# asbschmidt/CUDASW4

Hardware: AMD Instinct MI355X
Metric: GCUPS (higher is better)
Workload: dtype f16x2; 1 GPU; peak: allqueries.fasta (20 queries, 41752 residues) vs pseudo DB 1000000 x 512, half2 kernel configuration, blosum62, gop -11 gex -1, top 10, C++ host driver; db_subjects=1000000, db_residues=512000000, queries=20, kernel=half2, queries_in_flight=1, tail_overlaps=10, numa_node_rank0=0, numa_bound=True, resident=True, residency=resident, cached_chars=512000000, parallelism=db-shard x1 (one DB sharded), one top-K gather per step + host merge

## Files before the change

### cudasw4_amd/capi.py

```python
import ctypes
import os

_HERE = os.path.dirname(os.path.abspath(__file__))
LIB_PATH = os.environ.get("CUDASW4_AMD_LIB", os.path.join(_HERE, "lib", "libcudasw4_amd.so"))

KIND_F16X2, KIND_I16X2, KIND_I32, KIND_F32 = 0, 1, 2, 3
KIND_NAMES = {"half2": KIND_F16X2, "f16x2": KIND_F16X2, "dpxs16": KIND_I16X2, "i16x2": KIND_I16X2,
              "dpxs32": KIND_I32, "i32": KIND_I32, "float": KIND_F32, "f32": KIND_F32}
MAX_ACC = {KIND_F16X2: 2048, KIND_I16X2: 25000}

SW_OK = 0
ERR_NAMES = {-1: "SW_ERR_INVALID", -2: "SW_ERR_HIP", -3: "SW_ERR_NO_QUERY", -4: "SW_ERR_NO_MATRIX",
             -5: "SW_ERR_TEMP", -6: "SW_ERR_NO_DEVICE"}

EXPORTS = ["sw_batch_create", "sw_batch_destroy", "sw_scan_batch", "sw_batch_join", "sw_batch_side_events", "sw_batch_feedback",
           "sw_batch_handshake_active", "sw_batch_stats", "sw_batch_signal_state", "sw_batch_open_gates", "sw_batch_reset",
           "sw_batch_test_lose_side_launch", "sw_query_length", "sw_batch_describe_plan",
           "sw_version", "sw_last_error", "sw_device_count", "sw_ctx_create", "sw_ctx_destroy", "sw_set_matrix",
           "sw_set_query", "sw_scan_temp_bytes", "sw_scan_partition", "sw_rescore_overflow", "sw_rescore_overflow_stat",
           "sw_topk_temp_bytes",
           "sw_topk", "sw_plan_query", "sw_check_letter_codes", "sw_plan_launch", "sw_set_start_signal",
           "sw_window_overlap", "sw_reduce_windows", "sw_rescore_service", "sw_rescore_overflow_claim",
           "sw_rescore_service_temp_bytes", "sw_streams_run_concurrently", "sw_set_dry_signal", "sw_set_dirty_counter", "sw_set_grid_reserve",
           "sw_set_long16_min", "sw_scan_rows_pipelined",
           "sw_scan_rows_pipelined_temp_bytes", "sw_probe_handshake", "sw_launch_vgpr_slot",
           "sw_set_rows_pipeline_slot", "sw_packed_launch_falls_back", "sw_scan_partition_counted", "sw_rescore_overflow_pipelined", "sw_rescore_overflow_pipelined_temp_bytes", "sw_measure_valu_rate",
           "sw_align_hits"]
PSSM_EXPORTS = ["sw_set_query_pssm", "sw_query_is_pssm", "sw_align_hits_pssm", "sw_pssm_accumulate"]
STATS_EXPORTS = ["sw_score_histogram"]
STATS_LBINS, STATS_SBINS = 64, 256
RANK_EXPORTS = ["sw_zscore_keys", "sw_gather_hits"]
RANK_KEY_NONE = -3.0e38
HSPS_EXPORTS = ["sw_align_hsps", "sw_align_hsps_pssm"]
MAX_HSPS = 16
SHUFFLE_EXPORTS = ["sw_shuffle_subjects"]
MASK_EXPORTS = ["sw_mask_subjects", "sw_mask_subjects_phases"]


ALIGN_OK, ALIGN_EMPTY, ALIGN_NO_TRACE, ALIGN_SCORE_MISMATCH, ALIGN_BAD_LENGTH = 0, 1, 2, 3, 4
ALIGN_NOT_COMPUTED = 5
ALIGN_COORDS_ONLY = 1
CIGAR_OPS = {1: "I", 2: "D", 7: "=", 8: "X"}
ALIGN_RESULT_FIELDS = ["score", "status", "q_begin", "q_end", "s_begin", "s_end", "columns", "identities", "mismatches",
                       "gap_opens", "gap_columns", "cigar_len"]


def align_result_dtype():
    import numpy as np
    return np.dtype([(f, np.int32) for f in ALIGN_RESULT_FIELDS] + [("cigar_offset", np.int64)])


def align_trace_bytes(rows, cols):
    return (rows + 511) // 512 * (cols + 63) * 256


def cigar_string(words):
    return "".join("%d%s" % (int(w) >> 4, CIGAR_OPS[int(w) & 15]) for w in words) or "*"


class _AlignArgs(ctypes.Structure):
    _fields_ = [("query", ctypes.c_void_p), ("qlen", ctypes.c_int32), ("n", ctypes.c_int32),
                ("chars", ctypes.c_void_p), ("offsets", ctypes.c_void_p), ("lengths", ctypes.c_void_p),
                ("max_subject_len", ctypes.c_int32), ("gop", ctypes.c_int), ("gex", ctypes.c_int),
                ("expected_scores", ctypes.c_void_p), ("results", ctypes.c_void_p), ("cigar", ctypes.c_void_p),
                ("cigar_offsets", ctypes.c_void_p), ("flags", ctypes.c_int), ("trace_bytes", ctypes.c_size_t),
                ("temp", ctypes.c_void_p), ("temp_bytes", ctypes.c_size_t),
                ("temp_bytes_needed", ctypes.POINTER(ctypes.c_size_t)), ("phase_events", ctypes.c_void_p),
                ("stream", ctypes.c_void_p)]


class _HspArgs(ctypes.Structure):
    _fields_ = [("max_hsps", ctypes.c_int32), ("min_score", ctypes.c_int32)]


class _MaskParams(ctypes.Structure):
    _fields_ = [("window", ctypes.c_int32), ("trigger_sum", ctypes.c_int32), ("extend_sum", ctypes.c_int32)]


class SwError(RuntimeError):
    def __init__(self, code, msg):
        super().__init__("%s (%d): %s" % (ERR_NAMES.get(code, "SW_ERR"), code, msg))
        self.code = code


def _load():
    if not os.path.exists(LIB_PATH):
        raise ImportError("libcudasw4_amd.so is not built (run `python -c 'import __graft_entry__ as g; g.build()'` "
                          "or `make -C cudasw4_amd/csrc`): %s" % LIB_PATH)
    try:
        import torch
    except ImportError:
        pass
    L = ctypes.CDLL(LIB_PATH)
    vp, i32, i64, sz = ctypes.c_void_p, ctypes.c_int32, ctypes.c_int64, ctypes.c_size_t
    L.sw_version.restype = ctypes.c_char_p
    L.sw_last_error.restype = ctypes.c_char_p
    L.sw_device_count.restype = ctypes.c_int
    L.sw_ctx_create.argtypes = [ctypes.c_int, ctypes.POINTER(vp)]
    L.sw_ctx_destroy.argtypes = [vp]
    L.sw_set_matrix.argtypes = [vp, vp, ctypes.c_int]
    L.sw_set_query.argtypes = [vp, vp, i32, vp]
    L.sw_scan_temp_bytes.restype = sz
    L.sw_scan_temp_bytes.argtypes = [vp, ctypes.c_int, ctypes.c_int, i32, i32]
    L.sw_scan_partition.argtypes = [vp, ctypes.c_int, ctypes.c_int, vp, vp, vp, i32, i32, i32, ctypes.c_int,
                                    ctypes.c_int, vp, vp, i64, vp, vp, ctypes.c_int, vp, sz, vp]
    L.sw_rescore_overflow.argtypes = [vp, ctypes.c_int, vp, vp, i32, vp, vp, vp, i32, ctypes.c_int, ctypes.c_int,
                                      vp, vp, i64, vp, sz, vp]
    L.sw_rescore_overflow_stat.argtypes = [vp, ctypes.c_int, vp, vp, i32, vp, vp, vp, i32, ctypes.c_int, ctypes.c_int,
                                           vp, vp, i64, vp, sz, i32, vp, vp]
    L.sw_topk_temp_bytes.restype = sz
    L.sw_topk_temp_bytes.argtypes = [i64, ctypes.c_int]
    L.sw_topk.argtypes = [vp, vp, vp, i64, ctypes.c_int, vp, vp, vp, sz, vp]
    L.sw_plan_query.argtypes = [ctypes.c_int, i32, ctypes.POINTER(i32), ctypes.POINTER(i32)]
    L.sw_check_letter_codes.argtypes = [ctypes.c_void_p, ctypes.c_void_p, ctypes.c_size_t, ctypes.c_void_p, ctypes.c_void_p]
    L.sw_set_start_signal.argtypes = [vp, vp]
    L.sw_probe_handshake.argtypes = [vp, vp, vp, vp]
    L.sw_rescore_overflow_claim.argtypes = [vp, ctypes.c_int, vp, vp, i32, vp, vp, vp, i32, ctypes.c_int, ctypes.c_int, vp, vp, i64, vp, sz, i32, vp, vp]
    L.sw_rescore_overflow_pipelined_temp_bytes.restype = sz
    L.sw_rescore_overflow_pipelined_temp_bytes.argtypes = [vp, i32]
    L.sw_rescore_overflow_pipelined.argtypes = [vp, vp, vp, i32, vp, vp, vp, i32, i32, ctypes.c_int, ctypes.c_int, vp, vp, i64, vp, i32, vp, vp, sz, vp]
    L.sw_measure_valu_rate.argtypes = [vp, ctypes.c_int, ctypes.c_int, ctypes.POINTER(ctypes.c_double), ctypes.POINTER(ctypes.c_double)]
    L.sw_launch_vgpr_slot.argtypes = [vp, ctypes.c_int, ctypes.c_int, i32, i32]
    L.sw_set_rows_pipeline_slot.argtypes = [vp, ctypes.c_int]
    L.sw_set_dry_signal.argtypes = [vp, vp, ctypes.c_uint32]
    L.sw_set_grid_reserve.argtypes = [vp, i32]
    L.sw_set_long16_min.argtypes = [vp, i32]
    L.sw_scan_rows_pipelined_temp_bytes.restype = sz
    L.sw_scan_rows_pipelined_temp_bytes.argtypes = [vp, i32, i32]
    L.sw_scan_rows_pipelined.argtypes = [vp, vp, vp, vp, i32, i32, i32, ctypes.c_int, ctypes.c_int, vp, vp, i64, vp, vp, vp, i32, vp, sz, vp]
    L.sw_window_overlap.argtypes = [vp, ctypes.c_int, ctypes.c_int]
    L.sw_window_overlap.restype = i32
    L.sw_reduce_windows.argtypes = [vp, vp, vp, vp, i32, vp, vp, ctypes.c_int64, vp]
    L.sw_plan_launch.argtypes = [vp, ctypes.c_int, ctypes.c_int, i32, i32, ctypes.POINTER(i32), ctypes.POINTER(i32),
                                 ctypes.POINTER(i32), ctypes.POINTER(i32)]
    if hasattr(L, "sw_align_hits"):
        L.sw_align_hits.argtypes = [vp, ctypes.POINTER(_AlignArgs)]
    if hasattr(L, "sw_set_query_pssm"):
        L.sw_set_query_pssm.argtypes = [vp, vp, i32, vp]
        L.sw_query_is_pssm.argtypes = [vp]
    if hasattr(L, "sw_score_histogram"):
        L.sw_score_histogram.argtypes = [vp, vp, vp, i64, vp, vp, vp, vp]
    if hasattr(L, "sw_zscore_keys"):
        dbl = ctypes.c_double
        L.sw_zscore_keys.argtypes = [vp, vp, vp, i64, dbl, dbl, dbl, dbl, vp, vp, vp, vp]
        L.sw_gather_hits.argtypes = [vp, vp, ctypes.c_int, vp, vp, vp, vp, vp]
    if hasattr(L, "sw_shuffle_subjects"):
        L.sw_shuffle_subjects.argtypes = [vp, vp, vp, vp, vp, i32, ctypes.c_uint32, i32, i32, vp, sz, vp]
    if hasattr(L, "sw_mask_subjects"):
        L.sw_mask_subjects.argtypes = [vp, vp, vp, vp, i32, ctypes.POINTER(_MaskParams), vp, vp, sz, ctypes.POINTER(sz), vp, vp]
        L.sw_mask_subjects_phases.argtypes = [vp, vp, vp, vp, i32, ctypes.POINTER(_MaskParams), vp, vp, sz, vp, vp, ctypes.POINTER(vp)]
    return L


lib = _load()


def check(rc):
    if rc != SW_OK:
        raise SwError(rc, lib.sw_last_error().decode())


def version():
    return lib.sw_version().decode()


def device_count():
    return int(lib.sw_device_count())


def plan_query(kind, qlen):
    r, s = ctypes.c_int32(), ctypes.c_int32()
    check(lib.sw_plan_query(kind, qlen, ctypes.byref(r), ctypes.byref(s)))
    return r.value, s.value


class Context:

    def __init__(self, device=0):
        h = ctypes.c_void_p()
        check(lib.sw_ctx_create(device, ctypes.byref(h)))
        self.handle = h
        self.device = device

    def close(self):
        if self.handle:
            lib.sw_ctx_destroy(self.handle)
            self.handle = None

    def __del__(self):
        try:
            self.close()
        except Exception:
            pass

    def set_matrix(self, m21):
        import numpy as np
        m = np.ascontiguousarray(m21, dtype=np.int8).reshape(-1)
        dim = int(round(len(m) ** 0.5))
        check(lib.sw_set_matrix(self.handle, m.ctypes.data, dim))

    def set_query(self, codes, stream=0):
        import numpy as np
        q = np.ascontiguousarray(codes, dtype=np.int8)
        check(lib.sw_set_query(self.handle, q.ctypes.data, len(q), stream))

    def set_query_pssm(self, pssm, stream=0):
        from . import pssm as _pssm
        if not hasattr(lib, "sw_set_query_pssm"):
            raise SwError(-1, "this build of libcudasw4_amd.so has no sw_set_query_pssm")
        m = _pssm.as_pssm(pssm)
        check(lib.sw_set_query_pssm(self.handle, m.ctypes.data, m.shape[0], stream))

    def query_is_pssm(self):
        return bool(lib.sw_query_is_pssm(self.handle))

    def scan_temp_bytes(self, kind, part_id, n, max_subject_len):
        return int(lib.sw_scan_temp_bytes(self.handle, kind, part_id, n, max_subject_len))

    def scan_partition(self, kind, part_id, chars, offsets, lengths, first_pos, n, max_subject_len, gop, gex,
                       scores, ids, id_offset=0, ovf_pos=0, ovf_count=0, ovf_check=0, temp=0, temp_bytes=0, stream=0):
        check(lib.sw_scan_partition(self.handle, kind, part_id, chars, offsets, lengths, first_pos, n, max_subject_len,
                                    gop, gex, scores, ids, id_offset, ovf_pos, ovf_count, ovf_check, temp, temp_bytes,
                                    stream))

    def measure_valu_rate(self, mix, millis=50):
        r, hz = ctypes.c_double(), ctypes.c_double()
        check(lib.sw_measure_valu_rate(self.handle, mix, millis, ctypes.byref(r), ctypes.byref(hz)))
        return r.value, hz.value

    def launch_vgpr_slot(self, kind, part_id, n, max_subject_len):
        return int(lib.sw_launch_vgpr_slot(self.handle, kind, part_id, n, max_subject_len))

    def set_rows_pipeline_slot(self, vgprs):
        check(lib.sw_set_rows_pipeline_slot(self.handle, vgprs))

    def scan_rows_pipelined_temp_bytes(self, n, max_subject_len):
        return int(lib.sw_scan_rows_pipelined_temp_bytes(self.handle, n, max_subject_len))

    def scan_rows_pipelined(self, chars, offsets, lengths, first_pos, n, max_subject_len, gop, gex, scores, ids, id_offset=0,
                            fail_count=0, temp=0, temp_bytes=0, stream=0, over_limit_count=0, over_limit_count2=0, packed_limit=0):
        check(lib.sw_scan_rows_pipelined(self.handle, chars, offsets, lengths, first_pos, n, max_subject_len, gop, gex, scores,
                                         ids, id_offset, fail_count, over_limit_count, over_limit_count2, packed_limit, temp,
                                         temp_bytes, stream))

    def rescore_overflow_pipelined_temp_bytes(self, max_subject_len):
        return int(lib.sw_rescore_overflow_pipelined_temp_bytes(self.handle, max_subject_len))

    def rescore_overflow_pipelined(self, ovf_pos, ovf_count, max_count, chars, offsets, lengths, max_subject_len, min_subject_len,
                                   gop, gex, scores, ids, id_offset, fail_count, packed_limit, true_count, temp, temp_bytes, stream=0):
        check(lib.sw_rescore_overflow_pipelined(self.handle, ovf_pos, ovf_count, max_count, chars, offsets, lengths, max_subject_len,
                                                min_subject_len, gop, gex, scores, ids, id_offset, fail_count, packed_limit,
                                                true_count, temp, temp_bytes, stream))

    def rescore_overflow_claim(self, kind, ovf_pos, ovf_count, max_count, chars, offsets, lengths, max_subject_len, gop, gex,
                               scores, ids, id_offset, temp, temp_bytes, packed_limit, true_count, stream=0):
        check(lib.sw_rescore_overflow_claim(self.handle, kind, ovf_pos, ovf_count, max_count, chars, offsets, lengths,
                                            max_subject_len, gop, gex, scores, ids, id_offset, temp, temp_bytes, packed_limit,
                                            true_count, stream))

    def rescore_overflow(self, kind, ovf_pos, ovf_count, max_count, chars, offsets, lengths, max_subject_len, gop, gex,
                         scores, ids, id_offset=0, temp=0, temp_bytes=0, stream=0):
        check(lib.sw_rescore_overflow(self.handle, kind, ovf_pos, ovf_count, max_count, chars, offsets, lengths,
                                      max_subject_len, gop, gex, scores, ids, id_offset, temp, temp_bytes, stream))

    def rescore_overflow_stat(self, kind, ovf_pos, ovf_count, max_count, chars, offsets, lengths, max_subject_len, gop, gex,
                              scores, ids, id_offset, temp, temp_bytes, packed_limit, true_count, stream=0):
        check(lib.sw_rescore_overflow_stat(self.handle, kind, ovf_pos, ovf_count, max_count, chars, offsets, lengths,
                                           max_subject_len, gop, gex, scores, ids, id_offset, temp, temp_bytes,
                                           packed_limit, true_count, stream))

    def plan_launch(self, kind, part_id, n, max_subject_len):
        k, r, s, l = ctypes.c_int32(), ctypes.c_int32(), ctypes.c_int32(), ctypes.c_int32()
        check(lib.sw_plan_launch(self.handle, kind, part_id, n, max_subject_len, ctypes.byref(k), ctypes.byref(r),
                                 ctypes.byref(s), ctypes.byref(l)))
        return k.value, r.value, s.value, l.value

    def check_letter_codes(self, chars, n, bad_flag, stream=0):
        check(lib.sw_check_letter_codes(self.handle, chars, n, bad_flag, stream))

    def topk(self, scores, ids, n, k, out_scores, out_ids, temp, temp_bytes, stream=0):
        check(lib.sw_topk(self.handle, scores, ids, n, k, out_scores, out_ids, temp, temp_bytes, stream))


def align_hits(ctx, query, qlen, n, chars, offsets, lengths, max_subject_len, gop, gex, results, cigar=0, cigar_offsets=0,
               expected_scores=0, flags=0, trace_bytes=0, temp=0, temp_bytes=0, stream=0, phase_events=None):
    need = ctypes.c_size_t(0)
    ev = (ctypes.c_void_p * 4)(*phase_events) if phase_events is not None else None
    a = _AlignArgs(query, qlen, n, chars, offsets, lengths, max_subject_len, gop, gex, expected_scores, results, cigar,
                   cigar_offsets, flags, trace_bytes, temp, temp_bytes, ctypes.pointer(need),
                   ctypes.cast(ev, ctypes.c_void_p) if ev is not None else None, stream)
    check(lib.sw_align_hits(ctx.handle if ctx is not None else None, ctypes.byref(a)))
    return int(need.value)


def align_hits_pssm(ctx, pssm, consensus, qlen, n, chars, offsets, lengths, max_subject_len, gop, gex, results, cigar=0,
                    cigar_offsets=0, expected_scores=0, flags=0, trace_bytes=0, temp=0, temp_bytes=0, stream=0, phase_events=None):
    if not hasattr(lib, "sw_align_hits_pssm"):
        raise SwError(-1, "this build of libcudasw4_amd.so has no sw_align_hits_pssm")
    f = lib.sw_align_hits_pssm
    if f.argtypes is None:
        f.argtypes = [ctypes.c_void_p, ctypes.POINTER(_AlignArgs), ctypes.c_void_p]
    need = ctypes.c_size_t(0)
    ev = (ctypes.c_void_p * 4)(*phase_events) if phase_events is not None else None
    a = _AlignArgs(consensus or None, qlen, n, chars, offsets, lengths, max_subject_len, gop, gex, expected_scores, results, cigar,
                   cigar_offsets, flags, trace_bytes, temp, temp_bytes, ctypes.pointer(need),
                   ctypes.cast(ev, ctypes.c_void_p) if ev is not None else None, stream)
    check(f(ctx.handle if ctx is not None else None, ctypes.byref(a), pssm or None))
    return int(need.value)


def _align_args(query, qlen, n, chars, offsets, lengths, max_subject_len, gop, gex, results, cigar, cigar_offsets, expected_scores,
                flags, trace_bytes, temp, temp_bytes, stream, phase_events):
    need = ctypes.c_size_t(0)
    ev = (ctypes.c_void_p * 4)(*phase_events) if phase_events is not None else None
    a = _AlignArgs(query or None, qlen, n, chars, offsets, lengths, max_subject_len, gop, gex, expected_scores, results, cigar,
                   cigar_offsets, flags, trace_bytes, temp, temp_bytes, ctypes.pointer(need),
                   ctypes.cast(ev, ctypes.c_void_p) if ev is not None else None, stream)
    return a, need, ev


def align_hsps(ctx, query, qlen, n, chars, offsets, lengths, max_subject_len, gop, gex, results, cigar=0, cigar_offsets=0,
               max_hsps=1, min_score=1, expected_scores=0, flags=0, trace_bytes=0, temp=0, temp_bytes=0, stream=0,
               phase_events=None):
    if not hasattr(lib, "sw_align_hsps"):
        raise SwError(-1, "this build of libcudasw4_amd.so has no sw_align_hsps")
    f = lib.sw_align_hsps
    if f.argtypes is None:
        f.argtypes = [ctypes.c_void_p, ctypes.POINTER(_AlignArgs), ctypes.POINTER(_HspArgs)]
    a, need, _keep = _align_args(query, qlen, n, chars, offsets, lengths, max_subject_len, gop, gex, results, cigar, cigar_offsets,
                                 expected_scores, flags, trace_bytes, temp, temp_bytes, stream, phase_events)
    h = _HspArgs(max_hsps, min_score)
    check(f(ctx.handle if ctx is not None else None, ctypes.byref(a), ctypes.byref(h)))
    return int(need.value)


def align_hsps_pssm(ctx, pssm, consensus, qlen, n, chars, offsets, lengths, max_subject_len, gop, gex, results, cigar=0,
                    cigar_offsets=0, max_hsps=1, min_score=1, expected_scores=0, flags=0, trace_bytes=0, temp=0, temp_bytes=0,
                    stream=0, phase_events=None):
    if not hasattr(lib, "sw_align_hsps_pssm"):
        raise SwError(-1, "this build of libcudasw4_amd.so has no sw_align_hsps_pssm")
    f = lib.sw_align_hsps_pssm
    if f.argtypes is None:
        f.argtypes = [ctypes.c_void_p, ctypes.POINTER(_AlignArgs), ctypes.POINTER(_HspArgs), ctypes.c_void_p]
    a, need, _keep = _align_args(consensus, qlen, n, chars, offsets, lengths, max_subject_len, gop, gex, results, cigar,
                                 cigar_offsets, expected_scores, flags, trace_bytes, temp, temp_bytes, stream, phase_events)
    h = _HspArgs(max_hsps, min_score)
    check(f(ctx.handle if ctx is not None else None, ctypes.byref(a), ctypes.byref(h), pssm or None))
    return int(need.value)


class _PssmAccumulateArgs(ctypes.Structure):
    _fields_ = [("query", ctypes.c_void_p), ("qlen", ctypes.c_int32), ("n", ctypes.c_int32), ("chars", ctypes.c_void_p),
                ("offsets", ctypes.c_void_p), ("lengths", ctypes.c_void_p), ("results", ctypes.c_void_p),
                ("cigar", ctypes.c_void_p), ("include", ctypes.c_void_p), ("counts", ctypes.c_void_p),
                ("weights", ctypes.c_void_p), ("wcounts", ctypes.c_void_p), ("used", ctypes.c_void_p),
                ("phase_events", ctypes.c_void_p), ("stream", ctypes.c_void_p)]


def pssm_accumulate(ctx, query, qlen, n, chars, offsets, lengths, results, cigar, include, counts, weights, wcounts, used,
                    stream=0, phase_events=None):
    if not hasattr(lib, "sw_pssm_accumulate"):
        raise SwError(-1, "this build of libcudasw4_amd.so has no sw_pssm_accumulate")
    f = lib.sw_pssm_accumulate
    if f.argtypes is None:
        f.argtypes = [ctypes.c_void_p, ctypes.POINTER(_PssmAccumulateArgs)]
    ev = (ctypes.c_void_p * 3)(*phase_events) if phase_events is not None else None
    a = _PssmAccumulateArgs(query or None, qlen, n, chars or None, offsets or None, lengths or None, results or None,
                            cigar or None, include or None, counts or None, weights or None, wcounts or None, used or None,
                            ctypes.cast(ev, ctypes.c_void_p) if ev is not None else None, stream or None)
    check(f(ctx.handle if ctx is not None else None, ctypes.byref(a)))


def score_histogram(ctx, scores, lengths, n, hist, sumlen, skipped, stream=0):
    if not hasattr(lib, "sw_score_histogram"):
        raise SwError(-1, "this build of libcudasw4_amd.so has no sw_score_histogram")
    check(lib.sw_score_histogram(ctx.handle if ctx is not None else None, scores or None, lengths or None, n, hist or None,
                                 sumlen or None, skipped or None, stream or None))


def zscore_keys(ctx, scores, lengths, n, a, b1, sd, z_min, keys, positions=0, count=0, stream=0):
    if not hasattr(lib, "sw_zscore_keys"):
        raise SwError(-1, "this build of libcudasw4_amd.so has no sw_zscore_keys")
    check(lib.sw_zscore_keys(ctx.handle if ctx is not None else None, scores or None, lengths or None, n, a, b1, sd, z_min,
                             keys or None, positions or None, count or None, stream or None))

# ... 45 lines not shown
```

### cudasw4_amd/csrc/sw_api.hip

```cpp
#include <hip/hip_runtime.h>

#include <algorithm>
#include <cstdio>
#include <cmath>
#include <cstdlib>
#include <cstring>
#include <string>

#include "../../include/cudasw4_amd.h"
#include "../../include/cudasw4_amd_engine.h"
#include "../../include/cudasw4_amd_pssm.h"
#include "sw_ctx.hpp"
#include "sw_launch.hpp"
#include "sw_pssm.hpp"
#include "sw_rows_pipeline.hpp"

using swi::fail;
using swi::kWorkSlots;
using swi::Profile;
using swp::LaunchPlan;
using swp::LaunchRequest;
using swp::PlanSettings;

namespace {

thread_local std::string g_last_error = "";

const swk::KindLaunch* kind_launch(int kind) {
    switch (kind) {
        case SW_KIND_F16X2: return &swk::launch_f16x2();
        case SW_KIND_I16X2: return &swk::launch_i16x2();
        case SW_KIND_I32: return &swk::launch_i32();
        case SW_KIND_F32: return &swk::launch_f32();
    }
    return nullptr;
}

bool kind_packed(int kind) { return kind == SW_KIND_F16X2 || kind == SW_KIND_I16X2; }

struct QueryPlan {
    int rows = 0;
    int nstripes = 0;
    int lanes = 16;
};

QueryPlan plan_query(int kind, int32_t qlen, int lanes) {
    const swk::KindLaunch* kl = kind_launch(kind);
    QueryPlan pl;
    pl.lanes = lanes;
    if (!kl || qlen <= 0) return pl;
    const int maxrows = swk::max_rows(kind, lanes);
    const int maxrows_multi = (kind == SW_KIND_F32 && lanes <= 16) ? std::min(maxrows, swk::kMaxRowsScalarMulti) : maxrows;
    double two_wave_penalty = 1.05;
    if (const char* e = getenv("CUDASW4_AMD_TWO_WAVE_PENALTY")) two_wave_penalty = std::max(1.0, atof(e));
    const bool has_three_wave_multi = kl->packed && lanes <= 16 && swk::kWaves3MaxRowsPackedMulti > maxrows / 2;
    double best = 1e300;
    auto consider = [&](int ns) {
        const int64_t per_lane = (qlen + (int64_t)lanes * ns - 1) / ((int64_t)lanes * ns);
        int r = (int)((per_lane + swk::kRowsGranule - 1) / swk::kRowsGranule * swk::kRowsGranule);
        r = std::max(r, swk::kRowsGranule);
        if (r > (ns > 1 ? maxrows_multi : maxrows)) return;
        if (ns > 1 && 2 * r <= maxrows) return;
        double cost = ns * (r + (ns > 1 ? 3.0 : 1.2));
        if (has_three_wave_multi && ns > 1 && r > swk::kWaves3MaxRowsPackedMulti) cost *= two_wave_penalty;
        if (cost < best - 1e-9) { best = cost; pl.rows = r; pl.nstripes = ns; }
    };
    if (qlen <= (int64_t)lanes * maxrows) consider(1);
    const int64_t stripe_multi = (int64_t)lanes * maxrows_multi;
    const int ns_m = std::max<int>(2, (int)((qlen + stripe_multi - 1) / stripe_multi));
    int ns_hi = ns_m + 2;
    if (has_three_wave_multi) {
        const int64_t stripe3 = (int64_t)lanes * swk::kWaves3MaxRowsPackedMulti;
        ns_hi = std::max<int>(ns_hi, (int)((qlen + stripe3 - 1) / stripe3) + 1);
    }
    for (int ns = ns_m; ns <= ns_hi; ns++) consider(ns);
    return pl;
}

}

#ifndef SW_LANES8_MAX_QUERY_PACKED
#define SW_LANES8_MAX_QUERY_PACKED 256
#endif
#ifndef SW_LANES4_MAX_QUERY_PACKED
#define SW_LANES4_MAX_QUERY_PACKED 96
#endif
#ifndef SW_LANES4_MAX_QUERY_SCALAR
#define SW_LANES4_MAX_QUERY_SCALAR 128
#endif
#ifndef SW_LANES4_MAX_SUBJECT
#define SW_LANES4_MAX_SUBJECT 1280
#endif
#ifndef SW_LANES4_MIN_BATCHES_PER_CU
#define SW_LANES4_MIN_BATCHES_PER_CU 12
#endif
#ifndef SW_LANES8_MAX_SUBJECT
#define SW_LANES8_MAX_SUBJECT 192
#endif
#ifndef SW_LANES8_MAX_QUERY_SCALAR
#define SW_LANES8_MAX_QUERY_SCALAR 256
#endif

namespace {

void refresh_score_max(sw_ctx* ctx) { ctx->plan.score_max = std::max(1, ctx->pssm_mode ? ctx->pssm_max : ctx->matrix_max); }
bool have_scores(const sw_ctx* ctx) { return ctx->have_matrix || ctx->pssm_mode; }

int max_grid(const PlanSettings& s) {
    const int g = std::max(1, s.num_cus) * s.grid_mult;
    return s.grid_cap > 0 ? std::min(g, s.grid_cap) : g;
}

int rescore_lanes(int32_t max_subject_len) { return max_subject_len > 1280 ? 64 : 16; }

int shape_index(int lanes) { return lanes == 64 ? 1 : lanes == 8 ? 2 : lanes == 4 ? 3 : 0; }

int effective_kind_of(const PlanSettings& s, int kind, int32_t max_subject_len) {
    if (kind != SW_KIND_I32 || s.i32_native || !s.have_query) return kind;
    const int64_t bound = (int64_t)std::min(s.qlen, max_subject_len) * s.score_max + ((int64_t)1 << 22) + 4096;
    return bound < ((int64_t)1 << 24) ? SW_KIND_F32 : SW_KIND_I32;
}

int lanes_for_partition_any(const PlanSettings& s, int kind, int part_id, int32_t n, int32_t max_subject_len);
int lanes_for_partition(const PlanSettings& s, int kind, int part_id, int32_t n, int32_t max_subject_len) {
    const int lanes = lanes_for_partition_any(s, kind, part_id, n, max_subject_len);
    return (lanes == 16 && kind_packed(kind) && max_subject_len >= 0xffff) ? 64 : lanes;
}
int lanes_for_partition_any(const PlanSettings& s, int kind, int part_id, int32_t n, int32_t max_subject_len) {
    if (part_id < SW_NUM_LENGTH_PARTITIONS - 2) {
        if (!s.have_query) return 16;
        const int32_t limit4 = s.lanes4_max_q >= 0 ? s.lanes4_max_q : kind_packed(kind) ? SW_LANES4_MAX_QUERY_PACKED : SW_LANES4_MAX_QUERY_SCALAR;
        const int64_t batches4 = (int64_t)n / (64 * (kind_packed(kind) ? 2 : 1));
        const bool enough4 = s.lanes4_max_q >= 0 || batches4 >= (int64_t)SW_LANES4_MIN_BATCHES_PER_CU * std::max(1, s.num_cus);
        const int32_t lmax4 = s.lanes4_max_subject >= 0 ? s.lanes4_max_subject : SW_LANES4_MAX_SUBJECT;
        if (s.qlen <= 4 * swk::max_rows(kind, 4) && s.qlen <= limit4 && enough4 && max_subject_len <= lmax4) return 4;
        const bool fits8 = s.qlen <= 8 * swk::max_rows(kind, 8);
        const int32_t limit = s.lanes8_max_q >= 0 ? s.lanes8_max_q : kind_packed(kind) ? SW_LANES8_MAX_QUERY_PACKED : SW_LANES8_MAX_QUERY_SCALAR;
        if (fits8 && s.qlen <= limit) return 8;
        return 16;
    }
    const int64_t fills_gpu_twice = (int64_t)2 * std::max(1, s.num_cus) * 4 * 32;
    if (part_id == SW_NUM_LENGTH_PARTITIONS - 2) return n >= (s.long16_min >= 0 ? s.long16_min : 512) ? 16 : 64;
    return n >= fills_gpu_twice ? 16 : 64;
}


int ensure_profile(sw_ctx* ctx, const LaunchPlan& lp, int shift, hipStream_t stream) {
    Profile& pr = ctx->profiles[lp.kind][shape_index(lp.lanes)][lp.frame];
    if (pr.valid && (pr.shift != shift || pr.rows != lp.rows || pr.nstripes != lp.nstripes)) pr.valid = false;
    if (pr.valid) {
        SW_HIP(hipStreamWaitEvent(stream, pr.ready, 0));
        return SW_OK;
    }
    const swk::KindLaunch* kl = kind_launch(lp.kind);
    const int32_t qlen = ctx->plan.qlen;
    const size_t bytes = kl->tile_bytes(lp.rows, lp.lanes) * (size_t)lp.nstripes;
    if (bytes == 0) return fail(SW_ERR_INVALID, "no kernel compiled for this query plan");
    if (bytes > pr.capacity) {
        const size_t cap = std::max<size_t>(std::max(bytes, 2 * pr.capacity), size_t(2) << 20);
        if (pr.dev) SW_HIP(hipFree(pr.dev));
        pr.dev = nullptr;
        pr.capacity = 0;
        SW_HIP(hipMalloc(&pr.dev, cap));
        pr.capacity = cap;
    }
    if (ctx->pssm_mode) SW_HIP(kl->profile(lp.rows, lp.lanes, nullptr, qlen, ctx->d_pssm, qlen, lp.nstripes, pr.dev, shift, lp.frame == 2 ? 1 : 0, stream));
    else SW_HIP(kl->profile(lp.rows, lp.lanes, ctx->d_query, qlen, ctx->d_matrix, ctx->dim, lp.nstripes, pr.dev, shift, lp.frame == 2 ? 1 : 0, stream));
    pr.shift = shift;
    if (!pr.ready) SW_HIP(hipEventCreateWithFlags(&pr.ready, hipEventDisableTiming));
    SW_HIP(hipEventRecord(pr.ready, stream));
    pr.rows = lp.rows;
    pr.nstripes = lp.nstripes;
    pr.valid = true;
    return SW_OK;
}

int32_t border_capacity(int32_t max_len, int lanes) {
    const int64_t steps = ((int64_t)max_len + lanes - 1 + 3) / 4 * 4;
    return (int32_t)((steps + 15) / 16 * 16 + 16);
}
size_t border_bytes_per_wg(int32_t lcap, int lanes) {
    if (lanes == 4) return 0;
    const size_t region = lanes == 16 ? swk::group_region_words<16>(lcap) : lanes == 8 ? swk::group_region_words<8>(lcap) : swk::group_region_words<64>(lcap);
    return (size_t)(swk::kThreads / lanes) * region * sizeof(uint32_t);
}

constexpr int kChainMinRounds = 16;
constexpr int32_t kChainMaxSubject = 1024;
int chain_wanted(const PlanSettings& s, int kind, int lanes, bool multi, int stream_slots, int64_t nbatches, int32_t max_subject_len) {
    if (!kind_packed(kind) || lanes != 16 || !multi || stream_slots != 1) return 1;
    if (s.chain <= 1 || max_subject_len > kChainMaxSubject) return 1;
    if (!s.chain_all && nbatches <= (int64_t)std::max(s.chain, kChainMinRounds) * max_grid(s)) return 1;
    return std::min<int>(s.chain, swk::kChainMax);
}
int32_t chain_capacity(int32_t max_len, int chain, int lanes) {
    return border_capacity((int32_t)std::min<int64_t>(swk::chain_columns(max_len, chain), SW_MAX_SUBJECT_LEN), lanes);
}
size_t chain_bytes_per_wg(int32_t max_len, int chain, int lanes) {
    if (chain <= 1) return border_bytes_per_wg(border_capacity(max_len, lanes), lanes);
    return border_bytes_per_wg(chain_capacity(max_len, chain, lanes), lanes) + (size_t)(swk::kThreads / lanes) * swk::kChainMaxWords * sizeof(uint32_t);
}

__global__ void max_length_kernel(const int32_t* lengths, const int32_t* positions, const int32_t* count_ptr, int32_t first_pos,
                                  int32_t n, int32_t* out) {
    const int32_t cnt = count_ptr ? min(*count_ptr, n) : n;
    int32_t m = 0;
    for (int32_t i = blockIdx.x * blockDim.x + threadIdx.x; i < cnt; i += gridDim.x * blockDim.x)
        m = max(m, lengths[positions ? positions[i] : first_pos + i]);
    if (m > 0) atomicMax(out, m);
}

struct StreamPlan { int slots = 0, cols = 0, room = 0, base = 0, jump = 0; };
StreamPlan stream_plan(const PlanSettings& s, int kind, int lanes, int a, const QueryPlan& pl, int32_t max_subject_len) {
    StreamPlan sp;
    if (!kind_packed(kind) || lanes != 16 || a < 0) return sp;
    const bool multi = pl.nstripes > 1;
    const int P = swk::frame_classes(true, pl.rows, lanes, multi);
    sp.base = kind == SW_KIND_F16X2 ? -2016 : 0;
    const int top = kind == SW_KIND_F16X2 ? 1024 : 12400;
    sp.jump = s.stream_jump > 0 ? s.stream_jump : (kind == SW_KIND_F16X2 ? 512 : 2048);
    sp.room = top - sp.base - a * (2 * lanes + 4 + P);
    sp.cols = a > 0 ? std::min(sp.room / a, s.stream_cols_max) : s.stream_cols_max;
    sp.slots = std::max(1, std::min(s.stream_slots, swk::kStreamMaxSlots));
    if (sp.room < 4 * lanes * a || sp.cols < 4 * lanes) sp.slots = 1;
    if (multi) {
        const int32_t limit = s.stream_multi_max_subject >= 0 ? s.stream_multi_max_subject : (kind == SW_KIND_F16X2 ? 320 : 192);
        if (max_subject_len > limit) sp.slots = 1;
        sp.cols = std::min(sp.cols, s.stream_multi_cols_max);
    }
    return sp;
}

bool offs_possible(const PlanSettings& s, int kind, int lanes, int32_t max_subject_len, int gop, int gex, int ovf_check, int64_t* K_out) {
    const int a = -gex;
    const int64_t room = kind == SW_KIND_F16X2 ? 1536 : kind == SW_KIND_I16X2 ? 12500 : (int64_t)1 << 22;
    int64_t K = 1 << 21;
    while (K >= 4 * lanes && (int64_t)a * (K + 3 * lanes + 16) > room) K >>= 1;
    if (kind == SW_KIND_I16X2) K = std::min<int64_t>(K, std::max<int64_t>(2048, 4 * lanes));
    if (!kind_packed(kind) && max_subject_len + 3 * lanes + 16 > K) K = 0;
    if (K_out) *K_out = K;
    return s.use_offs && K >= 4 * lanes && (!kind_packed(kind) || (ovf_check && a >= 0)) && gop - gex >= -1000;
}
int packed_fallback_kind(int kind) { return kind == SW_KIND_F16X2 ? SW_KIND_F32 : SW_KIND_I32; }

}

namespace swp {

void settings_from_env(PlanSettings& s) {
    if (const char* e = getenv("CUDASW4_AMD_GRID_CAP")) s.grid_cap = std::max(0, atoi(e));
    if (const char* e = getenv("CUDASW4_AMD_NO_OFFS")) s.use_offs = !(e[0] == '1');
    if (const char* e = getenv("CUDASW4_AMD_I32_NATIVE")) s.i32_native = e[0] == '1';
    if (const char* e = getenv("CUDASW4_AMD_LANES8_MAX_Q")) s.lanes8_max_q = atoi(e);
    if (const char* e = getenv("CUDASW4_AMD_LANES4_MAX_Q")) s.lanes4_max_q = atoi(e);
    if (const char* e = getenv("CUDASW4_AMD_LANES4_MAX_SUBJECT")) s.lanes4_max_subject = atoi(e);
    if (const char* e = getenv("CUDASW4_AMD_STREAM")) s.stream_slots = std::max(0, std::min(swk::kStreamMaxSlots, atoi(e)));
    if (const char* e = getenv("CUDASW4_AMD_CHAIN")) s.chain = std::max(1, std::min(swk::kChainMax, atoi(e)));
    if (const char* e = getenv("CUDASW4_AMD_CHAIN_ALL")) s.chain_all = e[0] == '1';
}

LaunchPlan plan_launch(const PlanSettings& s, const LaunchRequest& req) {
    LaunchPlan lp;
    const int32_t max_len = req.max_subject_len;
    lp.kind = req.kind;
    if (!kind_launch(req.kind)) return lp;
    const bool list = req.part_id < 0;
    auto lanes_of = [&](int kind) { return list ? rescore_lanes(max_len) : lanes_for_partition(s, kind, req.part_id, req.n, max_len); };
    lp.kind = effective_kind_of(s, req.kind, max_len);
    lp.lanes = lanes_of(lp.kind);
    int64_t K = 0;
    if (req.gaps_known) {
        lp.offs = offs_possible(s, lp.kind, lp.lanes, max_len, req.gop, req.gex, req.ovf_list, &K);
        if (kind_packed(lp.kind) && !lp.offs) {
            lp.fell_back = true;
            lp.kind = effective_kind_of(s, packed_fallback_kind(lp.kind), max_len);
            lp.lanes = lanes_of(lp.kind);
            lp.offs = offs_possible(s, lp.kind, lp.lanes, max_len, req.gop, req.gex, false, &K);
        }
    }
    const int kind = lp.kind, lanes = lp.lanes;
    if (!s.have_query || max_len < 0) return lp;
    lp.valid = true;
    const QueryPlan pl = plan_query(kind, s.qlen, lanes);
    lp.rows = pl.rows;
    lp.nstripes = pl.nstripes;
    lp.multi = pl.nstripes > 1;
    lp.vgpr_slot = pl.rows > 0 ? swk::vgpr_slot_of(kind, pl.rows, lanes, lp.multi) : 0;
    const StreamPlan sp = req.service_workgroups > 0 ? StreamPlan() : stream_plan(s, kind, lanes, req.gaps_known ? -req.gex : 1, pl, max_len);
    lp.stream_slots = sp.slots; lp.stream_cols = sp.cols; lp.stream_room = sp.room; lp.stream_base = sp.base; lp.stream_jump = sp.jump;
    const bool uniform = swk::uniform_frame_launch(kind_packed(kind), lp.offs, lanes, lp.multi, sp.slots);
    lp.frame = lp.offs ? (uniform ? 2 : 1) : 0;
    if (lp.offs) {
        lp.flag_period = K;
        lp.period = uniform ? std::min<int64_t>(K, swk::kUniformMaxPeriod) : K;
    }
    const int subj_per_batch = (swk::kThreads / lanes) * (kind_packed(kind) ? 2 : 1);
    lp.nbatches = std::max<int64_t>(0, ((int64_t)req.n + subj_per_batch - 1) / subj_per_batch);
    int64_t grid = std::min<int64_t>(lp.nbatches, max_grid(s));
    if (req.service_workgroups > 0) grid = std::min<int64_t>(grid, req.service_workgroups);
    if (lp.multi) {
        auto round_capacity = [&](int cols) { return border_capacity(sp.slots > 1 ? std::max(max_len, cols) : max_len, lanes); };
        int cols = sp.cols;
        int chain = (list || req.claim || req.service_workgroups > 0) ? 1 : chain_wanted(s, kind, lanes, true, sp.slots, lp.nbatches, max_len);
        auto per_wg = [&]() { return chain > 1 ? chain_bytes_per_wg(max_len, chain, lanes) : border_bytes_per_wg(round_capacity(cols), lanes); };
        lp.scratch_needed = (size_t)grid * per_wg();
        if (sp.slots > 1) {
            while (cols > max_len && (size_t)grid * per_wg() > req.scratch) cols = cols * 3 / 4;
            lp.stream_cols = cols;
        }
        while (chain > 1 && (size_t)grid * per_wg() > req.scratch) chain--;
        lp.chain = chain;
        lp.lcap = chain > 1 ? chain_capacity(max_len, chain, lanes) : round_capacity(cols);
        lp.bytes_per_wg = per_wg();
        lp.scratch_too_small = req.scratch < lp.bytes_per_wg;
        if (lp.bytes_per_wg > 0) grid = (int64_t)std::min<size_t>((size_t)grid, req.scratch / lp.bytes_per_wg);
    }
    lp.grid = (int)grid;
    if (!req.gaps_known && kind_packed(req.kind) && !list) {
        LaunchRequest fb = req;
        fb.kind = packed_fallback_kind(req.kind);
        lp.scratch_needed = std::max(lp.scratch_needed, plan_launch(s, fb).scratch_needed);
    }
    return lp;
}

}

namespace {

constexpr uint32_t kWorkZeroBlock = 64;
hipError_t take_work_slot(sw_ctx* ctx, hipStream_t stream, uint32_t** out) {
    uint32_t* w = ctx->d_work + 2 * (ctx->work_next++ % kWorkSlots);
    *out = w;
    if (ctx->work_zeroed > 0) { ctx->work_zeroed--; return hipSuccess; }
    return hipMemsetAsync(w, 0, 2 * sizeof(uint32_t), stream);
}

struct Signals {
    uint32_t* start = nullptr;
    uint32_t* dry = nullptr;
};
Signals take_signals(sw_ctx* ctx) {
    const Signals sg{ctx->start_signal, ctx->dry_signal};
    ctx->start_signal = nullptr;
    ctx->dry_signal = nullptr;
    return sg;
}

int check_max_subject_len(sw_ctx* ctx, const int32_t* lengths, const int32_t* positions, const int32_t* count_ptr, int32_t first_pos,
                          int32_t n, int32_t max_subject_len, hipStream_t stream) {
    if (!ctx->check_bounds) return SW_OK;
    int32_t* slot = reinterpret_cast<int32_t*>(ctx->d_zeros + 64);
    int32_t longest = 0;
    SW_HIP(hipMemsetAsync(slot, 0, sizeof(int32_t), stream));
    hipLaunchKernelGGL(max_length_kernel, dim3(std::min(1024, (n + 255) / 256)), dim3(256), 0, stream, lengths, positions, count_ptr, first_pos, n, slot);
    SW_HIP(hipGetLastError());
    SW_HIP(hipMemcpyAsync(&longest, slot, sizeof(int32_t), hipMemcpyDeviceToHost, stream));
    SW_HIP(hipStreamSynchronize(stream));
    if (longest > max_subject_len)
        return fail(SW_ERR_INVALID, "max_subject_len " + std::to_string(max_subject_len) + " under-reports: a subject of the range has " +
                                        std::to_string(longest) + " residues");
    return SW_OK;
}

struct KindCode {
    swk::u32 (*encode_gap)(int);
    swk::u32 (*zero_at)(int, int);
    swk::u32 (*pos_word)(int);
};
template <int KIND>
constexpr KindCode kind_code() { return {swk::Arith<KIND>::encode_gap, swk::Arith<KIND>::zero_at, swk::Arith<KIND>::pos_word}; }
const KindCode kKindCode[4] = {kind_code<swk::F16X2>(), kind_code<swk::I16X2>(), kind_code<swk::I32>(), kind_code<swk::F32>()};

swk::ScanParams fill_scan_params(const LaunchPlan& lp, int gop, int gex) {
    const KindCode& code = kKindCode[lp.kind];
    const int a = -gex;
    swk::ScanParams p{};
    p.nstripes = lp.nstripes;
    p.gop = code.encode_gap(gop); p.gex = code.encode_gap(gex);
    if (lp.offs) {
        p.gop = code.encode_gap(gop - gex);
        p.gex_mag = a;
        const bool uniform = lp.frame == 2;
        const int P = swk::frame_classes(kind_packed(lp.kind), lp.rows, lp.lanes, lp.multi, uniform);
        p.wrap_class = code.encode_gap(-a * P);
        p.wrap_last = code.encode_gap(-a * ((lp.rows - 1) % P + (uniform ? 0 : 1)));
        p.flag_period = (int32_t)lp.flag_period;
        p.renorm_quads = (int32_t)(lp.period / 4);
        p.renorm_word = code.encode_gap(-(int)((int64_t)a * lp.period));
        if (uniform) {
            p.uniform_frame = 1;
            for (int u = 0; u < swk::kLevelWords; u++) p.levels[u] = code.zero_at(a, std::min<int>(u, (int)lp.period + 16));
        }
    }
    if (lp.stream_slots >= 1) {
        p.stream_slots = lp.stream_slots; p.stream_cols = lp.stream_cols; p.stream_room = lp.stream_room; p.level_base = lp.stream_base;
        p.jump = lp.stream_jump; p.jump_limit = lp.stream_jump - 4;
        p.jump_word = code.pos_word(lp.stream_jump);
    }
    if (lp.multi) p.lcap = lp.lcap;
    if (lp.chain > 1) p.chain = lp.chain;
    p.start_quorum = (uint32_t)std::min(lp.grid, 64);
    return p;
}

struct ListMode {
    int32_t* claim = nullptr;
    int service_workgroups = 0;
    const uint32_t* done_flag = nullptr;
    uint32_t done_value = 0;
};

LaunchRequest launch_request(int kind, int part_id, int32_t n, int32_t max_subject_len, int gop, int gex, bool ovf_list, size_t scratch,
                             const ListMode& list = ListMode()) {
    LaunchRequest req;
    req.kind = kind; req.part_id = part_id; req.n = n; req.max_subject_len = max_subject_len;
    req.gaps_known = true; req.gop = gop; req.gex = gex; req.ovf_list = ovf_list;
    req.claim = list.claim != nullptr; req.service_workgroups = list.service_workgroups;
    req.scratch = scratch;
    return req;
}
LaunchRequest sizing_request(int kind, int part_id, int32_t n, int32_t max_subject_len) {
    LaunchRequest req;
    req.kind = kind; req.part_id = part_id; req.n = n; req.max_subject_len = max_subject_len;
    return req;
}

int scan_common(sw_ctx* ctx, const LaunchPlan& lp, const Signals& sg, const int8_t* chars, const uint64_t* offsets, const int32_t* lengths,
                const int32_t* positions, const int32_t* count_ptr, int32_t first_pos, int32_t n,
                int32_t max_subject_len, int gop, int gex, float* scores, int32_t* ids, int64_t id_offset,
                int32_t* ovf_pos, int32_t* ovf_count, int ovf_check, void* temp,
                hipStream_t stream, int32_t* stat_count = nullptr, int32_t stat_limit = 0, const ListMode& list = ListMode()) {
    const int kind = lp.kind, lanes = lp.lanes;
    const swk::KindLaunch* kl = kind_launch(kind);
    if (n < 0 || max_subject_len < 0) return fail(SW_ERR_INVALID, "negative count or length");
    if (max_subject_len > SW_MAX_SUBJECT_LEN)
        return fail(SW_ERR_INVALID, "max_subject_len " + std::to_string(max_subject_len) + ": pass the longest subject of the range (lengths[last]), not the partition's nominal boundary");
    if (gop > 0 || gex > 0) return fail(SW_ERR_INVALID, "gap scores must be <= 0");
    if (kind_packed(kind) && (gop < -1000 || gex < -1000)) return fail(SW_ERR_INVALID, "gap score out of range for a 16-bit kind");
    if (!have_scores(ctx)) return fail(SW_ERR_NO_MATRIX, "sw_set_matrix has not been called");
    if (!ctx->plan.have_query) return fail(SW_ERR_NO_QUERY, "sw_set_query has not been called");
    if (n == 0) return SW_OK;
    if (lp.fell_back) { ovf_pos = nullptr; ovf_count = nullptr; ovf_check = 0; }
    if (!chars || !offsets || !lengths || !scores || !ids) return fail(SW_ERR_INVALID, "null buffer");
    if (ovf_check && kind_packed(kind) && (!ovf_pos || !ovf_count)) return fail(SW_ERR_INVALID, "overflow check without overflow buffers");
    SW_HIP(hipSetDevice(ctx->device));
    int rc = check_max_subject_len(ctx, lengths, positions, count_ptr, first_pos, n, max_subject_len, stream);
    if (rc != SW_OK) return rc;
    if (kind_packed(kind) && !lp.offs) return fail(SW_ERR_INVALID, "internal: a packed launch without the column-offset recurrence (packed_fallback_kind)");
    rc = ensure_profile(ctx, lp, lp.offs ? -gex : 0, stream);
    if (rc != SW_OK) return rc;

    swk::ScanParams p = fill_scan_params(lp, gop, gex);
    p.claim = list.claim;
    p.service = list.service_workgroups > 0 ? 1 : 0;
    p.done_flag = list.done_flag;
    p.done_value = list.done_value;
    p.chars = chars; p.offsets = offsets; p.lengths = lengths;
    p.positions = positions; p.count_ptr = count_ptr;
    p.first_pos = first_pos; p.n = n;
    p.profile = ctx->profiles[kind][shape_index(lanes)][lp.frame].dev;
    p.scores = scores; p.ids = ids; p.id_offset = id_offset;
    p.ovf_pos = ovf_pos; p.ovf_count = ovf_count; p.ovf_check = (ovf_check && kind_packed(kind)) ? 1 : 0;
    p.zeros = ctx->d_zeros + kind * 16;
    p.stat_count = stat_count; p.stat_limit = stat_limit;
    if (lp.chain > 1) p.chain_all = ctx->plan.chain_all ? 1 : 0;
    if (lp.multi) {
        if (lp.scratch_too_small) return fail(SW_ERR_TEMP, "temp buffer too small for a multi-stripe query");
        p.scratch = static_cast<uint32_t*>(temp);
    }
    SW_HIP(take_work_slot(ctx, stream, &p.work_counter));
    p.start_signal = sg.start;
    p.dry_signal = sg.dry;
    if (!stat_count && !positions && p.stream_slots > 1 && lanes == 16 && kind_packed(kind)) { p.stat_count = ctx->dirty_counter; p.stat_limit = INT32_MAX; }
    p.dry_value = ctx->dry_value;
    const int reserve = (list.service_workgroups > 0 || list.claim) ? 0 : ctx->grid_reserve;
    SW_HIP(kl->scan(lp.rows, lanes, lp.multi, lp.offs, lp.grid, reserve, stream, p));
    return SW_OK;
}

}


namespace swi {
int fail(int code, const std::string& msg) {
    g_last_error = msg;
    return code;
}
int32_t query_length(const sw_ctx* ctx) { return ctx && ctx->plan.have_query ? ctx->plan.qlen : 0; }
int device_of(const sw_ctx* ctx) { return ctx ? ctx->device : -1; }
int num_cus(const sw_ctx* ctx) { return ctx ? ctx->plan.num_cus : 0; }
const int8_t* matrix(const sw_ctx* ctx, int* dim) {
    if (!ctx || !ctx->have_matrix) return nullptr;
    *dim = ctx->dim;
    return ctx->d_matrix;
}
}

namespace {
template <class Fill>
int install_query(sw_ctx* ctx, int8_t** dev, size_t* dev_capacity, size_t bytes, int32_t qlen, bool pssm, void* stream, Fill fill) {
    SW_HIP(hipSetDevice(ctx->device));
    if (bytes > *dev_capacity) {
        if (*dev) SW_HIP(hipFree(*dev));
        *dev = nullptr;
        *dev_capacity = 0;
        const size_t cap = std::max<size_t>((bytes + 4095) / 4096 * 4096 * 2, size_t(1) << 16);
        SW_HIP(hipMalloc(dev, cap));
        *dev_capacity = cap;
    }
    hipStream_t s = static_cast<hipStream_t>(stream);
    const int slot = ctx->query_next;
    ctx->query_next = (ctx->query_next + 1) % sw_ctx::kQuerySlots;
    if (ctx->query_slot_used[slot]) SW_HIP(hipEventSynchronize(ctx->query_copied[slot]));
    if (bytes > ctx->h_query_capacity[slot]) {
        if (ctx->h_query[slot]) SW_HIP(hipHostFree(ctx->h_query[slot]));
        ctx->h_query[slot] = nullptr;
        ctx->h_query_capacity[slot] = 0;
        const size_t cap = std::max<size_t>((bytes + 4095) / 4096 * 4096 * 2, size_t(1) << 16);
        SW_HIP(hipHostMalloc(&ctx->h_query[slot], cap));
        ctx->h_query_capacity[slot] = cap;
    }
    if (!ctx->query_copied[slot]) SW_HIP(hipEventCreateWithFlags(&ctx->query_copied[slot], hipEventDisableTiming));
    fill(ctx->h_query[slot]);
    SW_HIP(hipMemcpyAsync(*dev, ctx->h_query[slot], bytes, hipMemcpyHostToDevice, s));
    ctx->work_next = (ctx->work_next + kWorkZeroBlock - 1) / kWorkZeroBlock * kWorkZeroBlock;
    SW_HIP(hipMemsetAsync(ctx->d_work + 2 * (ctx->work_next % kWorkSlots), 0, 2 * kWorkZeroBlock * sizeof(uint32_t), s));
    ctx->work_zeroed = kWorkZeroBlock;
    SW_HIP(hipEventRecord(ctx->query_copied[slot], s));
    ctx->query_slot_used[slot] = true;
    ctx->plan.qlen = qlen;
    ctx->plan.have_query = true;
    ctx->pssm_mode = pssm;
    refresh_score_max(ctx);
    for (auto& row : ctx->profiles)
        for (auto& shape : row)
            for (auto& pr : shape) pr.valid = false;
    return SW_OK;
}
// ... 267 lines not shown
        else out_pos[slot] = -1;
    }
    __syncthreads();
    if (threadIdx.x == 0) *out_count = min(k, cap);
}
constexpr int32_t kPipeRescoreCap = 64;
size_t pipe_rescore_header_bytes() { return 256 + (size_t)kPipeRescoreCap * sizeof(int32_t); }
}

int sw_scan_rows_pipelined(sw_ctx* ctx, const int8_t* chars, const uint64_t* offsets, const int32_t* lengths, int32_t first_pos,
                           int32_t n, int32_t max_subject_len, int gop, int gex, float* scores, int32_t* ids, int64_t id_offset,
                           int32_t* fail_count, int32_t* over_limit_count, int32_t* over_limit_count2, int32_t packed_limit,
                           void* temp, size_t temp_bytes, void* stream_) {
    if (!ctx) return fail(SW_ERR_INVALID, "null context");
    const Signals sg = take_signals(ctx);
    uint32_t* const start_signal = sg.start;
    const bool dry_armed = sg.dry != nullptr;
    hipStream_t stream = static_cast<hipStream_t>(stream_);
    if ((int64_t)max_subject_len * (int64_t)(-gex) >= ((int64_t)1 << 28)) return fail(SW_ERR_INVALID, "subject length x gap extension out of range for sw_scan_rows_pipelined");
    const int rc = rows_common_checks(ctx, chars, offsets, lengths, first_pos, n, max_subject_len, gop, gex, scores, ids, dry_armed, stream, "sw_scan_rows_pipelined");
    if (rc != SW_OK || n == 0) return rc;
    const int cpl = pipeline_cpl(ctx, n, max_subject_len);
    const int64_t stages = pipeline_stages(cpl, max_subject_len);
    const int64_t tickets = (int64_t)n * stages;
    if (tickets > (int64_t)1 << 24) return fail(SW_ERR_INVALID, "too many pipeline stages for one sw_scan_rows_pipelined launch");
    const size_t need = kPipeCtrlBytes + (size_t)tickets * ((size_t)ctx->plan.qlen + 1) * sizeof(unsigned long long);
    if (!temp || temp_bytes < need) return fail(SW_ERR_TEMP, "temp buffer too small for sw_scan_rows_pipelined (sw_scan_rows_pipelined_temp_bytes)");
    swk::PipelineParams p{};
    p.chars = chars; p.offsets = offsets; p.lengths = lengths; p.first_pos = first_pos; p.n = n;
    p.gop = gop; p.gex = gex; p.scores = scores; p.ids = ids; p.id_offset = id_offset;
    p.fail_count = fail_count;
    p.stat_count = over_limit_count; p.stat_count2 = over_limit_count2; p.stat_limit = packed_limit;
    return launch_pipeline(ctx, p, cpl, stages, tickets, start_signal, temp, stream);
}

size_t sw_rescore_overflow_pipelined_temp_bytes(sw_ctx* ctx, int32_t max_subject_len) {
    if (!ctx || !ctx->plan.have_query || max_subject_len < 0) return 0;
    const int64_t tickets = (int64_t)kPipeRescoreCap * pipeline_stages(pipeline_cpl(ctx, kPipeRescoreCap, max_subject_len), max_subject_len);
    return pipe_rescore_header_bytes() + kPipeCtrlBytes + (size_t)tickets * ((size_t)ctx->plan.qlen + 1) * sizeof(unsigned long long);
}

int sw_rescore_overflow_pipelined(sw_ctx* ctx, int32_t* ovf_pos, const int32_t* ovf_count, int32_t max_count, const int8_t* chars,
                                  const uint64_t* offsets, const int32_t* lengths, int32_t max_subject_len, int32_t min_subject_len,
                                  int gop, int gex, float* scores, int32_t* ids, int64_t id_offset, int32_t* fail_count,
                                  int32_t packed_limit, int32_t* true_overflow_count, void* temp, size_t temp_bytes, void* stream_) {
    if (!ctx) return fail(SW_ERR_INVALID, "null context");
    const bool dry_armed = take_signals(ctx).dry != nullptr;
    hipStream_t stream = static_cast<hipStream_t>(stream_);
    if (!ovf_pos || !ovf_count) return fail(SW_ERR_INVALID, "null overflow buffers");
    if (max_count <= 0) return SW_OK;
    if ((int64_t)max_subject_len * (int64_t)(-gex) >= ((int64_t)1 << 28)) return fail(SW_ERR_INVALID, "subject length x gap extension out of range for sw_rescore_overflow_pipelined");
    const int rc = rows_common_checks(ctx, chars, offsets, lengths, 0, 1, max_subject_len, gop, gex, scores, ids, dry_armed, stream, "sw_rescore_overflow_pipelined");
    if (rc != SW_OK) return rc;
    const int cpl = pipeline_cpl(ctx, kPipeRescoreCap, max_subject_len);
    const int64_t stages = pipeline_stages(cpl, max_subject_len);
    const int64_t tickets = (int64_t)kPipeRescoreCap * stages;
    const size_t need = sw_rescore_overflow_pipelined_temp_bytes(ctx, max_subject_len);
    if (!temp || temp_bytes < need) return fail(SW_ERR_TEMP, "temp buffer too small for sw_rescore_overflow_pipelined");
    int32_t* out_count = static_cast<int32_t*>(temp);
    int32_t* out_pos = reinterpret_cast<int32_t*>(static_cast<char*>(temp) + 256);
    hipLaunchKernelGGL(pipeline_pick_kernel, dim3(1), dim3(256), 0, stream, ovf_pos, ovf_count, max_count, lengths, std::max(min_subject_len, 1),
                       kPipeRescoreCap, out_pos, out_count);
    SW_HIP(hipGetLastError());
    swk::PipelineParams p{};
    p.chars = chars; p.offsets = offsets; p.lengths = lengths; p.first_pos = 0; p.n = kPipeRescoreCap;
    p.positions = out_pos; p.count_ptr = out_count;
    p.gop = gop; p.gex = gex; p.scores = scores; p.ids = ids; p.id_offset = id_offset;
    p.fail_count = fail_count;
    p.stat_count = true_overflow_count; p.stat_count2 = nullptr; p.stat_limit = packed_limit;
    return launch_pipeline(ctx, p, cpl, stages, tickets, nullptr, static_cast<char*>(temp) + pipe_rescore_header_bytes(), stream);
}

int sw_set_dirty_counter(sw_ctx* ctx, int32_t* counter) {
    if (!ctx) return fail(SW_ERR_INVALID, "null context");
    ctx->dirty_counter = counter;
    return SW_OK;
}

int sw_set_dry_signal(sw_ctx* ctx, uint32_t* signal, uint32_t value) {
    if (!ctx) return fail(SW_ERR_INVALID, "null context");
    ctx->dry_signal = signal;
    ctx->dry_value = value;
    return SW_OK;
}

int sw_set_long16_min(sw_ctx* ctx, int32_t subjects) {
    if (!ctx) return fail(SW_ERR_INVALID, "null context");
    ctx->plan.long16_min = subjects < 0 ? ctx->long16_min_default : subjects;
    return SW_OK;
}

int sw_set_grid_reserve(sw_ctx* ctx, int32_t workgroups) {
    if (!ctx) return fail(SW_ERR_INVALID, "null context");
    if (workgroups < 0) return fail(SW_ERR_INVALID, "negative reserve");
    ctx->grid_reserve = workgroups;
    return SW_OK;
}

namespace {
__global__ void reduce_windows_kernel(const float* __restrict__ win_scores, const int32_t* __restrict__ win_first,
                                      const int32_t* __restrict__ real_pos, int32_t n_real, float* __restrict__ scores,
                                      int32_t* __restrict__ ids, int64_t id_offset) {
    const int32_t i = blockIdx.x * blockDim.x + threadIdx.x;
    if (i >= n_real) return;
    float m = -1.0f;
    for (int32_t w = win_first[i]; w < win_first[i + 1]; w++) m = fmaxf(m, win_scores[w]);
    const int32_t pos = real_pos[i];
    scores[pos] = m;
    ids[pos] = (int32_t)(id_offset + pos);
}
}

int32_t sw_window_overlap(sw_ctx* ctx, int gop, int gex) {
    if (!ctx || !ctx->plan.have_query || !have_scores(ctx)) return -1;
    const int cost = std::min(-gop, -gex);
    if (cost <= 0) return -1;
    const int64_t span = (int64_t)ctx->plan.qlen + (int64_t)ctx->plan.qlen * ctx->plan.score_max / cost + 1;
    return span > 0x3fffffff ? -1 : (int32_t)span;
}

int sw_reduce_windows(sw_ctx* ctx, const float* win_scores, const int32_t* win_first, const int32_t* real_pos, int32_t n_real,
                      float* scores, int32_t* ids, int64_t id_offset, void* stream) {
    if (!ctx) return fail(SW_ERR_INVALID, "null context");
    if (n_real <= 0) return SW_OK;
    if (!win_scores || !win_first || !real_pos || !scores || !ids) return fail(SW_ERR_INVALID, "null buffer");
    SW_HIP(hipSetDevice(ctx->device));
    hipLaunchKernelGGL(reduce_windows_kernel, dim3((n_real + 255) / 256), dim3(256), 0, static_cast<hipStream_t>(stream), win_scores,
                       win_first, real_pos, n_real, scores, ids, id_offset);
    SW_HIP(hipGetLastError());
    return SW_OK;
}

int sw_plan_query(int kind, int32_t qlen, int32_t* rows_per_lane, int32_t* nstripes) {
    if (!kind_launch(kind) || qlen <= 0) return fail(SW_ERR_INVALID, "bad kind or query length");
    const QueryPlan pl = plan_query(kind, qlen, 16);
    if (rows_per_lane) *rows_per_lane = pl.rows;
    if (nstripes) *nstripes = pl.nstripes;
    return SW_OK;
}

int sw_plan_launch(sw_ctx* ctx, int kind, int part_id, int32_t n, int32_t max_subject_len, int32_t* effective_kind,
                   int32_t* rows_per_lane, int32_t* nstripes, int32_t* lanes) {
    if (!ctx || !kind_launch(kind)) return fail(SW_ERR_INVALID, "null context or unknown kind");
    if (!ctx->plan.have_query) return fail(SW_ERR_NO_QUERY, "sw_set_query has not been called");
    if (part_id >= SW_NUM_LENGTH_PARTITIONS || max_subject_len < 0) return fail(SW_ERR_INVALID, "bad partition id or length");
    const LaunchPlan lp = swp::plan_launch(ctx->plan, sizing_request(kind, part_id, n, max_subject_len));
    if (effective_kind) *effective_kind = lp.kind;
    if (rows_per_lane) *rows_per_lane = lp.rows;
    if (nstripes) *nstripes = lp.nstripes;
    if (lanes) *lanes = lp.lanes;
    return SW_OK;
}

int sw_launch_vgpr_slot(sw_ctx* ctx, int kind, int part_id, int32_t n, int32_t max_subject_len) {
    if (!ctx || !kind_launch(kind) || !ctx->plan.have_query || part_id >= SW_NUM_LENGTH_PARTITIONS || max_subject_len < 0) return 0;
    return swp::plan_launch(ctx->plan, sizing_request(kind, part_id, n, max_subject_len)).vgpr_slot;
}

int sw_set_rows_pipeline_slot(sw_ctx* ctx, int vgprs) {
    if (!ctx) return fail(SW_ERR_INVALID, "null context");
    if (vgprs != 0 && vgprs != 128 && vgprs != 168 && vgprs != 256) return fail(SW_ERR_INVALID, "a register-file slot is 128, 168 or 256 VGPRs (0: as few as the stage needs)");
    ctx->pipe_slot = vgprs;
    return SW_OK;
}

size_t sw_scan_temp_bytes(sw_ctx* ctx, int kind, int part_id, int32_t n, int32_t max_subject_len) {
    if (!ctx || !ctx->plan.have_query || !kind_launch(kind) || max_subject_len < 0 || n <= 0) return 0;
    return swp::plan_launch(ctx->plan, sizing_request(kind, part_id, n, max_subject_len)).scratch_needed;
}

int sw_scan_partition(sw_ctx* ctx, int kind, int part_id, const int8_t* chars, const uint64_t* offsets,
                      const int32_t* lengths, int32_t first_pos, int32_t n, int32_t max_subject_len, int gop, int gex,
                      float* scores, int32_t* ids, int64_t id_offset, int32_t* ovf_pos, int32_t* ovf_count,
                      int ovf_check, void* temp, size_t temp_bytes, void* stream) {
    if (!ctx) return fail(SW_ERR_INVALID, "null context");
    const Signals sg = take_signals(ctx);
    if (part_id < 0 || part_id >= SW_NUM_LENGTH_PARTITIONS || !kind_launch(kind))
        return fail(SW_ERR_INVALID, part_id < 0 || part_id >= SW_NUM_LENGTH_PARTITIONS ? "partition id out of range" : "unknown kind");
    const LaunchPlan lp = swp::plan_launch(ctx->plan, launch_request(kind, part_id, n, max_subject_len, gop, gex, ovf_check != 0, temp ? temp_bytes : 0));
    return scan_common(ctx, lp, sg, chars, offsets, lengths, nullptr, nullptr, first_pos, n, max_subject_len, gop, gex,
                       scores, ids, id_offset, ovf_pos, ovf_count, ovf_check, temp, static_cast<hipStream_t>(stream));
}

namespace {
bool packed_range(const sw_ctx* ctx, int kind, int part_id) {
    return ctx && kind_launch(kind) && kind_packed(kind) && ctx->plan.have_query && part_id >= 0 && part_id < SW_NUM_LENGTH_PARTITIONS;
}
__global__ void add_counter_kernel(const int32_t* src, int32_t* dst) {
    if (*src) atomicAdd(dst, *src);
}
}

int sw_packed_launch_falls_back(sw_ctx* ctx, int kind, int part_id, int32_t n, int32_t max_subject_len, int gop, int gex) {
    if (!packed_range(ctx, kind, part_id)) return 0;
    return swp::plan_launch(ctx->plan, launch_request(kind, part_id, n, max_subject_len, gop, gex, true, swp::kUnlimitedScratch)).fell_back ? 1 : 0;
}

int sw_scan_partition_counted(sw_ctx* ctx, int kind, int part_id, const int8_t* chars, const uint64_t* offsets,
                              const int32_t* lengths, int32_t first_pos, int32_t n, int32_t max_subject_len, int gop, int gex,
                              float* scores, int32_t* ids, int64_t id_offset, int32_t packed_limit, int32_t* over_limit_count,
                              int32_t* over_limit_total, void* temp, size_t temp_bytes, void* stream) {
    if (!ctx) return fail(SW_ERR_INVALID, "null context");
    const Signals sg = take_signals(ctx);
    LaunchPlan lp;
    if (over_limit_count && packed_range(ctx, kind, part_id))
        lp = swp::plan_launch(ctx->plan, launch_request(kind, part_id, n, max_subject_len, gop, gex, true, temp ? temp_bytes : 0));
    if (!lp.fell_back)
        return fail(SW_ERR_INVALID, "sw_scan_partition_counted: not a packed launch that falls back to its 32-bit kind, or no counter");
    const int rc = scan_common(ctx, lp, sg, chars, offsets, lengths, nullptr, nullptr, first_pos, n, max_subject_len, gop, gex,
                               scores, ids, id_offset, nullptr, nullptr, 0, temp, static_cast<hipStream_t>(stream),
                               over_limit_count, packed_limit);
    if (rc != SW_OK || n == 0 || !over_limit_total) return rc;
    hipLaunchKernelGGL(add_counter_kernel, dim3(1), dim3(1), 0, static_cast<hipStream_t>(stream), over_limit_count, over_limit_total);
    SW_HIP(hipGetLastError());
    return SW_OK;
}

namespace {
int rescore_list(sw_ctx* ctx, int kind, const int32_t* ovf_pos, const int32_t* ovf_count, int32_t max_count, const int8_t* chars,
                 const uint64_t* offsets, const int32_t* lengths, int32_t max_subject_len, int gop, int gex, float* scores, int32_t* ids,
                 int64_t id_offset, void* temp, size_t temp_bytes, int32_t packed_limit, int32_t* true_overflow_count, const ListMode& list,
                 bool service, void* stream) {
    if (!ctx) return fail(SW_ERR_INVALID, "null context");
    const Signals sg = take_signals(ctx);
    if (kind != SW_KIND_I32 && kind != SW_KIND_F32) return fail(SW_ERR_INVALID, "overflow re-score needs a 32-bit kind");
    if (service && (!ovf_pos || !ovf_count || !list.done_flag)) return fail(SW_ERR_INVALID, "null overflow buffers or flag");
    if (!ovf_pos || !ovf_count) return fail(SW_ERR_INVALID, "null overflow buffers");
    if (max_count <= 0 || (service && list.service_workgroups <= 0)) return SW_OK;
    const LaunchPlan lp = swp::plan_launch(ctx->plan, launch_request(kind, -1, max_count, max_subject_len, gop, gex, false, temp ? temp_bytes : 0, list));
    return scan_common(ctx, lp, sg, chars, offsets, lengths, ovf_pos, ovf_count, 0, max_count, max_subject_len, gop, gex,
                       scores, ids, id_offset, nullptr, nullptr, 0, temp, static_cast<hipStream_t>(stream),
                       true_overflow_count, packed_limit, list);
}
}

int sw_rescore_overflow(sw_ctx* ctx, int kind, const int32_t* ovf_pos, const int32_t* ovf_count, int32_t max_count,
                        const int8_t* chars, const uint64_t* offsets, const int32_t* lengths, int32_t max_subject_len,
                        int gop, int gex, float* scores, int32_t* ids, int64_t id_offset, void* temp,
                        size_t temp_bytes, void* stream) {
    return sw_rescore_overflow_stat(ctx, kind, ovf_pos, ovf_count, max_count, chars, offsets, lengths, max_subject_len, gop, gex,
                                    scores, ids, id_offset, temp, temp_bytes, 0, nullptr, stream);
}

int sw_rescore_overflow_stat(sw_ctx* ctx, int kind, const int32_t* ovf_pos, const int32_t* ovf_count, int32_t max_count,
                             const int8_t* chars, const uint64_t* offsets, const int32_t* lengths, int32_t max_subject_len,
                             int gop, int gex, float* scores, int32_t* ids, int64_t id_offset, void* temp,
                             size_t temp_bytes, int32_t packed_limit, int32_t* true_overflow_count, void* stream) {
    return rescore_list(ctx, kind, ovf_pos, ovf_count, max_count, chars, offsets, lengths, max_subject_len, gop, gex, scores, ids, id_offset,
                        temp, temp_bytes, packed_limit, true_overflow_count, ListMode(), false, stream);
}

size_t sw_rescore_service_temp_bytes(sw_ctx* ctx, int kind, int32_t max_subject_len, int workgroups) {
    if (!ctx || !ctx->plan.have_query || !kind_launch(kind) || max_subject_len < 0 || workgroups <= 0) return 0;
    LaunchRequest req = sizing_request(kind, -1, 0, max_subject_len);
    req.service_workgroups = workgroups;
    return (size_t)workgroups * swp::plan_launch(ctx->plan, req).bytes_per_wg;
}

int sw_rescore_service(sw_ctx* ctx, int kind, int32_t* ovf_pos, const int32_t* ovf_count, int32_t max_count,
                       const int8_t* chars, const uint64_t* offsets, const int32_t* lengths, int32_t max_subject_len,
                       int gop, int gex, float* scores, int32_t* ids, int64_t id_offset, void* temp, size_t temp_bytes,
                       int32_t packed_limit, int32_t* true_overflow_count, const uint32_t* done_flag, uint32_t done_value,
                       int workgroups, void* stream) {
    ListMode lm;
    lm.claim = ovf_pos;
    lm.service_workgroups = workgroups;
    lm.done_flag = done_flag;
    lm.done_value = done_value;
    return rescore_list(ctx, kind, ovf_pos, ovf_count, max_count, chars, offsets, lengths, max_subject_len, gop, gex, scores, ids, id_offset,
                        temp, temp_bytes, packed_limit, true_overflow_count, lm, true, stream);
}

int sw_rescore_overflow_claim(sw_ctx* ctx, int kind, int32_t* ovf_pos, const int32_t* ovf_count, int32_t max_count,
                              const int8_t* chars, const uint64_t* offsets, const int32_t* lengths, int32_t max_subject_len,
                              int gop, int gex, float* scores, int32_t* ids, int64_t id_offset, void* temp, size_t temp_bytes,
                              int32_t packed_limit, int32_t* true_overflow_count, void* stream) {
    ListMode lm;
    lm.claim = ovf_pos;
    return rescore_list(ctx, kind, ovf_pos, ovf_count, max_count, chars, offsets, lengths, max_subject_len, gop, gex, scores, ids, id_offset,
                        temp, temp_bytes, packed_limit, true_overflow_count, lm, false, stream);
}

}
```

### cudasw4_amd/csrc/sw_ctx.hpp

```cpp
#pragma once
#include <hip/hip_runtime.h>

#include <cstddef>
#include <cstdint>
#include <string>

#include "../../include/cudasw4_amd.h"
#include "sw_internal.hpp"
#include "sw_plan.hpp"

#define SW_HIP(expr)                                                                              \
    do {                                                                                          \
        hipError_t e__ = (expr);                                                                  \
        if (e__ != hipSuccess)                                                                    \
            return swi::fail(SW_ERR_HIP, std::string(#expr) + ": " + hipGetErrorString(e__));     \
    } while (0)

namespace swi {
struct Profile {
    unsigned char* dev = nullptr;
    size_t capacity = 0;
    bool valid = false;
    int rows = 0, nstripes = 0;
    int shift = 0;
    hipEvent_t ready = nullptr;
};
constexpr uint32_t kWorkSlots = 4096;
}

struct sw_ctx {
    int device = 0;
    swp::PlanSettings plan;
    int8_t* d_matrix = nullptr;
    int dim = 21;
    uint32_t* d_zeros = nullptr;
    uint32_t* d_work = nullptr;
    uint32_t work_next = 0;
    uint32_t work_zeroed = 0;
    uint32_t* start_signal = nullptr;
    uint32_t* dry_signal = nullptr;
    int32_t* dirty_counter = nullptr;
    uint32_t dry_value = 0;
    int grid_reserve = 0;
    bool have_matrix = false;
    int8_t* d_query = nullptr;
    size_t query_capacity = 0;
    static constexpr int kQuerySlots = 4;
    int8_t* h_query[kQuerySlots] = {};
    size_t h_query_capacity[kQuerySlots] = {};
    hipEvent_t query_copied[kQuerySlots] = {};
    bool query_slot_used[kQuerySlots] = {};
    int query_next = 0;
    bool pssm_mode = false;
    int8_t* d_pssm = nullptr;
    size_t pssm_capacity = 0;
    int pssm_max = 1;
    swi::Profile profiles[4][4][3];
    int64_t long16_min_default = -1;
    int matrix_max = 1;
    bool check_bounds = false;
    uint32_t pipe_spin_limit = 1u << 20;
    int32_t pipe_drop_stage = -1;
    int32_t pipe_cpl = 0;
    int32_t pipe_quorum = 0;
    int32_t pipe_slot = 0;
};
```

### cudasw4_amd/csrc/sw_dp_kernel.hpp

```cpp
#pragma once

#include <hip/hip_runtime.h>
#include <stdint.h>

#include <type_traits>

#include "sw_pssm.hpp"

namespace swk {

typedef uint32_t u32;
typedef short s16x2 __attribute__((ext_vector_type(2)));
typedef unsigned short u16x2 __attribute__((ext_vector_type(2)));
typedef _Float16 f16x2 __attribute__((ext_vector_type(2)));

constexpr int kGroup = 16;
constexpr int kThreads = 256;
constexpr int kPadLetter = 20;
constexpr int kLetters = 21;

enum { F16X2 = 0, I16X2 = 1, I32 = 2, F32 = 3 };

constexpr int DPP_ROW_SHL1 = 0x101;
constexpr int DPP_ROW_SHR1 = 0x111;
constexpr int DPP_ROW_ROR1 = 0x121;
constexpr int DPP_QUAD_SHR1 = 0x90;
constexpr int DPP_WAVE_SHL1 = 0x130;
constexpr int DPP_WAVE_SHR1 = 0x138;

template <int LANES>
struct Shift {
    static_assert(LANES == 4 || LANES == 8 || LANES == 16 || LANES == 64, "group = a DPP quad, half a DPP row, a DPP row or the whole wave");
    static constexpr int kShr1 = LANES <= 16 ? DPP_ROW_SHR1 : DPP_WAVE_SHR1;
    static constexpr int kShl1 = LANES <= 16 ? DPP_ROW_SHL1 : DPP_WAVE_SHL1;
};

template <int CTRL, bool ZERO_FILL>
__device__ __forceinline__ u32 dpp(u32 old, u32 src) {
    return (u32)__builtin_amdgcn_update_dpp((int)old, (int)src, CTRL, 0xf, 0xf, ZERO_FILL);
}

template <int LANES, bool ZERO_FILL>
__device__ __forceinline__ u32 prev_lane(u32 headval, u32 src, bool head) {
    if constexpr (LANES == 8) {
        const u32 v = dpp<DPP_ROW_SHR1, false>(headval, src);
        return head ? headval : v;
    } else if constexpr (LANES == 4) {
        const u32 v = dpp<DPP_QUAD_SHR1, false>(headval, src);
        return head ? headval : v;
    } else {
        (void)head;
        return dpp<Shift<LANES>::kShr1, ZERO_FILL>(headval, src);
    }
}

template <int KIND>
struct Arith;

template <>
struct Arith<I16X2> {
    static constexpr bool kPacked = true;
    static constexpr int kSubjects = 2;
    static constexpr int kLimit = 25000;
    static constexpr bool kWindow = true;
    static constexpr int kBias = 1024;
    static constexpr u32 kZero = (u32)kBias | ((u32)kBias << 16);
    static __host__ __device__ u32 encode_gap(int g) { u32 m = (u32)(-g) & 0xffffu; return m | (m << 16); }
    static __host__ __device__ u32 encode_score(int s) { return (u32)(uint16_t)(int16_t)s; }
    static __device__ __forceinline__ u32 add(u32 a, u32 b) {
        return __builtin_bit_cast(u32, (u16x2)(__builtin_bit_cast(u16x2, a) + __builtin_bit_cast(u16x2, b)));
    }
    static __device__ __forceinline__ u32 max3(u32 a, u32 b, u32 c) {
        return __builtin_bit_cast(u32, __builtin_elementwise_maximum(
            __builtin_elementwise_maximum(__builtin_bit_cast(f16x2, a), __builtin_bit_cast(f16x2, b)),
            __builtin_bit_cast(f16x2, c)));
    }
    static __device__ __forceinline__ u32 max2(u32 a, u32 b) {
        return __builtin_bit_cast(u32, __builtin_elementwise_maximum(__builtin_bit_cast(f16x2, a), __builtin_bit_cast(f16x2, b)));
    }
    static __device__ __forceinline__ u32 cell_h(u32 t, u32 e, u32 f) { return max3(t, e, f); }
    static __device__ __forceinline__ u32 gap(u32 a, u32 g) {
        return __builtin_bit_cast(u32, (u16x2)(__builtin_bit_cast(u16x2, a) - __builtin_bit_cast(u16x2, g)));
    }
    static __device__ __forceinline__ u32 fold2(u32 m, u32 a, u32 b) { return max3(m, a, b); }
    static __host__ __device__ u32 zero_at(int a, int k) { u32 z = (u32)(kBias + a * k) & 0xffffu; return z | (z << 16); }
    static __host__ __device__ u32 pos_word(int a) { u32 m = (u32)a & 0xffffu; return m | (m << 16); }
    static __device__ __forceinline__ u32 level_word(int v) { const u32 z = (u32)(kBias + v) & 0xffffu; return z | (z << 16); }
    static __device__ __forceinline__ u32 true_of(u32 m, u32 z) { return gap(m, z); }
    static __device__ __forceinline__ u32 lower(u32 a, u32 w) {
        return __builtin_bit_cast(u32, __builtin_elementwise_sub_sat(__builtin_bit_cast(u16x2, a), __builtin_bit_cast(u16x2, w)));
    }
    static __device__ __forceinline__ u32 true_max(u32 a, u32 b) {
        return __builtin_bit_cast(u32, __builtin_elementwise_max(__builtin_bit_cast(u16x2, a), __builtin_bit_cast(u16x2, b)));
    }
    static __device__ __forceinline__ int true_lo(u32 v) { return (int)(v & 0xffffu); }
    static __device__ __forceinline__ int true_hi(u32 v) { return (int)(v >> 16); }
    static constexpr u32 kOne = 1u;
    static __device__ __forceinline__ u32 add_pair(u32 wa, u32 wb, u32 c) {
        u32 d;
        asm("v_pk_mad_u16 %0, %1, %2, %3 op_sel:[0,1,0] op_sel_hi:[1,0,1]" : "=v"(d) : "v"(wa), "v"(wb), "v"(c));
        return d;
    }
};

template <>
struct Arith<F16X2> {
    static constexpr bool kPacked = true;
    static constexpr int kSubjects = 2;
    static constexpr int kLimit = 2048;
    static constexpr bool kWindow = true;
    static constexpr u32 kZero = 0u;
    static __host__ __device__ u32 half_bits(int v) {
        if (v == 0) return 0;
        u32 sign = v < 0 ? 0x8000u : 0u;
        u32 a = (u32)(v < 0 ? -v : v);
        int e = 0;
        while ((a >> (e + 1)) != 0) e++;
        u32 mant = (a << (10 - e)) & 0x3ffu;
        return sign | ((u32)(e + 15) << 10) | mant;
    }
    static __host__ __device__ u32 encode_gap(int g) { u32 h = half_bits(g); return h | (h << 16); }
    static __host__ __device__ u32 encode_score(int s) { return half_bits(s); }
    static __device__ __forceinline__ u32 add(u32 a, u32 b) {
        return __builtin_bit_cast(u32, (f16x2)(__builtin_bit_cast(f16x2, a) + __builtin_bit_cast(f16x2, b)));
    }
    static __device__ __forceinline__ u32 max3(u32 a, u32 b, u32 c) {
        return __builtin_bit_cast(u32, __builtin_elementwise_maximum(
            __builtin_elementwise_maximum(__builtin_bit_cast(f16x2, a), __builtin_bit_cast(f16x2, b)),
            __builtin_bit_cast(f16x2, c)));
    }
    static __device__ __forceinline__ u32 max2(u32 a, u32 b) {
        return __builtin_bit_cast(u32, __builtin_elementwise_maximum(__builtin_bit_cast(f16x2, a), __builtin_bit_cast(f16x2, b)));
    }
    static __device__ __forceinline__ u32 cell_h(u32 t, u32 e, u32 f) { return max3(t, e, f); }
    static __device__ __forceinline__ u32 gap(u32 a, u32 g) { return add(a, g); }
    static __device__ __forceinline__ u32 fold2(u32 m, u32 a, u32 b) { return max3(m, a, b); }
    static __host__ __device__ u32 zero_at(int a, int k) { u32 h = half_bits(a * k); return h | (h << 16); }
    static __host__ __device__ u32 pos_word(int a) { u32 h = half_bits(a); return h | (h << 16); }
    static __device__ __forceinline__ u32 level_word(int v) {
        const u32 h = (u32)__builtin_bit_cast(unsigned short, (_Float16)(float)v);
        return h | (h << 16);
    }
    static __device__ __forceinline__ u32 true_of(u32 m, u32 z) {
        return __builtin_bit_cast(u32, (f16x2)(__builtin_bit_cast(f16x2, m) - __builtin_bit_cast(f16x2, z)));
    }
    static __device__ __forceinline__ u32 lower(u32 a, u32 w) { return add(a, w); }
    static __device__ __forceinline__ u32 true_max(u32 a, u32 b) { return max2(a, b); }
    static __device__ __forceinline__ int true_lo(u32 v) { return (int)(float)__builtin_bit_cast(f16x2, v).x; }
    static __device__ __forceinline__ int true_hi(u32 v) { return (int)(float)__builtin_bit_cast(f16x2, v).y; }
    static constexpr u32 kOne = 0x3c00u;
    static __device__ __forceinline__ u32 add_pair(u32 wa, u32 wb, u32 c) {
        u32 d;
        asm("v_pk_fma_f16 %0, %1, %2, %3 op_sel:[0,1,0] op_sel_hi:[1,0,1]" : "=v"(d) : "v"(wa), "v"(wb), "v"(c));
        return d;
    }
};

template <>
struct Arith<I32> {
    static constexpr bool kPacked = false;
    static constexpr int kSubjects = 1;
    static constexpr int kLimit = 0x7fffffff;
    static constexpr bool kWindow = true;
    static constexpr u32 kZero = 0u;
    static __host__ __device__ u32 encode_gap(int g) { return (u32)g; }
    static __host__ __device__ u32 encode_score(int s) { return (u32)s; }
    static __device__ __forceinline__ u32 max3(u32 a, u32 b, u32 c) {
        u32 d;
        asm("v_max3_i32 %0, %1, %2, %3" : "=v"(d) : "v"(a), "v"(b), "v"(c));
        return d;
    }
    static __device__ __forceinline__ u32 max3_zero(u32 a, u32 b) {
        u32 d;
        asm("v_max3_i32 %0, %1, %2, 0" : "=v"(d) : "v"(a), "v"(b));
        return d;
    }
    static __device__ __forceinline__ u32 add(u32 a, u32 b) { return a + b; }
    static __device__ __forceinline__ u32 max2(u32 a, u32 b) { return (u32)((int)a > (int)b ? (int)a : (int)b); }
    static __device__ __forceinline__ u32 cell_h(u32 t, u32 e, u32 f) { return max3(t, e, f); }
    static __device__ __forceinline__ u32 gap(u32 a, u32 g) { return a + g; }
    static __device__ __forceinline__ u32 gap_state(u32 ext, u32 open) { return max3_zero(ext, open); }
    static __device__ __forceinline__ u32 fold2(u32 m, u32 a, u32 b) { return max3(m, a, b); }
    static __device__ __forceinline__ int score_lo(u32 v) { return (int)v; }
    static __host__ __device__ u32 zero_at(int a, int k) { return (u32)(a * k); }
    static __host__ __device__ u32 pos_word(int a) { return (u32)a; }
    static __device__ __forceinline__ u32 true_of(u32 m, u32 z) { return m - z; }
    static __device__ __forceinline__ u32 true_max(u32 a, u32 b) { return max2(a, b); }
    static __device__ __forceinline__ int true_lo(u32 v) { return (int)v; }
    static __device__ __forceinline__ int true_hi(u32) { return 0; }
};

template <>
struct Arith<F32> {
    static constexpr bool kPacked = false;
    static constexpr int kSubjects = 1;
    static constexpr int kLimit = 0x7fffffff;
    static constexpr bool kWindow = false;
    static constexpr u32 kZero = 0u;
    static __host__ __device__ u32 encode_gap(int g) { return __builtin_bit_cast(u32, (float)g); }
    static __host__ __device__ u32 encode_score(int s) { return __builtin_bit_cast(u32, (float)s); }
    static __device__ __forceinline__ float f(u32 v) { return __builtin_bit_cast(float, v); }
    static __device__ __forceinline__ u32 u(float v) { return __builtin_bit_cast(u32, v); }
    static __device__ __forceinline__ u32 add(u32 a, u32 b) { return u(f(a) + f(b)); }
    static __device__ __forceinline__ u32 max2(u32 a, u32 b) { return u(__builtin_fmaxf(f(a), f(b))); }
    static __device__ __forceinline__ u32 max3(u32 a, u32 b, u32 c) { return u(__builtin_fmaxf(__builtin_fmaxf(f(a), f(b)), f(c))); }
    static __device__ __forceinline__ u32 cell_h(u32 t, u32 e, u32 ff) { return u(__builtin_fmaxf(__builtin_fmaxf(f(t), f(e)), f(ff))); }
    static __device__ __forceinline__ u32 gap(u32 a, u32 g) { return u(f(a) + f(g)); }
    static __device__ __forceinline__ u32 gap_state(u32 ext, u32 open) { return u(__builtin_fmaxf(__builtin_fmaxf(f(ext), f(open)), 0.0f)); }
    static __device__ __forceinline__ u32 fold2(u32 m, u32 a, u32 b) { return u(__builtin_fmaxf(__builtin_fmaxf(f(m), f(a)), f(b))); }
    static __device__ __forceinline__ int score_lo(u32 v) { return (int)f(v); }
    static __host__ __device__ u32 zero_at(int a, int k) { return __builtin_bit_cast(u32, (float)(a * k)); }
    static __host__ __device__ u32 pos_word(int a) { return __builtin_bit_cast(u32, (float)a); }
    static __device__ __forceinline__ u32 true_of(u32 m, u32 z) { return u(f(m) - f(z)); }
    static __device__ __forceinline__ u32 true_max(u32 a, u32 b) { return max2(a, b); }
    static __device__ __forceinline__ int true_lo(u32 v) { return (int)f(v); }
    static __device__ __forceinline__ int true_hi(u32) { return 0; }
};

template <int NW>
struct Chunks {
    static constexpr int kRem = NW % 4;
    static constexpr int kWant3 = (4 - kRem) % 4;
    static constexpr bool kSplit = NW >= 3 * kWant3;
    static constexpr int kN3 = kSplit ? kWant3 : 1;
    static constexpr int kN4 = kSplit ? (NW - 3 * kWant3) / 4 : NW / 4;
    static constexpr int kCount = kN4 + kN3;
    static constexpr int first(int c) { return c < kN4 ? 4 * c : 4 * kN4 + 3 * (c - kN4); }
    static constexpr int words(int c) { return c < kN4 ? 4 : (kSplit ? 3 : kRem); }
    static constexpr int chunk_of(int w) { return w < 4 * kN4 ? w / 4 : kN4 + (w - 4 * kN4) / 3; }
    static constexpr bool starts_chunk(int w) { return first(chunk_of(w)) == w; }
    static constexpr bool lead_ok(int lead, int ahead, int slack) {
        for (int r = 0; r < NW; r++) {
            const int need = chunk_of(r + ahead < NW ? r + ahead : NW - 1);
            if (need >= lead && first(need - lead) + slack > r) return false;
        }
        return true;
    }
    static constexpr int lead_for(int ahead, int slack) {
        int lead = 1;
        while (lead < kCount && !lead_ok(lead, ahead, slack)) lead++;
        return lead;
    }
};

template <int KIND, int R, int LANES = kGroup>
struct Geometry {
    static constexpr bool kPacked = Arith<KIND>::kPacked;
    static constexpr bool kWide = kPacked && LANES <= 16;
    static constexpr int NW = (kPacked && !kWide) ? (R + 1) / 2 : R;
    using C = Chunks<NW>;
    static constexpr int NCH = C::kCount;
    static constexpr int kChunkRowBytes = (LANES <= 16 ? 16 : LANES) * 16;
    static constexpr int kRowBytes = NCH * kChunkRowBytes;
    static constexpr int kTileBytes = kLetters * kRowBytes;
    static constexpr int kStripeRows = LANES * R;
    static constexpr int kLetterShift = LANES <= 16 ? 8 : 10;
    static constexpr int kLetterUnits = kRowBytes >> kLetterShift;
    static_assert(kPadLetter * kLetterUnits < 256, "letter offset must fit a byte");
};

constexpr int kUniformMaxPeriod = 256;
constexpr int kLevelWords = kUniformMaxPeriod + 16;

struct ScanParams {
    const int8_t* chars;
    const uint64_t* offsets;
    const int32_t* lengths;
    const int32_t* positions;
    const int32_t* count_ptr;
    int32_t first_pos;
    int32_t n;
    const unsigned char* profile;
    int32_t nstripes;
    u32 gop, gex;
    float* scores;
    int32_t* ids;
    int64_t id_offset;
    int32_t* ovf_pos;
    int32_t* ovf_count;
    int32_t ovf_check;
    u32* scratch;
    int32_t lcap;
    const u32* zeros;
    u32* work_counter;
    int32_t gex_mag;
    int32_t renorm_quads;
    u32 renorm_word;
    u32 wrap_class;
    u32 wrap_last;
    int32_t* stat_count;
    int32_t stat_limit;
    u32* start_signal;
    u32 start_quorum;
    int32_t* claim;
    int32_t service;
    const u32* done_flag;
    u32 done_value;
    u32* dry_signal;
    u32 dry_value;
    int32_t stream_slots;
    int32_t stream_cols;
    int32_t stream_room;
    int32_t level_base;
    int32_t jump;
    u32 jump_word;
    int32_t jump_limit;
    int32_t uniform_frame;
    int32_t flag_period;
    int32_t chain;
    int32_t chain_all;
    u32 levels[kLevelWords];
};

constexpr int32_t kListEmpty = -1, kListTaken = -2;

typedef u32 u32x3 __attribute__((ext_vector_type(3)));

template <int NW, int CHUNK_ROW_BYTES>
__device__ __forceinline__ void lds_read_chunk(u32 (&dst)[NW], const unsigned char* p, int c) {
    using C = Chunks<NW>;
    const int w = C::first(c);
    if (c < C::kN4) {
        const uint4 v = *reinterpret_cast<const uint4*>(p + c * CHUNK_ROW_BYTES);
        dst[w + 0] = v.x; dst[w + 1] = v.y; dst[w + 2] = v.z; dst[w + 3] = v.w;
    } else if (c < C::kCount) {
        const u32x3 v = *reinterpret_cast<const u32x3*>(p + c * CHUNK_ROW_BYTES);
        if constexpr (C::kSplit) {
            dst[w + 0] = v.x; dst[w + 1] = v.y; dst[w + 2] = v.z;
        } else {
            u32 x = v.x;
            if constexpr (C::kRem == 1) asm("" : "+v"(x) : "v"(v.y), "v"(v.z));
            if constexpr (C::kRem == 2) asm("" : "+v"(x) : "v"(v.z));
            dst[w] = x;
            if constexpr (C::kRem == 2) dst[w + 1] = v.y;
        }
    }
}

template <int NW, int CHUNK_ROW_BYTES>
__device__ __forceinline__ void lds_read_words(u32 (&dst)[NW], const unsigned char* p) {
#pragma unroll
    for (int c = 0; c < Chunks<NW>::kCount; c++) lds_read_chunk<NW, CHUNK_ROW_BYTES>(dst, p, c);
}

#ifndef SWK_WAVES3_MAX_R
#define SWK_WAVES3_MAX_R 36
#endif
#ifndef SWK_WAVES3_MAX_R_MULTI
#define SWK_WAVES3_MAX_R_MULTI 32
#endif
#ifndef SWK_WAVES4_MAX_R
#define SWK_WAVES4_MAX_R 22
#endif
#ifndef SWK_CLASSES_PACKED
#define SWK_CLASSES_PACKED 8
#endif
#ifndef SWK_CLASSES_PACKED_SMALL
#define SWK_CLASSES_PACKED_SMALL 4
#endif
#ifndef SWK_CLASSES_SCALAR
#define SWK_CLASSES_SCALAR 4
#endif
constexpr int frame_classes(bool packed, int R, int lanes, bool multi, bool uniform = false) {
    (void)lanes;
    const int want = packed ? ((R > SWK_WAVES3_MAX_R || (multi && R >= 25 && (uniform || R > SWK_WAVES3_MAX_R_MULTI))) ? SWK_CLASSES_PACKED : SWK_CLASSES_PACKED_SMALL)
                            : SWK_CLASSES_SCALAR;
    int P = want;
    while (P > 1 && 2 * P > R) P--;
    return P;
}

constexpr int kLookahead = 12;

template <int NW, int CHUNK_ROW_BYTES>
__device__ __forceinline__ void lds_read_chunk2(u32 (&da)[NW], u32 (&db)[NW], const unsigned char* pa, const unsigned char* pb, int c) {
    lds_read_chunk<NW, CHUNK_ROW_BYTES>(da, pa, c);
    lds_read_chunk<NW, CHUNK_ROW_BYTES>(db, pb, c);
    __builtin_amdgcn_sched_barrier(0);
}

template <int NW, int CHUNK_ROW_BYTES>
__device__ __forceinline__ void lds_read_words2(u32 (&da)[NW], u32 (&db)[NW], const unsigned char* pa, const unsigned char* pb) {
#pragma unroll
    for (int c = 0; c < Chunks<NW>::kCount; c++) lds_read_chunk2<NW, CHUNK_ROW_BYTES>(da, db, pa, pb, c);
}

template <int NW, int CHUNK_ROW_BYTES>
__device__ __forceinline__ void lds_read_chunk1(u32 (&da)[NW], const unsigned char* pa, int c) {
    lds_read_chunk<NW, CHUNK_ROW_BYTES>(da, pa, c);
    __builtin_amdgcn_sched_barrier(0);
}

template <int KIND, int R, int P = 1>
struct StripeState {
    u32 H[R];
    u32 E[R];
    u32 upH_prev;
    u32 Hlast;
    u32 Fout;
    u32 yA, yB;
    u32 maxv[P + 3];
    u32 Zc[P + 4];
};

template <int KIND, int R, int LANES, int BYTE, bool MULTI, bool OFFS = false, int P = 1, bool ZFILL = true, bool UNI = false, bool ADDR = false>
__device__ __forceinline__ void dp_step(StripeState<KIND, R, P>& st, const unsigned char* tile,
                                        u32 lettersA, u32 lettersB, u32 gop, u32 gex, u32 inH, u32 inF,
                                        u32 apos = 0, bool first = false, u32 wrapP = 0, u32 wrapLast = 0, bool head = false,
                                        u32 laneStep = 0, const u32* zw = nullptr) {
    using A = Arith<KIND>;
    using G = Geometry<KIND, R, LANES>;
    const u32 step2 = LANES < 16 ? laneStep : 0x00100010u;
    const u32 step1 = LANES < 16 ? laneStep : 16u;
    constexpr u32 kSel = 0x0c0c000cu | ((u32)BYTE << 8);
    constexpr int kPostShift = G::kLetterShift - 8;

    static_assert(!A::kPacked || OFFS, "packed kinds run the column-offset recurrence only");
    u32 wa[G::NW];
    u32 wb[G::NW];
    static_assert(!ADDR || (A::kPacked && LANES == 16 && OFFS), "the address stream serves the packed kinds on 16-lane groups");
    if constexpr (ADDR) {
    } else if constexpr (A::kPacked && LANES <= 16) {
        constexpr u32 kSel2 = ((u32)(4 + BYTE) << 24) | 0x000c000cu | ((u32)BYTE << 8);
        const u32 inj = __builtin_amdgcn_perm(lettersB, lettersA, kSel2);
        st.yA = prev_lane<LANES, false>(inj, st.yA, head) + step2;
    } else {
        const u32 injA = __builtin_amdgcn_perm(0u, lettersA, kSel) << kPostShift;
        st.yA = prev_lane<LANES, false>(injA, st.yA, head) + step1;
        if constexpr (A::kPacked || !OFFS) lds_read_words<G::NW, G::kChunkRowBytes>(wa, tile + st.yA);
        if constexpr (A::kPacked) {
            const u32 injB = __builtin_amdgcn_perm(0u, lettersB, kSel) << kPostShift;
            st.yB = prev_lane<LANES, false>(injB, st.yB, head) + step1;
            lds_read_words<G::NW, G::kChunkRowBytes>(wb, tile + st.yB);
        }
    }

    if constexpr (OFFS) {
        constexpr int kLastClass = (R - 1) % P;
        constexpr int Q = A::kWindow ? BYTE : 0;
        u32 upH, F;
        if constexpr (MULTI) {
            (void)first;
            upH = prev_lane<LANES, false>(inH, st.Hlast, head);
            F = prev_lane<LANES, false>(inF, st.Fout, head);
        } else {
            const u32 bH = UNI ? zw[Q + kLastClass] : st.Zc[Q + kLastClass];
            upH = prev_lane<LANES, false>(bH, st.Hlast, head);
            if constexpr (ZFILL) F = prev_lane<LANES, true>(0u, st.Fout, head);
            else F = prev_lane<LANES, false>(st.Zc[Q], st.Fout, head);
        }
        u32 diag = st.upH_prev;
        st.upH_prev = upH;
        u32 m[P];
#pragma unroll
        for (int c = 0; c < P; c++) m[c] = A::kWindow ? st.maxv[Q + c] : A::add(st.maxv[c], apos);
        auto score = [&](int r) -> u32 {
            if constexpr (G::kWide) return 0u;
            else if constexpr (A::kPacked) return __builtin_amdgcn_perm(wb[r >> 1], wa[r >> 1], (r & 1) ? 0x07060302u : 0x05040100u);
            else return wa[r];
        };
        auto diag_term = [&](int, u32 d, u32 sc) -> u32 { return A::add(d, sc); };
        constexpr int kAhead = G::kWide ? (kLookahead < R ? kLookahead : R) : 1;
        using CH = Chunks<G::NW>;
        constexpr int kChunksAll = CH::kCount;
        constexpr int kChunks0 = G::kWide ? CH::lead_for(kAhead, 4) : 1;
        static_assert(!G::kWide || kChunks0 >= kChunksAll || CH::lead_ok(kChunks0, kAhead, 4), "a score word would be used before its read is issued");
        const unsigned char* const pa = ADDR ? tile + 16 + __builtin_amdgcn_perm(lettersA, laneStep, 0x0c0c0500u) : tile + (st.yA & 0xffffu);
        const unsigned char* const pb = ADDR ? tile + 16 + __builtin_amdgcn_perm(lettersA, laneStep, 0x0c0c0700u) : tile + (st.yA >> 16);
        u32 tq[G::kWide ? R : 1];
        if constexpr (G::kWide) {
#pragma unroll
            for (int k = 0; k < kChunks0 && k < kChunksAll; k++) lds_read_chunk2<G::NW, G::kChunkRowBytes>(wa, wb, pa, pb, k);
#pragma unroll
            for (int r = 0; r < kAhead; r++) tq[r] = A::add_pair(wa[r], wb[r], r == 0 ? diag : st.H[r - 1]);
        }
        constexpr bool kProg1 = !A::kPacked;
        constexpr int kChunks0S = kProg1 ? CH::lead_for(2, 6) : 1;
        if constexpr (kProg1) {
#pragma unroll
            for (int k = 0; k < kChunks0S && k < kChunksAll; k++) lds_read_chunk1<G::NW, G::kChunkRowBytes>(wa, tile + st.yA, k);
        }
        u32 s_next = score(0);
        u32 t_next = G::kWide ? 0u : diag_term(0, diag, s_next);
        s_next = R > 1 ? score(1) : 0u;
#pragma unroll
        for (int r = 0; r < R; r++) {
            const int c = r % P;
            const u32 zop = UNI ? zw[Q + c + 2] : st.Zc[Q + c + 1];
            if constexpr (G::kWide) {
                if (r % 4 == 0) __builtin_amdgcn_sched_barrier(0);
                if (CH::starts_chunk(r) && CH::chunk_of(r) + kChunks0 < kChunksAll)
                    lds_read_chunk2<G::NW, G::kChunkRowBytes>(wa, wb, pa, pb, CH::chunk_of(r) + kChunks0);
                t_next = tq[r];
            }
            if constexpr (kProg1) {
                if (r % 4 == 0) __builtin_amdgcn_sched_barrier(0);
                if (CH::starts_chunk(r) && CH::chunk_of(r) + kChunks0S < kChunksAll)
                    lds_read_chunk1<G::NW, G::kChunkRowBytes>(wa, tile + st.yA, CH::chunk_of(r) + kChunks0S);
            }
            const u32 t = t_next;
            const u32 h = A::cell_h(t, st.E[r], F);
            const u32 s1 = s_next;
            if (r + 2 < R) s_next = score(r + 2);
            const u32 hg = A::gap(h, gop);
            if constexpr (G::kWide) {
                if (r + kAhead < R) tq[r + kAhead] = A::add_pair(wa[r + kAhead], wb[r + kAhead], st.H[r + kAhead - 1]);
            } else {
                if (r + 1 < R) t_next = diag_term(r + 1, st.H[r], s1);
            }
            const u32 fm = A::max3(F, hg, zop);
            st.E[r] = A::max3(st.E[r], hg, zop);
            if (r == R - 1) F = (UNI && kLastClass == 0) ? fm : A::gap(fm, wrapLast);
            else if (c == P - 1) F = A::gap(fm, wrapP);
            else F = fm;
            if ((r / P) & 1) m[c] = A::fold2(m[c], st.H[r - P], h);
            else if (r + P >= R) m[c] = A::max2(m[c], h);
            st.H[r] = h;
        }
#pragma unroll
        for (int c = 0; c < P; c++) st.maxv[Q + c] = m[c];
        if constexpr (!A::kWindow) {
#pragma unroll
            for (int k = (kLastClass == 0 ? 0 : 1); k <= P; k++) st.Zc[k] = A::add(st.Zc[k], apos);
        }
        st.Hlast = st.H[R - 1];
        st.Fout = F;
    } else {
        u32 upH, F;
        if constexpr (MULTI) {
            upH = prev_lane<LANES, false>(inH, st.Hlast, head);
            F = prev_lane<LANES, false>(inF, st.Fout, head);
        } else {
            upH = prev_lane<LANES, true>(0u, st.Hlast, head);
            F = prev_lane<LANES, true>(0u, st.Fout, head);
        }
        u32 diag = st.upH_prev;
        st.upH_prev = upH;

        u32 maxv = st.maxv[0];
#pragma unroll
        for (int r = 0; r < R; r++) {
            const u32 t = A::add(diag, wa[r]);
            diag = st.H[r];
            const u32 h = A::cell_h(t, st.E[r], F);
            const u32 hg = A::gap(h, gop);
            st.E[r] = A::gap_state(A::gap(st.E[r], gex), hg);
            F = A::gap_state(A::gap(F, gex), hg);
            st.H[r] = h;
            if (r & 1) maxv = A::fold2(maxv, st.H[r - 1], h);
            else if (r == R - 1) maxv = A::max2(maxv, h);
        }
        st.maxv[0] = maxv;
        st.Hlast = st.H[R - 1];
        st.Fout = F;
    }
}

template <int TILE_BYTES>
__device__ __forceinline__ void load_tile(unsigned char* lds, const unsigned char* gsrc) {
    static_assert(TILE_BYTES % 16 == 0, "tile must be 16-byte granular");
    const uint4* src = reinterpret_cast<const uint4*>(gsrc);
    uint4* dst = reinterpret_cast<uint4*>(lds + 16);
    for (int i = threadIdx.x; i < TILE_BYTES / 16; i += kThreads) dst[i] = src[i];
}

template <class MAX>
__device__ __forceinline__ u32 half_row_max(u32 v, MAX&& mx) {
    v = mx(v, dpp<0x141, false>(v, v));
    v = mx(v, dpp<0xB1, false>(v, v));
    v = mx(v, dpp<0x4E, false>(v, v));
    return v;
}

template <class MAX>
__device__ __forceinline__ u32 quad_max(u32 v, MAX&& mx) {
    v = mx(v, dpp<0xB1, false>(v, v));
    v = mx(v, dpp<0x4E, false>(v, v));
    return v;
}

template <int KIND>
__device__ __forceinline__ u32 row_max_true(u32 v) {
    using A = Arith<KIND>;
    v = A::true_max(v, dpp<0x128, false>(v, v));
    v = A::true_max(v, dpp<0x124, false>(v, v));
    v = A::true_max(v, dpp<0x122, false>(v, v));
    v = A::true_max(v, dpp<0x121, false>(v, v));
    return v;
}

template <int KIND, int LANES>
__device__ __forceinline__ u32 group_max(u32 v) {
    using A = Arith<KIND>;
    if constexpr (LANES == 8) return half_row_max(v, [](u32 a, u32 b) { return A::max2(a, b); });
    if constexpr (LANES == 4) return quad_max(v, [](u32 a, u32 b) { return A::max2(a, b); });
    v = row_max_true<KIND>(v);
    if constexpr (LANES == 64) {
        v = A::max2(v, (u32)__shfl_xor((int)v, 16));
        v = A::max2(v, (u32)__shfl_xor((int)v, 32));
    }
    return v;
}

template <int LANES>
struct Border {
    static constexpr int kBlockCols = 2 * LANES;
    static constexpr int kQuadsPerBlock = LANES / 2;
    static constexpr int kBlockBytes = 8 * kBlockCols;
    static constexpr int kBlockWords = 2 * kBlockCols;
    static constexpr int kInBytes = kBlockBytes, kOutBytes = kBlockBytes, kDummyBytes = 8 * (kThreads / LANES) + 32;
    static constexpr int kGroupBytes = kInBytes + kOutBytes + 16;
    static constexpr int ring_bytes(int groups) { return groups * kGroupBytes + kDummyBytes; }
    static_assert(kGroupBytes % 16 == 0, "rings are read and written 16 bytes at a time");
    static constexpr int blocks(int steps) { return (steps + kBlockCols - 1) / kBlockCols + 3; }
};
template <int LANES>
constexpr int border_region_words(int lcap) { return Border<LANES>::blocks(lcap) * Border<LANES>::kBlockWords; }

template <int LANES>
constexpr int stream_region_words(int lcap) { return LANES == 16 ? Border<LANES>::blocks(lcap) * Border<LANES>::kBlockCols : 0; }
template <int LANES>
constexpr int group_region_words(int lcap) { return border_region_words<LANES>(lcap) + stream_region_words<LANES>(lcap); }

constexpr int kChainMax = 8;
constexpr int kChainMinCols = 12;
constexpr int kChainMaxWords = (kChainMax - 1) * kGroup;
constexpr int chain_pair_columns(int lmax) { return ((lmax + 3) & ~3) < kChainMinCols ? kChainMinCols : ((lmax + 3) & ~3); }
constexpr int64_t chain_columns(int max_len, int c) { return (int64_t)(c - 1) * (chain_pair_columns(max_len) + 4) + max_len; }

__device__ __forceinline__ void announce_start(const ScanParams& p) {
    if (p.start_signal && threadIdx.x == 0) {
        if (atomicAdd(p.work_counter + 1, 1u) + 1u == p.start_quorum)
            __hip_atomic_fetch_add(p.start_signal, 1u, __ATOMIC_RELEASE, __HIP_MEMORY_SCOPE_SYSTEM);
    }
}

#ifndef SWK_I32_WAVES3_MAX_R
#define SWK_I32_WAVES3_MAX_R 32
#endif
#ifndef SWK_I32_WAVES3_MAX_R_MULTI
#define SWK_I32_WAVES3_MAX_R_MULTI 32
#endif
#ifndef SWK_F32_WAVES3_MAX_R
#define SWK_F32_WAVES3_MAX_R 48
#endif
#ifndef SWK_F32_WAVES3_MAX_R_MULTI
#define SWK_F32_WAVES3_MAX_R_MULTI 48
#endif
constexpr int min_waves_of(int KIND, int R, int LANES, bool MULTI) {
    const bool packed = KIND == F16X2 || KIND == I16X2;
    if (packed && LANES <= 16 && MULTI && R <= SWK_WAVES3_MAX_R_MULTI) return 3;
    if (packed) return (LANES <= 16 && !MULTI && R <= SWK_WAVES4_MAX_R) ? 4 : (LANES <= 16 && !MULTI && R <= SWK_WAVES3_MAX_R) ? 3 : 2;
    if (KIND == I32 && LANES <= 16 && R > (MULTI ? SWK_I32_WAVES3_MAX_R_MULTI : SWK_I32_WAVES3_MAX_R)) return 2;
    if (KIND == F32 && LANES <= 16 && R > (MULTI ? SWK_F32_WAVES3_MAX_R_MULTI : SWK_F32_WAVES3_MAX_R)) return 2;
    return (R <= 16 && !MULTI && LANES <= 16) ? 4 : 3;
}
template <int KIND, int R, int LANES, bool MULTI>
constexpr int min_waves() { return min_waves_of(KIND, R, LANES, MULTI); }
constexpr int vgpr_slot_of(int KIND, int R, int LANES, bool MULTI) { return (512 / min_waves_of(KIND, R, LANES, MULTI)) & ~7; }

template <int KIND, int R, int LANES, bool MULTI, bool OFFS = false>
__global__ void __launch_bounds__(kThreads, (min_waves<KIND, R, LANES, MULTI>())) sw_scan_kernel(const ScanParams p) {
    using A = Arith<KIND>;
    using G = Geometry<KIND, R, LANES>;
    constexpr int kGroups = kThreads / LANES;
    using BD = Border<LANES>;
    constexpr int SHL1 = Shift<LANES>::kShl1;
    constexpr int kQuadsPerLetterBlock = LANES;
    static_assert(!A::kPacked || OFFS, "packed kinds run the column-offset recurrence only (sw_launch.hpp: launch_scan_ro)");
    constexpr bool kUni = A::kPacked;
    constexpr bool kAddr = A::kPacked && MULTI && LANES == 16;
    constexpr bool kChain = kAddr;
    constexpr int P = OFFS ? frame_classes(A::kPacked, R, LANES, MULTI, kUni) : 1;
    __shared__ __attribute__((aligned(16))) unsigned char lds[16 + G::kTileBytes];
    __shared__ int chainEnd[kChain ? (kThreads / 64) * kChainMax : 1];
    __shared__ __attribute__((aligned(16))) unsigned char rings[MULTI ? BD::ring_bytes(kGroups) : 16];

    const int tid = threadIdx.x;
    const int lane = tid & (LANES - 1);
    const int group = tid / LANES;
    const bool head = lane == 0;
    const int slot = LANES < 16 ? (tid & 15) : lane;
    const u32 laneStep = kAddr ? 16u * (u32)slot : (A::kPacked ? 0x00100010u : 16u) * ((LANES < 16 && head) ? u32(slot + 1) : 1u);
    announce_start(p);
    if (p.positions) __builtin_amdgcn_s_setprio(2);
    const bool service = p.service != 0;
    const int n = (p.count_ptr && !service) ? *p.count_ptr : p.n;
    constexpr int kSubjPerBatch = kGroups * A::kSubjects;
    const int nbatches = (n + kSubjPerBatch - 1) / kSubjPerBatch;
    if (!service && (int)blockIdx.x >= nbatches) return;
    const int kC = kChain ? min(max(p.chain, 1), kChainMax) : 1;
    const int nchain = (!kChain || kC == 1) ? 0 : p.chain_all ? (nbatches + kC - 1) / kC : max(0, (nbatches - kC * (int)gridDim.x + kC - 1) / kC);
    const int nclaims = kChain ? nchain + max(0, nbatches - nchain * kC) : nbatches;

    if constexpr (!MULTI) {
        load_tile<G::kTileBytes>(lds, p.profile);
        __syncthreads();
    }

    unsigned char* const ringIn = rings + (MULTI ? group * BD::kGroupBytes : 0);
    unsigned char* const ringOut = ringIn + BD::kInBytes;
    u32* const gBorder = MULTI ? p.scratch + ((size_t)blockIdx.x * kGroups + group) * (size_t)group_region_words<LANES>(p.lcap) : nullptr;
    typedef const __attribute__((address_space(1))) unsigned char* StreamPtr;
    StreamPtr streamBase = nullptr;
    u32 streamOff = 0;
    if constexpr (kAddr) {
        constexpr int kGroupsPerWave = 64 / LANES;
        const int g0 = group & ~(kGroupsPerWave - 1);
        const uintptr_t b = reinterpret_cast<uintptr_t>(p.scratch + ((size_t)blockIdx.x * kGroups + g0) * (size_t)group_region_words<LANES>(p.lcap) +
                                                        border_region_words<LANES>(p.lcap));
        streamBase = (StreamPtr)(((uintptr_t)(u32)__builtin_amdgcn_readfirstlane((int)(b >> 32)) << 32) |
                                 (uintptr_t)(u32)__builtin_amdgcn_readfirstlane((int)(u32)b));
        streamOff = 4u * (u32)((group - g0) * group_region_words<LANES>(p.lcap) + LANES - lane);
    }

    const u32 apos = OFFS ? A::pos_word(p.gex_mag) : 0u;
    const u32 apos4 = OFFS ? A::pos_word(4 * p.gex_mag) : 0u;
    const int rq = kUni ? p.renorm_quads : 0;
    const int kmask = 4 * rq - 1;
    const u32 zstart = (OFFS && !kUni) ? A::zero_at(p.gex_mag, LANES - lane) : A::kZero;
    const u32 zbefore = (OFFS && !kUni) ? A::zero_at(p.gex_mag, LANES - lane - 1) : A::kZero;

    __shared__ int next_batch, batch_avail;
    auto claim_entry = [&](int i) -> int {
        for (int spin = 0; spin < (1 << 20); spin++) {
            const int v = __hip_atomic_load(p.claim + i, __ATOMIC_RELAXED, __HIP_MEMORY_SCOPE_AGENT);
            if (v == kListTaken) return -1;
            if (v >= 0) return atomicCAS(p.claim + i, v, kListTaken) == v ? v : -1;
            __builtin_amdgcn_s_sleep(2);
        }
        return -1;
    };
    for (;;) {
        __syncthreads();
        if (tid == 0) {
            int b = (int)atomicAdd(p.work_counter, 1u), avail = n;
            if (service) {
                avail = 0;
                for (u32 spin = 0; b < nbatches; spin++) {
                    avail = __hip_atomic_load(p.count_ptr, __ATOMIC_RELAXED, __HIP_MEMORY_SCOPE_AGENT);
                    if (avail > b * kSubjPerBatch) break;
                    const u32 done = __hip_atomic_load(p.done_flag, __ATOMIC_RELAXED, __HIP_MEMORY_SCOPE_SYSTEM);
                    if ((int32_t)(done - p.done_value) >= 0 || spin > 600000u) { b = nbatches; break; }
                    __builtin_amdgcn_s_sleep(127);
                }
                avail = min(avail, n);
            }
            if (b == nclaims && p.dry_signal) __hip_atomic_store(p.dry_signal, p.dry_value, __ATOMIC_RELAXED, __HIP_MEMORY_SCOPE_SYSTEM);
            next_batch = b;
            batch_avail = avail;
        }
        __syncthreads();
        const int b = next_batch;
        if (b >= nclaims) break;
        const int navail = batch_avail;
        int hb = b, cnt = 1;
        if constexpr (kChain) {
            if (b < nchain) { hb = kC * b; cnt = min(kC, nbatches - hb); }
            else hb = nchain * kC + (b - nchain);
            hb = __builtin_amdgcn_readfirstlane(hb);
            cnt = __builtin_amdgcn_readfirstlane(cnt);
        }
        struct Pair {
            bool valid0 = false, valid1 = false;
            int pos0 = 0, pos1 = 0, len0 = 0, len1 = 0, lmax = 0;
            const int8_t* s0 = nullptr;
            const int8_t* s1 = nullptr;
        };
        auto load_pair = [&](int hbk) -> Pair {
            Pair r;
            const int batch = service ? hbk : nbatches - 1 - hbk;
            const int i0 = batch * kSubjPerBatch + group * A::kSubjects;
            const int i1 = i0 + 1;
            r.valid0 = i0 < navail;
            r.valid1 = A::kPacked && (i1 < navail);
            r.s0 = p.chars;
            r.s1 = p.chars;
            if (p.claim) {
                int v = -1;
                if (r.valid0 && lane == 0) v = claim_entry(i0);
                if constexpr (LANES == 64) v = __builtin_amdgcn_readfirstlane(v);
                else v = __shfl(v, (tid & 63) & ~(LANES - 1));
                r.valid0 = v >= 0;
                r.pos0 = r.valid0 ? v : 0;
                if (r.valid0) {
                    r.len0 = p.lengths[r.pos0];
                    r.s0 = p.chars + (p.offsets[r.pos0] - p.offsets[0]);
                }
                r.valid1 = false;
            } else {
                if (r.valid0) {
                    r.pos0 = p.positions ? p.positions[i0] : p.first_pos + i0;
                    r.len0 = p.lengths[r.pos0];
                    r.s0 = p.chars + (p.offsets[r.pos0] - p.offsets[0]);
                }
                if (r.valid1) {
                    r.pos1 = p.positions ? p.positions[i1] : p.first_pos + i1;
                    r.len1 = p.lengths[r.pos1];
                    r.s1 = p.chars + (p.offsets[r.pos1] - p.offsets[0]);
                }
            }
            int lmax = r.len0 > r.len1 ? r.len0 : r.len1;
            if constexpr (LANES <= 16) {
                if constexpr (LANES <= 4) lmax = max(lmax, __shfl_xor(lmax, 4));
                if constexpr (LANES <= 8) lmax = max(lmax, __shfl_xor(lmax, 8));
                lmax = max(lmax, __shfl_xor(lmax, 16));
                lmax = max(lmax, __shfl_xor(lmax, 32));
            }
            r.lmax = lmax;
            return r;
        };
        Pair pr;
        if constexpr (!kChain) pr = load_pair(hb);
        const bool valid0 = pr.valid0, valid1 = pr.valid1;
        const int pos0 = pr.pos0, pos1 = pr.pos1, len0 = pr.len0, len1 = pr.len1;
        const int8_t* const s0 = pr.s0;
        const int8_t* const s1 = pr.s1;
        int nquads = (pr.lmax + LANES - 1 + 3) >> 2;
        if constexpr (MULTI) nquads = min(nquads, (p.lcap - 4) >> 2);
        nquads = __builtin_amdgcn_readfirstlane(nquads);
        const int len0pad = (len0 + 3) & ~3, len1pad = (len1 + 3) & ~3;
        auto letters4 = [&](const int8_t* s, int lenpad, int j) -> u32 {
            u32 w = 0x14141414u;
            if (j < lenpad) w = *reinterpret_cast<const u32*>(s + j);
            return w * (u32)G::kLetterUnits;
        };
        if constexpr (kAddr) {
            u32* const sw = gBorder + border_region_words<LANES>(p.lcap) + LANES;
            const int wcap = 4 * ((p.lcap - 4) >> 2) + LANES;
            sw[lane - LANES] = (u32)(kPadLetter * G::kLetterUnits) * 0x01000100u;
            auto put4 = [&](const Pair& q, int col0, int c) {
                if (col0 + 4 * c + 4 > wcap) return;
                const u32 a = letters4(q.s0, (q.len0 + 3) & ~3, 4 * c), b = letters4(q.s1, (q.len1 + 3) & ~3, 4 * c);
                *reinterpret_cast<uint4*>(sw + col0 + 4 * c) = make_uint4(__builtin_amdgcn_perm(b, a, 0x040c000cu), __builtin_amdgcn_perm(b, a, 0x050c010cu),
                                                                          __builtin_amdgcn_perm(b, a, 0x060c020cu), __builtin_amdgcn_perm(b, a, 0x070c030cu));
            };
            int col0 = 0;
            for (int k = 0; k + 1 < cnt; k++) {
                const Pair q = load_pair(hb + k);
                const int T = chain_pair_columns(__builtin_amdgcn_readfirstlane(q.lmax));
                for (int c = lane; c < T / 4 + 1; c += LANES) put4(q, col0, c);
                if ((tid & 63) == 0) chainEnd[(tid >> 6) * kChainMax + k] = col0 + T;
                col0 += T + 4;
            }
            const Pair q = load_pair(hb + cnt - 1);
            nquads = (col0 + __builtin_amdgcn_readfirstlane(q.lmax) + LANES - 1 + 3) >> 2;
            nquads = __builtin_amdgcn_readfirstlane(min(nquads, (p.lcap - 4) >> 2));
            for (int c = lane; c < nquads - col0 / 4 + LANES / 4; c += LANES) put4(q, col0, c);
            __builtin_amdgcn_fence(__ATOMIC_RELEASE, "workgroup");
        }

        u32 maxv = 0u;
        for (int stripe = 0; stripe < p.nstripes; stripe++) {
            const bool first = stripe == 0;
            if constexpr (MULTI) {
                __syncthreads();
                load_tile<G::kTileBytes>(lds, p.profile + (size_t)stripe * G::kTileBytes);
                __syncthreads();
            }
            StripeState<KIND, R, P> st;
            u32 zw[P + 5];
            const int tg0 = kUni ? __builtin_amdgcn_readfirstlane(LANES * stripe) : 0;
            auto load_levels = [&](int q) {
                const int u0 = __builtin_amdgcn_readfirstlane((tg0 + 4 * q) & kmask);
#pragma unroll
                for (int k = 0; k < P + 5; k++) zw[k] = p.levels[u0 + k];
#pragma unroll
                for (int k = 0; k < P + 5; k++) asm volatile("" : "+s"(zw[k]));
            };
            if constexpr (kUni) {
                load_levels(0);
#pragma unroll
                for (int r = 0; r < R; r++) { st.H[r] = zw[r % P]; st.E[r] = zw[r % P + 1]; }
                st.upH_prev = A::gap(zw[(R - 1) % P], p.gex); st.Hlast = zw[(R - 1) % P]; st.Fout = zw[0];
                const u32 seed = (kChain && cnt > 1) ? 0u : maxv;
#pragma unroll
                for (int d = 0; d < P + 3; d++) st.maxv[d] = A::add(seed, zw[d + 1]);
            } else {
                u32 zc[P + 5];
                zc[0] = zbefore; zc[1] = zstart;
#pragma unroll
                for (int k = 2; k < P + 5; k++) zc[k] = A::add(zc[k - 1], apos);
#pragma unroll
                for (int r = 0; r < R; r++) { st.H[r] = zc[r % P]; st.E[r] = zc[r % P + 1]; }
                st.upH_prev = zc[(R - 1) % P]; st.Hlast = zc[(R - 1) % P]; st.Fout = zbefore;
#pragma unroll
                for (int k = 0; k < P + 4; k++) st.Zc[k] = zc[k + 1];
#pragma unroll
                for (int d = 0; d < P + 3; d++) st.maxv[d] = OFFS ? A::add(maxv, zc[A::kWindow ? d + 1 : d]) : maxv;
            }
            st.yA = ((u32)(kPadLetter * G::kLetterUnits) << G::kLetterShift) + 16u * (u32)(slot + 1);
            st.yB = st.yA;
            if constexpr (A::kPacked && LANES <= 16) st.yA |= st.yA << 16;

            auto fetch = [&](const int8_t* s, int lenpad, int blk) -> u32 {
                if constexpr (kAddr) return 0u;
                else return letters4(s, lenpad, blk * (4 * LANES) + lane * 4);
            };
            u32 nextA = fetch(s0, len0pad, 0);
            u32 nextB = A::kPacked ? fetch(s1, len1pad, 0) : 0u;
            u32 lettersA = 0, lettersB = 0;
            StreamPtr streamAt = streamBase;
            auto stream_word = [&](int k) -> u32 { return ((const __attribute__((address_space(1))) u32*)(streamAt + (size_t)streamOff))[k]; };
            u32 nxtW = 0;

            const bool last = stripe + 1 == p.nstripes;
            const unsigned char* inPtr = ringIn;
            unsigned char* outPtr = (lane == LANES - 1) ? ringOut : rings + kGroups * BD::kGroupBytes + 8 * group;
            const u32 walkIn = 32u;
            const u32 walkOut = (lane == LANES - 1) ? 32u : 0u;
            uint4 pend = make_uint4(A::kZero, A::kZero, A::kZero, A::kZero);
            uint2 nxt = make_uint2(A::kZero, A::kZero);
            const u32* const gIn = MULTI ? gBorder + 2 * (LANES - 1) + 4 * lane : nullptr;
            auto first_stripe_pairs = [&](int j) -> uint4 {
                if constexpr (kUni) {
                    constexpr int kLastClass = (R - 1) % P;
                    return make_uint4(A::zero_at(p.gex_mag, (j & kmask) + kLastClass), A::kZero, A::zero_at(p.gex_mag, ((j + 1) & kmask) + kLastClass), A::kZero);
                } else if constexpr (OFFS) {
                    constexpr int kLastClass = (R - 1) % P;
                    const int K = 4 * rq;
                    const int j0 = K > 0 ? (j & (K - 1)) : j, j1 = K > 0 ? ((j + 1) & (K - 1)) : j + 1;
                    return make_uint4(A::zero_at(p.gex_mag, j0 + LANES + kLastClass), A::kZero, A::zero_at(p.gex_mag, j1 + LANES + kLastClass), A::kZero);
                } else {
                    return make_uint4(A::kZero, A::kZero, A::kZero, A::kZero);
                }
            };
            if constexpr (MULTI) {
                __builtin_amdgcn_fence(__ATOMIC_ACQUIRE, "workgroup");
                if (!first) {
                    const uint4 b0 = *reinterpret_cast<const uint4*>(gIn);
                    pend = *reinterpret_cast<const uint4*>(gIn + BD::kBlockWords);
                    *reinterpret_cast<uint4*>(ringIn + 16 * lane) = b0;
                } else {
                    *reinterpret_cast<uint4*>(ringIn + 16 * lane) = first_stripe_pairs(2 * lane);
                }
                __builtin_amdgcn_fence(__ATOMIC_RELEASE, "wavefront");
                nxt = *reinterpret_cast<const uint2*>(inPtr);
                if constexpr (kAddr) nxtW = stream_word(0);
            }
            auto block_end = [&](int blk) {
                int t = tid;
                asm volatile("" : "+v"(t));
                const int ln = t & (LANES - 1), grp = t / LANES;
                unsigned char* const rIn = rings + grp * BD::kGroupBytes + 16 * ln;
                u32* const gb = p.scratch + ((size_t)blockIdx.x * kGroups + grp) * (size_t)group_region_words<LANES>(p.lcap) + 4 * ln;
                __builtin_amdgcn_fence(__ATOMIC_ACQ_REL, "wavefront");
                if (!last) {
                    const uint4 v = *reinterpret_cast<const uint4*>(rIn + BD::kInBytes);
                    *reinterpret_cast<uint4*>(gb + (size_t)blk * BD::kBlockWords) = v;
                }
                outPtr -= walkOut * BD::kQuadsPerBlock;
                inPtr -= walkIn * BD::kQuadsPerBlock;
                if (first) {
                    *reinterpret_cast<uint4*>(rIn) = first_stripe_pairs((blk + 1) * BD::kBlockCols + 2 * ln);
                } else {
                    *reinterpret_cast<uint4*>(rIn) = pend;
                    pend = *reinterpret_cast<const uint4*>(gb + 2 * (LANES - 1) + (size_t)(blk + 2) * BD::kBlockWords);
                }
                __builtin_amdgcn_fence(__ATOMIC_ACQ_REL, "wavefront");
                nxt = *reinterpret_cast<const uint2*>(inPtr);
            };

            auto lower_frame = [&]() {
                if constexpr (kUni) {
                    const u32 w = p.renorm_word;
#pragma unroll
                    for (int r = 0; r < R; r++) { st.H[r] = A::lower(st.H[r], w); st.E[r] = A::lower(st.E[r], w); }
                    st.upH_prev = A::lower(st.upH_prev, w);
                    if constexpr (KIND == I16X2) st.upH_prev = A::true_max(st.upH_prev, A::gap(A::kZero, p.gex));
                    st.Hlast = A::lower(st.Hlast, w);
                    st.Fout = A::lower(st.Fout, w);
#pragma unroll
                    for (int d = 0; d < P + 3; d++) st.maxv[d] = A::lower(st.maxv[d], w);
                }
            };
            auto quad = [&](int q) {
                if (!kAddr && (q & (kQuadsPerLetterBlock - 1)) == 0) {
                    lettersA = nextA; lettersB = nextB;
                    nextA = fetch(s0, len0pad, q / kQuadsPerLetterBlock + 1);
                    if constexpr (A::kPacked) nextB = fetch(s1, len1pad, q / kQuadsPerLetterBlock + 1);
                }
                const bool lower = kUni && ((tg0 + 4 * q + 4) & kmask) == 0;
                auto border_step = [&](auto byte_tag) {
                    constexpr int BYTE = decltype(byte_tag)::value;
                    const uint2 in = nxt;
                    if constexpr (MULTI) {
                        if constexpr (BYTE == 3) {
                            inPtr += walkIn;
                            nxt = *reinterpret_cast<const uint2*>(inPtr);
                        } else {
                            nxt = *reinterpret_cast<const uint2*>(inPtr + 8 * (BYTE + 1));
                        }
                    }
                    if constexpr (kAddr) {
                        lettersA = nxtW;
                        if constexpr (BYTE == 3) {
                            streamAt += 16;
                            nxtW = stream_word(0);
                        } else {
                            nxtW = stream_word(BYTE + 1);
                        }
                    }
                    dp_step<KIND, R, LANES, BYTE, MULTI, OFFS, P, true, kUni, kAddr>(st, lds, lettersA, lettersB, p.gop, p.gex, in.x, in.y, apos, first,
                                                                                 p.wrap_class, p.wrap_last, head, laneStep, zw);
                    if constexpr (kUni && BYTE == 3) {
                        if (lower) lower_frame();
                    }
                    if constexpr (MULTI) *reinterpret_cast<uint2*>(outPtr + 8 * BYTE) = make_uint2(st.Hlast, st.Fout);
                };
                border_step(std::integral_constant<int, 0>{});
                border_step(std::integral_constant<int, 1>{});
                border_step(std::integral_constant<int, 2>{});
                border_step(std::integral_constant<int, 3>{});
                if constexpr (MULTI) outPtr += walkOut;
                if constexpr (!kAddr) {
                    lettersA = dpp<SHL1, true>(0u, lettersA);
                    if constexpr (A::kPacked) lettersB = dpp<SHL1, true>(0u, lettersB);
                }
                if constexpr (OFFS && A::kWindow) {
                    if constexpr (!kUni) {
#pragma unroll
                        for (int k = 0; k < P + 4; k++) st.Zc[k] = A::add(st.Zc[k], apos4);
                    }
#pragma unroll
                    for (int d = 0; d < P + 3; d++) st.maxv[d] = A::add(st.maxv[d], apos4);
                }
                if constexpr (kUni) load_levels(q + 1);
            };
            auto reset_lanes = [&](int k, int j) {
                if constexpr (kChain) {
                    int t = tid;
                    asm volatile("" : "+v"(t));
                    const int ln = t & (LANES - 1), grp = t / LANES;
                    if ((ln >> 2) == j) {
                        u32 m = A::true_of(st.maxv[0], zw[1]);
#pragma unroll
                        for (int d = 1; d < P + 3; d++) m = A::true_max(m, A::true_of(st.maxv[d], zw[d + 1]));
                        u32* const pm = p.scratch + (size_t)gridDim.x * kGroups * (size_t)group_region_words<LANES>(p.lcap) +
                                        ((size_t)blockIdx.x * kGroups + grp) * kChainMaxWords + kGroup * k + ln;
                        if (!first) m = A::true_max(m, *pm);
                        *pm = m;
#pragma unroll
                        for (int d = 0; d < P + 3; d++) st.maxv[d] = zw[d + 1];
#pragma unroll
                        for (int r = 0; r < R; r++) { st.H[r] = zw[r % P]; st.E[r] = zw[r % P + 1]; }
                        st.upH_prev = A::gap(zw[(R - 1) % P], p.gex); st.Hlast = zw[(R - 1) % P]; st.Fout = zw[0];
                    }
                }
            };
            if constexpr (!MULTI) {
                for (int q = 0; q < nquads; q++) quad(q);
            } else if constexpr (kChain) {
                constexpr int kNever = 0x7fffffff;
                const int* const ends = chainEnd + (tid >> 6) * kChainMax;
                int rk = 0, rj = 0;
                int nextReset = cnt > 1 ? __builtin_amdgcn_readfirstlane((ends[0] >> 2) + 1) : kNever;
                for (int q0 = 0; q0 < nquads; q0 += BD::kQuadsPerBlock) {
                    const int qend = min(nquads, q0 + BD::kQuadsPerBlock);
                    int q = q0;
                    for (;;) {
                        const int seg = min(qend, nextReset);
                        for (; q < seg; q++) quad(q);
                        if (q >= qend) break;
                        reset_lanes(rk, rj);
                        nextReset++;
                        if (++rj == 4) {
                            rj = 0;
                            rk++;
                            nextReset = rk + 1 < cnt ? __builtin_amdgcn_readfirstlane((ends[rk] >> 2) + 1) : kNever;
                        }
                    }
                    if (qend == q0 + BD::kQuadsPerBlock) block_end(q0 / BD::kQuadsPerBlock);
                }
            } else {
                for (int q0 = 0; q0 < nquads; q0 += BD::kQuadsPerBlock) {
                    const int qend = min(nquads, q0 + BD::kQuadsPerBlock);
                    for (int q = q0; q < qend; q++) quad(q);
                    if (qend == q0 + BD::kQuadsPerBlock) block_end(q0 / BD::kQuadsPerBlock);
                }
            }
            if constexpr (MULTI) {
                if (!last) {
                    const int done = nquads & ~(BD::kQuadsPerBlock - 1);
                    const int slot = 4 * (nquads - done) + lane;
                    u32* const g = gBorder + (size_t)(done / BD::kQuadsPerBlock) * BD::kBlockWords;
                    __builtin_amdgcn_fence(__ATOMIC_ACQ_REL, "wavefront");
                    if (slot < BD::kBlockCols) *reinterpret_cast<uint2*>(ringOut + 8 * slot) = make_uint2(A::kZero, A::kZero);
                    else *reinterpret_cast<uint2*>(g + 2 * slot) = make_uint2(A::kZero, A::kZero);
                    __builtin_amdgcn_fence(__ATOMIC_ACQ_REL, "wavefront");
                    *reinterpret_cast<uint4*>(g + 4 * lane) = *reinterpret_cast<const uint4*>(ringOut + 16 * lane);
                }
            }
            if constexpr (kUni) {
                const u32 above = maxv;
                maxv = A::true_of(st.maxv[0], zw[1]);
#pragma unroll
                for (int d = 1; d < P + 3; d++) maxv = A::true_max(maxv, A::true_of(st.maxv[d], zw[d + 1]));
                if constexpr (kChain) {
                    if (cnt > 1) maxv = A::true_max(maxv, above);
                }
            } else if constexpr (OFFS) {
                if constexpr (A::kWindow) {
                    maxv = A::true_of(st.maxv[0], st.Zc[0]);
#pragma unroll
                    for (int d = 1; d < P + 3; d++) maxv = A::true_max(maxv, A::true_of(st.maxv[d], st.Zc[d]));
                } else {
                    maxv = A::true_of(st.maxv[0], A::gap(A::gap(st.Zc[1], p.gex), p.gex));
#pragma unroll
                    for (int c = 1; c < P; c++)
                        maxv = A::true_max(maxv, A::true_of(st.maxv[c], A::gap(A::gap(st.Zc[c + 1], p.gex), p.gex)));
                }
            } else {
                maxv = st.maxv[0];
            }
            if constexpr (MULTI) __builtin_amdgcn_fence(__ATOMIC_RELEASE, "workgroup");
        }

        auto finish = [&](bool valid0, bool valid1, int pos0, int pos1, u32 maxv, int nq, int col0) {
            int sc0, sc1, guard = 0;
            if constexpr (OFFS) {
                if constexpr (LANES == 8) {
                    maxv = half_row_max(maxv, [](u32 a, u32 b) { return A::true_max(a, b); });
                } else if constexpr (LANES == 4) {
                    maxv = quad_max(maxv, [](u32 a, u32 b) { return A::true_max(a, b); });
                } else {
                    maxv = row_max_true<KIND>(maxv);
                }
                if constexpr (LANES == 64) {
                    maxv = A::true_max(maxv, (u32)__shfl_xor((int)maxv, 16));
                    maxv = A::true_max(maxv, (u32)__shfl_xor((int)maxv, 32));
                }
                sc0 = A::true_lo(maxv);
                sc1 = A::true_hi(maxv);
                if constexpr (kUni) {
                    const int tgmax = 4 * nq + col0 + LANES * (p.nstripes - 1);
                    constexpr int kColP = frame_classes(true, R, LANES, MULTI);
                    guard = max(p.gex_mag * ((tgmax > 4 * rq ? 4 * rq : tgmax) + P + 8),
                                p.gex_mag * (min(4 * nq, p.flag_period) + 2 * LANES + 4 + kColP));
                } else {
                    guard = p.gex_mag * (4 * nq + 2 * LANES + 4 + P);
                }
            } else {
                maxv = group_max<KIND, LANES>(maxv);
                sc0 = A::score_lo(maxv);
                sc1 = 0;
            }
            if (lane == 0) {
                if (valid0) {
                    if (A::kPacked && p.ovf_check && sc0 >= A::kLimit - guard) {
                        __hip_atomic_store(p.ovf_pos + atomicAdd(p.ovf_count, 1), pos0, __ATOMIC_RELAXED, __HIP_MEMORY_SCOPE_AGENT);
                    } else {
                        p.scores[pos0] = (float)sc0;
                        if (p.stat_count && sc0 >= p.stat_limit) atomicAdd(p.stat_count, 1);
                    }
                    p.ids[pos0] = (int32_t)(p.id_offset + pos0);
                }
                if (valid1) {
                    if (p.ovf_check && sc1 >= A::kLimit - guard) {
                        __hip_atomic_store(p.ovf_pos + atomicAdd(p.ovf_count, 1), pos1, __ATOMIC_RELAXED, __HIP_MEMORY_SCOPE_AGENT);
                    } else {
                        p.scores[pos1] = (float)sc1;
                    }
                    p.ids[pos1] = (int32_t)(p.id_offset + pos1);
                }
            }
        };
        if constexpr (kChain) {
            int col0 = 0;
            for (int k = 0; k < cnt; k++) {
                const Pair q = load_pair(hb + k);
                const int lm = __builtin_amdgcn_readfirstlane(q.lmax);
                const bool lastPair = k + 1 == cnt;
                int t = tid;
                asm volatile("" : "+v"(t));
                const u32* const pm = p.scratch + (size_t)gridDim.x * kGroups * (size_t)group_region_words<LANES>(p.lcap) +
                                      ((size_t)blockIdx.x * kGroups + t / LANES) * kChainMaxWords + kGroup * k + (t & (LANES - 1));
                u32 m = maxv;
                if (!lastPair) m = *pm;
                finish(q.valid0, q.valid1, q.pos0, q.pos1, m, lastPair ? nquads - col0 / 4 : (lm + LANES - 1 + 3) >> 2, col0);
                col0 += chain_pair_columns(lm) + 4;
            }
        } else {
            finish(valid0, valid1, pos0, pos1, maxv, nquads, 0);
        }
    }
}

template <int KIND, int R, int LANES>
__global__ void sw_build_profile_kernel(const int8_t* __restrict__ query, int32_t qlen,
                                        const int8_t* __restrict__ matrix21, int32_t pad_row, int32_t nstripes,
                                        unsigned char* __restrict__ profile, int32_t shift, int32_t head_extra) {
    using A = Arith<KIND>;
    using G = Geometry<KIND, R, LANES>;
    constexpr int kWordsPerRow = G::kRowBytes / 4;
    constexpr int kWordsPerChunkRow = G::kChunkRowBytes / 4;
    const size_t total = (size_t)nstripes * kLetters * kWordsPerRow;
    u32* out = reinterpret_cast<u32*>(profile);
    for (size_t i = (size_t)blockIdx.x * blockDim.x + threadIdx.x; i < total; i += (size_t)gridDim.x * blockDim.x) {
        const int word = (int)(i % kWordsPerRow);
        const int letter = (int)((i / kWordsPerRow) % kLetters);
        const int stripe = (int)(i / ((size_t)kWordsPerRow * kLetters));
        const int chunk = word / kWordsPerChunkRow, lane = ((word % kWordsPerChunkRow) / 4) % LANES, sub = word % 4;
        const int w = G::C::first(chunk) + sub;
        u32 v = 0;
        if (sub < G::C::words(chunk) && w < G::NW) {
            auto entry = [&](int row_in_lane) -> u32 {
                if (row_in_lane >= R) return 0u;
                const int64_t row = (int64_t)stripe * G::kStripeRows + lane * R + row_in_lane;
                const bool pssm = query == nullptr;
                const int qc = row < qlen ? (pssm ? (int)row : (int)query[row]) : pad_row;
                const int score = pssm ? (int)matrix21[pssm_index(qc, letter)] : (int)matrix21[qc * kLetters + letter];
                const int P = frame_classes(A::kPacked, R, LANES, nstripes > 1, head_extra != 0);
                const int cls = row_in_lane % P, above = (row_in_lane == 0 ? R - 1 : row_in_lane - 1) % P;
                const int head = row_in_lane == 0 ? head_extra : 0;
                return A::encode_score(score + shift * (1 + head + cls - above));
            };
            if constexpr (G::kWide) v = w < R ? (entry(w) | (A::kOne << 16)) : 0u;
            else if constexpr (A::kPacked) v = entry(2 * w) | (entry(2 * w + 1) << 16);
            else v = entry(w);
        }
        out[i] = v;
    }
}

}
```

### cudasw4_amd/csrc/sw_kind_f16x2.hip

```cpp
#include "sw_launch.hpp"

namespace swk {
#define SWK_CASE_SCAN16_F16X2(R) case R: return launch_scan_r<F16X2, R, 16>(multi, offs, grid, reserve, stream, p);
#define SWK_CASE_SCAN64_F16X2(R) case R: return launch_scan_r<F16X2, R, 64>(multi, offs, grid, reserve, stream, p);
#define SWK_CASE_PROF16_F16X2(R) case R: return launch_profile_r<F16X2, R, 16>(q, qlen, m, pr, ns, out, shift, hx, s);
#define SWK_CASE_PROF64_F16X2(R) case R: return launch_profile_r<F16X2, R, 64>(q, qlen, m, pr, ns, out, shift, hx, s);
#define SWK_CASE_TILE16_F16X2(R) case R: return tile_bytes_r<F16X2, R, 16>();
#define SWK_CASE_TILE64_F16X2(R) case R: return tile_bytes_r<F16X2, R, 64>();
#define SWK_CASE_SCAN8_F16X2(R) case R: return launch_scan_r<F16X2, R, 8>(multi, offs, grid, reserve, stream, p);
#define SWK_CASE_PROF8_F16X2(R) case R: return launch_profile_r<F16X2, R, 8>(q, qlen, m, pr, ns, out, shift, hx, s);
#define SWK_CASE_TILE8_F16X2(R) case R: return tile_bytes_r<F16X2, R, 8>();
#define SWK_CASE_SCAN4_F16X2(R) case R: return launch_scan_r<F16X2, R, 4>(multi, offs, grid, reserve, stream, p);
#define SWK_CASE_PROF4_F16X2(R) case R: return launch_profile_r<F16X2, R, 4>(q, qlen, m, pr, ns, out, shift, hx, s);
#define SWK_CASE_TILE4_F16X2(R) case R: return tile_bytes_r<F16X2, R, 4>();
SWK_DEFINE_KIND(launch_f16x2, F16X2, SWK_FOR_EACH_R_PACKED)
}
```

### cudasw4_amd/csrc/sw_kind_f32.hip

```cpp
#include "sw_launch.hpp"

namespace swk {
#define SWK_CASE_SCAN16_F32(R) case R: return launch_scan_r<F32, R, 16>(multi, offs, grid, reserve, stream, p);
#define SWK_CASE_SCAN64_F32(R) case R: return launch_scan_r<F32, R, 64>(multi, offs, grid, reserve, stream, p);
#define SWK_CASE_PROF16_F32(R) case R: return launch_profile_r<F32, R, 16>(q, qlen, m, pr, ns, out, shift, hx, s);
#define SWK_CASE_PROF64_F32(R) case R: return launch_profile_r<F32, R, 64>(q, qlen, m, pr, ns, out, shift, hx, s);
#define SWK_CASE_TILE16_F32(R) case R: return tile_bytes_r<F32, R, 16>();
#define SWK_CASE_TILE64_F32(R) case R: return tile_bytes_r<F32, R, 64>();
#define SWK_CASE_SCAN8_F32(R) case R: return launch_scan_r<F32, R, 8>(multi, offs, grid, reserve, stream, p);
#define SWK_CASE_PROF8_F32(R) case R: return launch_profile_r<F32, R, 8>(q, qlen, m, pr, ns, out, shift, hx, s);
#define SWK_CASE_TILE8_F32(R) case R: return tile_bytes_r<F32, R, 8>();
#define SWK_CASE_SCAN4_F32(R) case R: return launch_scan_r<F32, R, 4>(multi, offs, grid, reserve, stream, p);
#define SWK_CASE_PROF4_F32(R) case R: return launch_profile_r<F32, R, 4>(q, qlen, m, pr, ns, out, shift, hx, s);
#define SWK_CASE_TILE4_F32(R) case R: return tile_bytes_r<F32, R, 4>();
SWK_DEFINE_KIND(launch_f32, F32, SWK_FOR_EACH_R_I32)
}
```

### cudasw4_amd/csrc/sw_kind_i16x2.hip

```cpp
#include "sw_launch.hpp"

namespace swk {
#define SWK_CASE_SCAN16_I16X2(R) case R: return launch_scan_r<I16X2, R, 16>(multi, offs, grid, reserve, stream, p);
#define SWK_CASE_SCAN64_I16X2(R) case R: return launch_scan_r<I16X2, R, 64>(multi, offs, grid, reserve, stream, p);
#define SWK_CASE_PROF16_I16X2(R) case R: return launch_profile_r<I16X2, R, 16>(q, qlen, m, pr, ns, out, shift, hx, s);
#define SWK_CASE_PROF64_I16X2(R) case R: return launch_profile_r<I16X2, R, 64>(q, qlen, m, pr, ns, out, shift, hx, s);
#define SWK_CASE_TILE16_I16X2(R) case R: return tile_bytes_r<I16X2, R, 16>();
#define SWK_CASE_TILE64_I16X2(R) case R: return tile_bytes_r<I16X2, R, 64>();
#define SWK_CASE_SCAN8_I16X2(R) case R: return launch_scan_r<I16X2, R, 8>(multi, offs, grid, reserve, stream, p);
#define SWK_CASE_PROF8_I16X2(R) case R: return launch_profile_r<I16X2, R, 8>(q, qlen, m, pr, ns, out, shift, hx, s);
#define SWK_CASE_TILE8_I16X2(R) case R: return tile_bytes_r<I16X2, R, 8>();
#define SWK_CASE_SCAN4_I16X2(R) case R: return launch_scan_r<I16X2, R, 4>(multi, offs, grid, reserve, stream, p);
#define SWK_CASE_PROF4_I16X2(R) case R: return launch_profile_r<I16X2, R, 4>(q, qlen, m, pr, ns, out, shift, hx, s);
#define SWK_CASE_TILE4_I16X2(R) case R: return tile_bytes_r<I16X2, R, 4>();
SWK_DEFINE_KIND(launch_i16x2, I16X2, SWK_FOR_EACH_R_PACKED)
}
```

### cudasw4_amd/csrc/sw_kind_i32.hip

```cpp
#include "sw_launch.hpp"

namespace swk {
#define SWK_CASE_SCAN16_I32(R) case R: return launch_scan_r<I32, R, 16>(multi, offs, grid, reserve, stream, p);
#define SWK_CASE_SCAN64_I32(R) case R: return launch_scan_r<I32, R, 64>(multi, offs, grid, reserve, stream, p);
#define SWK_CASE_PROF16_I32(R) case R: return launch_profile_r<I32, R, 16>(q, qlen, m, pr, ns, out, shift, hx, s);
#define SWK_CASE_PROF64_I32(R) case R: return launch_profile_r<I32, R, 64>(q, qlen, m, pr, ns, out, shift, hx, s);
#define SWK_CASE_TILE16_I32(R) case R: return tile_bytes_r<I32, R, 16>();
#define SWK_CASE_TILE64_I32(R) case R: return tile_bytes_r<I32, R, 64>();
#define SWK_CASE_SCAN8_I32(R) case R: return launch_scan_r<I32, R, 8>(multi, offs, grid, reserve, stream, p);
#define SWK_CASE_PROF8_I32(R) case R: return launch_profile_r<I32, R, 8>(q, qlen, m, pr, ns, out, shift, hx, s);
#define SWK_CASE_TILE8_I32(R) case R: return tile_bytes_r<I32, R, 8>();
#define SWK_CASE_SCAN4_I32(R) case R: return launch_scan_r<I32, R, 4>(multi, offs, grid, reserve, stream, p);
#define SWK_CASE_PROF4_I32(R) case R: return launch_profile_r<I32, R, 4>(q, qlen, m, pr, ns, out, shift, hx, s);
#define SWK_CASE_TILE4_I32(R) case R: return tile_bytes_r<I32, R, 4>();
SWK_DEFINE_KIND(launch_i32, I32, SWK_FOR_EACH_R_I32)
}
```

### cudasw4_amd/csrc/sw_launch.hpp

```cpp
#pragma once
#include <hip/hip_runtime.h>

#include <algorithm>
#include <atomic>

#include "sw_dp_kernel.hpp"
#include "sw_stream_kernel.hpp"

namespace swk {

constexpr int kRowsGranule = 1;
#ifndef SWK_MAX_ROWS_PACKED
#define SWK_MAX_ROWS_PACKED 48
#endif
constexpr int kMaxRowsPacked = SWK_MAX_ROWS_PACKED;
#ifndef SWK_MAX_ROWS_SCALAR
#define SWK_MAX_ROWS_SCALAR 36
#endif
constexpr int kMaxRowsScalar = SWK_MAX_ROWS_SCALAR;
#ifndef SWK_MAX_ROWS_SCALAR_MULTI
#define SWK_MAX_ROWS_SCALAR_MULTI 32
#endif
constexpr int kMaxRowsScalarMulti = SWK_MAX_ROWS_SCALAR_MULTI;
#ifndef SWK_MAX_ROWS_I32
#define SWK_MAX_ROWS_I32 48
#endif
constexpr int kMaxRowsI32 = SWK_MAX_ROWS_I32;
constexpr int kWaves3MaxRowsPackedMulti = SWK_WAVES3_MAX_R_MULTI;
constexpr int kMaxRowsPackedLong = 16;
constexpr int kMaxRowsScalarLong = 8;
constexpr int kMaxRowsShortGroups = 32;
constexpr int max_rows(int kind, int lanes) {
    const bool packed = kind == F16X2 || kind == I16X2;
    if (lanes < 16) return kMaxRowsShortGroups;
    return lanes == 16 ? (packed ? kMaxRowsPacked : kind == I32 ? kMaxRowsI32 : kMaxRowsScalar) : (packed ? kMaxRowsPackedLong : kMaxRowsScalarLong);
}

struct KindLaunch {
    hipError_t (*scan)(int R, int lanes, bool multi, bool offs, int grid, int reserve, hipStream_t stream, const ScanParams& p);
    hipError_t (*profile)(int R, int lanes, const int8_t* query, int32_t qlen, const int8_t* matrix21, int32_t pad_row,
                          int32_t nstripes, unsigned char* out, int32_t shift, int32_t head_extra, hipStream_t stream);
    size_t (*tile_bytes)(int R, int lanes);
    hipError_t (*warm)(hipStream_t stream);
    bool packed;
};

const KindLaunch& launch_f16x2();
const KindLaunch& launch_i16x2();
const KindLaunch& launch_i32();
const KindLaunch& launch_f32();

template <class K>
int resident_workgroups(K kernel) {
    static std::atomic<int> cached[64];
    int dev = 0;
    if (hipGetDevice(&dev) != hipSuccess || dev < 0 || dev >= 64) return 0;
    int v = cached[dev].load(std::memory_order_relaxed);
    if (v == 0) {
        int per_cu = 0, cus = 0;
        if (hipOccupancyMaxActiveBlocksPerMultiprocessor(&per_cu, kernel, kThreads, 0) != hipSuccess ||
            hipDeviceGetAttribute(&cus, hipDeviceAttributeMultiprocessorCount, dev) != hipSuccess || per_cu <= 0 || cus <= 0) {
            (void)hipGetLastError();
            v = -1;
        } else {
            v = per_cu * cus;
        }
        cached[dev].store(v, std::memory_order_relaxed);
    }
    return v > 0 ? v : 0;
}

template <class K>
hipError_t launch_scan_k(K kernel, int grid, int reserve, hipStream_t stream, const ScanParams& p) {
    if (reserve > 0) {
        const int resident = resident_workgroups(kernel);
        if (resident > 0 && grid > resident - reserve) {
            ScanParams q = p;
            grid = resident - reserve > 1 ? resident - reserve : 1;
            if (q.start_quorum > (u32)grid) q.start_quorum = (u32)grid;
            hipLaunchKernelGGL(kernel, dim3(grid), dim3(kThreads), 0, stream, q);
            return hipGetLastError();
        }
    }
    hipLaunchKernelGGL(kernel, dim3(grid), dim3(kThreads), 0, stream, p);
    return hipGetLastError();
}

constexpr bool uniform_frame_launch(bool packed, bool offs, int lanes, bool multi, int stream_slots) {
    return packed && offs && !(lanes == 16 && (!multi || stream_slots > 1));
}

template <int KIND, int R, int LANES, bool OFFS>
hipError_t launch_scan_ro(bool multi, int grid, int reserve, hipStream_t stream, const ScanParams& p) {
    constexpr int kMaxR = max_rows(KIND, LANES);
    constexpr bool kPacked = Arith<KIND>::kPacked;
    if constexpr (R > kMaxR || (kPacked && !OFFS)) {
        return hipErrorInvalidValue;
    } else if ((p.uniform_frame != 0) != uniform_frame_launch(kPacked, OFFS, LANES, multi, p.stream_slots) ||
               (p.uniform_frame && (p.renorm_quads < LANES || 4 * p.renorm_quads > kUniformMaxPeriod))) {
        return hipErrorInvalidValue;
    } else if constexpr (kPacked && LANES == 16) {
        if (p.positions || p.claim || p.service || p.count_ptr || p.stream_slots < 1) return hipErrorInvalidValue;
        if (multi) {
            if constexpr (2 * R > kMaxR) {
                if (p.stream_slots > 1) return launch_scan_k(sw_scan_stream_kernel<KIND, R, LANES, true>, grid, reserve, stream, p);
                return launch_scan_k(sw_scan_kernel<KIND, R, LANES, true, OFFS>, grid, reserve, stream, p);
            } else {
                return hipErrorInvalidValue;
            }
        } else {
            return launch_scan_k(sw_scan_stream_kernel<KIND, R, LANES, false>, grid, reserve, stream, p);
        }
    } else {
        if (multi) {
            if constexpr (2 * R > kMaxR && LANES >= 16) {
                return launch_scan_k(sw_scan_kernel<KIND, R, LANES, true, OFFS>, grid, reserve, stream, p);
            } else {
                return hipErrorInvalidValue;
            }
        } else {
            return launch_scan_k(sw_scan_kernel<KIND, R, LANES, false, OFFS>, grid, reserve, stream, p);
        }
    }
}

template <int KIND, int R, int LANES>
hipError_t launch_scan_r(bool multi, bool offs, int grid, int reserve, hipStream_t stream, const ScanParams& p) {
    return offs ? launch_scan_ro<KIND, R, LANES, true>(multi, grid, reserve, stream, p)
                : launch_scan_ro<KIND, R, LANES, false>(multi, grid, reserve, stream, p);
}

template <int KIND, int R, int LANES>
hipError_t launch_profile_r(const int8_t* query, int32_t qlen, const int8_t* matrix21, int32_t pad_row, int32_t nstripes,
                            unsigned char* out, int32_t shift, int32_t head_extra, hipStream_t stream) {
    if constexpr (R > max_rows(KIND, LANES)) {
        return hipErrorInvalidValue;
    } else {
        const size_t total = (size_t)nstripes * kLetters * (Geometry<KIND, R, LANES>::kRowBytes / 4);
        const int grid = (int)std::min<size_t>((total + 255) / 256, 65536);
        hipLaunchKernelGGL((sw_build_profile_kernel<KIND, R, LANES>), dim3(grid), dim3(256), 0, stream, query, qlen,
                           matrix21, pad_row, nstripes, out, shift, head_extra);
        return hipGetLastError();
    }
}

template <int KIND, int R, int LANES>
constexpr size_t tile_bytes_r() {
    if constexpr (R > max_rows(KIND, LANES)) return 0;
    else return (size_t)Geometry<KIND, R, LANES>::kTileBytes;
}

#define SWK_FOR_EACH_R_PACKED(X) \
    X(1) X(2) X(3) X(4) X(5) X(6) X(7) X(8) X(9) X(10) X(11) X(12) X(13) X(14) X(15) X(16) X(17) X(18) X(19) X(20) X(21) X(22) X(23) X(24) X(25) X(26) X(27) X(28) X(29) X(30) X(31) X(32) X(33) X(34) X(35) X(36) X(37) X(38) X(39) X(40) X(41) X(42) X(43) X(44) X(45) X(46) X(47) X(48)
#define SWK_FOR_EACH_R_I32(X) SWK_FOR_EACH_R_PACKED(X)
#define SWK_FOR_EACH_R_SCALAR(X) \
    X(1) X(2) X(3) X(4) X(5) X(6) X(7) X(8) X(9) X(10) X(11) X(12) X(13) X(14) X(15) X(16) X(17) X(18) X(19) X(20) X(21) X(22) X(23) X(24) X(25) X(26) X(27) X(28) X(29) X(30) X(31) X(32)

#define SWK_DEFINE_KIND(FN, KIND, FOR_EACH_R)                                                                      \
    static hipError_t FN##_scan(int R, int lanes, bool multi, bool offs, int grid, int reserve, hipStream_t stream, \
                                const ScanParams& p) {                                                              \
        if (lanes == 16) { switch (R) { FOR_EACH_R(SWK_CASE_SCAN16_##KIND) } }                                      \
        else if (lanes == 64) { switch (R) { FOR_EACH_R(SWK_CASE_SCAN64_##KIND) } }                                 \
        else if (lanes == 8) { switch (R) { FOR_EACH_R(SWK_CASE_SCAN8_##KIND) } }                                   \
        else if (lanes == 4) { switch (R) { FOR_EACH_R(SWK_CASE_SCAN4_##KIND) } }                                   \
        return hipErrorInvalidValue;                                                                                \
    }                                                                                                               \
    static hipError_t FN##_profile(int R, int lanes, const int8_t* q, int32_t qlen, const int8_t* m, int32_t pr,    \
                                   int32_t ns, unsigned char* out, int32_t shift, int32_t hx, hipStream_t s) {      \
        if (lanes == 16) { switch (R) { FOR_EACH_R(SWK_CASE_PROF16_##KIND) } }                                      \
        else if (lanes == 64) { switch (R) { FOR_EACH_R(SWK_CASE_PROF64_##KIND) } }                                 \
        else if (lanes == 8) { switch (R) { FOR_EACH_R(SWK_CASE_PROF8_##KIND) } }                                   \
        else if (lanes == 4) { switch (R) { FOR_EACH_R(SWK_CASE_PROF4_##KIND) } }                                   \
        return hipErrorInvalidValue;                                                                                \
    }                                                                                                               \
    static size_t FN##_tile_bytes(int R, int lanes) {                                                               \
        if (lanes == 16) { switch (R) { FOR_EACH_R(SWK_CASE_TILE16_##KIND) } }                                      \
        else if (lanes == 64) { switch (R) { FOR_EACH_R(SWK_CASE_TILE64_##KIND) } }                                 \
        else if (lanes == 8) { switch (R) { FOR_EACH_R(SWK_CASE_TILE8_##KIND) } }                                   \
        else if (lanes == 4) { switch (R) { FOR_EACH_R(SWK_CASE_TILE4_##KIND) } }                                   \
        return 0;                                                                                                   \
    }                                                                                                               \
    static __global__ void FN##_warm_kernel() {}                                                                    \
    static hipError_t FN##_warm(hipStream_t s) {                                                                    \
        hipLaunchKernelGGL(FN##_warm_kernel, dim3(1), dim3(64), 0, s);                                              \
        return hipGetLastError();                                                                                   \
    }                                                                                                               \
    const KindLaunch& FN() {                                                                                        \
        static const KindLaunch k{FN##_scan, FN##_profile, FN##_tile_bytes, FN##_warm, Arith<KIND>::kPacked};       \
        return k;                                                                                                   \
    }

}
```

### cudasw4_amd/csrc/sw_plan.hpp

```cpp
#pragma once
#include <cstddef>
#include <cstdint>

namespace swp {

struct PlanSettings {
    int num_cus = 0;
    int grid_mult = 4;
    int grid_cap = 0;
    int32_t qlen = 0;
    bool have_query = false;
    int score_max = 1;
    bool use_offs = true;
    bool i32_native = false;
    int32_t lanes4_max_subject = -1;
    int32_t lanes4_max_q = -1;
    int32_t lanes8_max_q = -1;
    int64_t long16_min = -1;
    int32_t stream_slots = 4;
    int32_t stream_jump = 0;
    int32_t stream_cols_max = 4096;
    int32_t stream_multi_cols_max = 1536;
    int32_t stream_multi_max_subject = -1;
    int32_t chain = 3;
    bool chain_all = false;
};
void settings_from_env(PlanSettings& s);

constexpr size_t kUnlimitedScratch = ~(size_t)0;

struct LaunchRequest {
    int kind = 0;
    int part_id = -1;
    int32_t n = 0;
    int32_t max_subject_len = 0;
    bool gaps_known = false;
    int gop = 0, gex = 0;
    bool ovf_list = false;
    bool claim = false;
    int service_workgroups = 0;
    size_t scratch = kUnlimitedScratch;
};

struct LaunchPlan {
    bool valid = false;
    int kind = 0;
    bool fell_back = false;
    int lanes = 16, rows = 0, nstripes = 0;
    bool multi = false;
    bool offs = false;
    int frame = 0;
    int64_t period = 0;
    int64_t flag_period = 0;
    int stream_slots = 0, stream_cols = 0, stream_room = 0, stream_base = 0, stream_jump = 0;
    int chain = 1;
    int32_t lcap = 0;
    int64_t nbatches = 0;
    int grid = 0;
    size_t bytes_per_wg = 0;
    size_t scratch_needed = 0;
    bool scratch_too_small = false;
    int vgpr_slot = 0;
};

LaunchPlan plan_launch(const PlanSettings& s, const LaunchRequest& req);

}
```

### include/cudasw4_amd_engine.h

```cpp
#ifndef CUDASW4_AMD_ENGINE_H
#define CUDASW4_AMD_ENGINE_H

#include "cudasw4_amd.h"

#ifdef __cplusplus
extern "C" {
#endif

size_t sw_rescore_service_temp_bytes(sw_ctx* ctx, int kind, int32_t max_subject_len, int workgroups);
int sw_rescore_service(sw_ctx* ctx, int kind, int32_t* ovf_pos, const int32_t* ovf_count, int32_t max_count,
                       const int8_t* chars, const uint64_t* offsets, const int32_t* lengths, int32_t max_subject_len,
                       int gop, int gex, float* scores, int32_t* ids, int64_t id_offset, void* temp, size_t temp_bytes,
                       int32_t packed_limit, int32_t* true_overflow_count, const uint32_t* done_flag, uint32_t done_value,
                       int workgroups, void* stream);
int sw_rescore_overflow_claim(sw_ctx* ctx, int kind, int32_t* ovf_pos, const int32_t* ovf_count, int32_t max_count,
                              const int8_t* chars, const uint64_t* offsets, const int32_t* lengths, int32_t max_subject_len,
                              int gop, int gex, float* scores, int32_t* ids, int64_t id_offset, void* temp, size_t temp_bytes,
                              int32_t packed_limit, int32_t* true_overflow_count, void* stream);

int sw_set_start_signal(sw_ctx* ctx, uint32_t* signal);

int sw_probe_handshake(sw_ctx* ctx, void* side_stream, void* gated_stream, uint32_t* signal);

size_t sw_rescore_overflow_pipelined_temp_bytes(sw_ctx* ctx, int32_t max_subject_len);
int sw_rescore_overflow_pipelined(sw_ctx* ctx, int32_t* ovf_pos, const int32_t* ovf_count, int32_t max_count, const int8_t* chars,
                                  const uint64_t* offsets, const int32_t* lengths, int32_t max_subject_len,
                                  int32_t min_subject_len, int gop, int gex, float* scores, int32_t* ids, int64_t id_offset,
                                  int32_t* fail_count, int32_t packed_limit, int32_t* true_overflow_count, void* temp,
                                  size_t temp_bytes, void* stream);

int sw_launch_vgpr_slot(sw_ctx* ctx, int kind, int part_id, int32_t n, int32_t max_subject_len);
int sw_set_rows_pipeline_slot(sw_ctx* ctx, int vgprs);
size_t sw_scan_rows_pipelined_temp_bytes(sw_ctx* ctx, int32_t n, int32_t max_subject_len);
int sw_scan_rows_pipelined(sw_ctx* ctx, const int8_t* chars, const uint64_t* offsets, const int32_t* lengths,
                           int32_t first_pos, int32_t n, int32_t max_subject_len, int gop, int gex, float* scores,
                           int32_t* ids, int64_t id_offset, int32_t* fail_count, int32_t* over_limit_count,
                           int32_t* over_limit_count2, int32_t packed_limit, void* temp, size_t temp_bytes, void* stream);

int sw_set_long16_min(sw_ctx* ctx, int32_t subjects);

int sw_set_dry_signal(sw_ctx* ctx, uint32_t* signal, uint32_t value);
int sw_set_dirty_counter(sw_ctx* ctx, int32_t* counter);
int sw_set_grid_reserve(sw_ctx* ctx, int32_t workgroups);

int32_t sw_window_overlap(sw_ctx* ctx, int gop, int gex);
int sw_reduce_windows(sw_ctx* ctx, const float* win_scores, const int32_t* win_first, const int32_t* real_pos, int32_t n_real,
                      float* scores, int32_t* ids, int64_t id_offset, void* stream);

int sw_packed_launch_falls_back(sw_ctx* ctx, int kind, int part_id, int32_t n, int32_t max_subject_len, int gop, int gex);
int sw_scan_partition_counted(sw_ctx* ctx, int kind, int part_id, const int8_t* chars, const uint64_t* offsets,
                              const int32_t* lengths, int32_t first_pos, int32_t n, int32_t max_subject_len, int gop, int gex,
                              float* scores, int32_t* ids, int64_t id_offset, int32_t packed_limit, int32_t* over_limit_count,
                              int32_t* over_limit_total, void* temp, size_t temp_bytes, void* stream);

int sw_batch_describe_plan(sw_batch* b, const sw_batch_args* a, char* out, size_t cap);

#ifdef __cplusplus
}
#endif

#endif
```

Measured before the change: 12270 GCUPS.

## Use shorter stripes to trim padded query rows in multi-stripe packed kernel

Adds mixed-height stripes: when the query length leaves spare padded rows across stripes, the last few stripes use one row fewer per lane (R-1), so the kernel computes fewer padded cells. The profile builder, plan, and scan kernel learn a short_stripes count, with per-stripe row offsets, adjusted wrap words and border handling. Each stripe body is instantiated twice (R and R-1), which increases code size and may affect register allocation or instruction cache behavior.

Result: no change. 12300 GCUPS, median of 6 (+0.3%).

```diff
diff --git a/cudasw4_amd/capi.py b/cudasw4_amd/capi.py
--- a/cudasw4_amd/capi.py
+++ b/cudasw4_amd/capi.py
@@ -23,7 +23,7 @@
            "sw_window_overlap", "sw_reduce_windows", "sw_rescore_service", "sw_rescore_overflow_claim",
            "sw_rescore_service_temp_bytes", "sw_streams_run_concurrently", "sw_set_dry_signal", "sw_set_dirty_counter", "sw_set_grid_reserve",
            "sw_set_long16_min", "sw_scan_rows_pipelined",
-           "sw_scan_rows_pipelined_temp_bytes", "sw_probe_handshake", "sw_launch_vgpr_slot",
+           "sw_scan_rows_pipelined_temp_bytes", "sw_probe_handshake", "sw_launch_vgpr_slot", "sw_launch_short_stripes",
            "sw_set_rows_pipeline_slot", "sw_packed_launch_falls_back", "sw_scan_partition_counted", "sw_rescore_overflow_pipelined", "sw_rescore_overflow_pipelined_temp_bytes", "sw_measure_valu_rate",
            "sw_align_hits"]
 PSSM_EXPORTS = ["sw_set_query_pssm", "sw_query_is_pssm", "sw_align_hits_pssm", "sw_pssm_accumulate"]
@@ -133,6 +133,8 @@
     L.sw_reduce_windows.argtypes = [vp, vp, vp, vp, i32, vp, vp, ctypes.c_int64, vp]
     L.sw_plan_launch.argtypes = [vp, ctypes.c_int, ctypes.c_int, i32, i32, ctypes.POINTER(i32), ctypes.POINTER(i32),
                                  ctypes.POINTER(i32), ctypes.POINTER(i32)]
+    if hasattr(L, "sw_launch_short_stripes"):
+        L.sw_launch_short_stripes.argtypes = [vp, ctypes.c_int, ctypes.c_int, i32, i32]
     if hasattr(L, "sw_align_hits"):
         L.sw_align_hits.argtypes = [vp, ctypes.POINTER(_AlignArgs)]
     if hasattr(L, "sw_set_query_pssm"):
@@ -231,6 +233,9 @@
     def launch_vgpr_slot(self, kind, part_id, n, max_subject_len):
         return int(lib.sw_launch_vgpr_slot(self.handle, kind, part_id, n, max_subject_len))
 
+    def launch_short_stripes(self, kind, part_id, n, max_subject_len):
+        return int(lib.sw_launch_short_stripes(self.handle, kind, part_id, n, max_subject_len))
+
     def set_rows_pipeline_slot(self, vgprs):
         check(lib.sw_set_rows_pipeline_slot(self.handle, vgprs))
 
diff --git a/cudasw4_amd/csrc/sw_api.hip b/cudasw4_amd/csrc/sw_api.hip
--- a/cudasw4_amd/csrc/sw_api.hip
+++ b/cudasw4_amd/csrc/sw_api.hip
@@ -147,7 +147,7 @@
 
 int ensure_profile(sw_ctx* ctx, const LaunchPlan& lp, int shift, hipStream_t stream) {
     Profile& pr = ctx->profiles[lp.kind][shape_index(lp.lanes)][lp.frame];
-    if (pr.valid && (pr.shift != shift || pr.rows != lp.rows || pr.nstripes != lp.nstripes)) pr.valid = false;
+    if (pr.valid && (pr.shift != shift || pr.rows != lp.rows || pr.nstripes != lp.nstripes || pr.short_stripes != lp.short_stripes)) pr.valid = false;
     if (pr.valid) {
         SW_HIP(hipStreamWaitEvent(stream, pr.ready, 0));
         return SW_OK;
@@ -164,13 +164,14 @@
         SW_HIP(hipMalloc(&pr.dev, cap));
         pr.capacity = cap;
     }
-    if (ctx->pssm_mode) SW_HIP(kl->profile(lp.rows, lp.lanes, nullptr, qlen, ctx->d_pssm, qlen, lp.nstripes, pr.dev, shift, lp.frame == 2 ? 1 : 0, stream));
-    else SW_HIP(kl->profile(lp.rows, lp.lanes, ctx->d_query, qlen, ctx->d_matrix, ctx->dim, lp.nstripes, pr.dev, shift, lp.frame == 2 ? 1 : 0, stream));
+    if (ctx->pssm_mode) SW_HIP(kl->profile(lp.rows, lp.lanes, nullptr, qlen, ctx->d_pssm, qlen, lp.nstripes, pr.dev, shift, lp.frame == 2 ? 1 : 0, lp.short_stripes, stream));
+    else SW_HIP(kl->profile(lp.rows, lp.lanes, ctx->d_query, qlen, ctx->d_matrix, ctx->dim, lp.nstripes, pr.dev, shift, lp.frame == 2 ? 1 : 0, lp.short_stripes, stream));
     pr.shift = shift;
     if (!pr.ready) SW_HIP(hipEventCreateWithFlags(&pr.ready, hipEventDisableTiming));
     SW_HIP(hipEventRecord(pr.ready, stream));
     pr.rows = lp.rows;
     pr.nstripes = lp.nstripes;
+    pr.short_stripes = lp.short_stripes;
     pr.valid = true;
     return SW_OK;
 }
@@ -290,6 +291,8 @@
     lp.stream_slots = sp.slots; lp.stream_cols = sp.cols; lp.stream_room = sp.room; lp.stream_base = sp.base; lp.stream_jump = sp.jump;
     const bool uniform = swk::uniform_frame_launch(kind_packed(kind), lp.offs, lanes, lp.multi, sp.slots);
     lp.frame = lp.offs ? (uniform ? 2 : 1) : 0;
+    const bool scan16 = req.gaps_known ? uniform : swk::uniform_frame_launch(kind_packed(kind), s.use_offs, lanes, lp.multi, sp.slots);
+    if (scan16 && swk::mixed_stripes_kernel(kind_packed(kind), pl.rows, lanes, lp.multi)) lp.short_stripes = short_stripes_of(s.qlen, lanes, pl.rows, pl.nstripes);
     if (lp.offs) {
         lp.flag_period = K;
         lp.period = uniform ? std::min<int64_t>(K, swk::kUniformMaxPeriod) : K;
@@ -385,6 +388,10 @@
         const int P = swk::frame_classes(kind_packed(lp.kind), lp.rows, lp.lanes, lp.multi, uniform);
         p.wrap_class = code.encode_gap(-a * P);
         p.wrap_last = code.encode_gap(-a * ((lp.rows - 1) % P + (uniform ? 0 : 1)));
+        if (lp.short_stripes > 0) {
+            p.short_stripes = lp.short_stripes;
+            p.wrap_last_short = code.encode_gap(-a * ((lp.rows - 2) % P));
+        }
         p.flag_period = (int32_t)lp.flag_period;
         p.renorm_quads = (int32_t)(lp.period / 4);
         p.renorm_word = code.encode_gap(-(int)((int64_t)a * lp.period));
@@ -958,6 +965,11 @@
     return SW_OK;
 }
 
+int sw_launch_short_stripes(sw_ctx* ctx, int kind, int part_id, int32_t n, int32_t max_subject_len) {
+    if (!ctx || !kind_launch(kind) || !ctx->plan.have_query || part_id >= SW_NUM_LENGTH_PARTITIONS || max_subject_len < 0) return 0;
+    return swp::plan_launch(ctx->plan, sizing_request(kind, part_id, n, max_subject_len)).short_stripes;
+}
+
 int sw_launch_vgpr_slot(sw_ctx* ctx, int kind, int part_id, int32_t n, int32_t max_subject_len) {
     if (!ctx || !kind_launch(kind) || !ctx->plan.have_query || part_id >= SW_NUM_LENGTH_PARTITIONS || max_subject_len < 0) return 0;
     return swp::plan_launch(ctx->plan, sizing_request(kind, part_id, n, max_subject_len)).vgpr_slot;
diff --git a/cudasw4_amd/csrc/sw_ctx.hpp b/cudasw4_amd/csrc/sw_ctx.hpp
--- a/cudasw4_amd/csrc/sw_ctx.hpp
+++ b/cudasw4_amd/csrc/sw_ctx.hpp
@@ -21,7 +21,7 @@
     unsigned char* dev = nullptr;
     size_t capacity = 0;
     bool valid = false;
-    int rows = 0, nstripes = 0;
+    int rows = 0, nstripes = 0, short_stripes = 0;
     int shift = 0;
     hipEvent_t ready = nullptr;
 };
diff --git a/cudasw4_amd/csrc/sw_dp_kernel.hpp b/cudasw4_amd/csrc/sw_dp_kernel.hpp
--- a/cudasw4_amd/csrc/sw_dp_kernel.hpp
+++ b/cudasw4_amd/csrc/sw_dp_kernel.hpp
@@ -5,6 +5,7 @@
 
 #include <type_traits>
 
+#include "sw_plan.hpp"
 #include "sw_pssm.hpp"
 
 namespace swk {
@@ -309,6 +310,8 @@
     int32_t flag_period;
     int32_t chain;
     int32_t chain_all;
+    int32_t short_stripes;
+    u32 wrap_last_short;
     u32 levels[kLevelWords];
 };
 
@@ -403,13 +406,14 @@
     u32 Zc[P + 4];
 };
 
-template <int KIND, int R, int LANES, int BYTE, bool MULTI, bool OFFS = false, int P = 1, bool ZFILL = true, bool UNI = false, bool ADDR = false>
+template <int KIND, int R, int LANES, int BYTE, bool MULTI, bool OFFS = false, int P = 1, bool ZFILL = true, bool UNI = false, bool ADDR = false, int GR = R>
 __device__ __forceinline__ void dp_step(StripeState<KIND, R, P>& st, const unsigned char* tile,
                                         u32 lettersA, u32 lettersB, u32 gop, u32 gex, u32 inH, u32 inF,
                                         u32 apos = 0, bool first = false, u32 wrapP = 0, u32 wrapLast = 0, bool head = false,
                                         u32 laneStep = 0, const u32* zw = nullptr) {
     using A = Arith<KIND>;
-    using G = Geometry<KIND, R, LANES>;
+    using G = Geometry<KIND, GR, LANES>;
+    static_assert(GR == R || (GR == R + 1 && G::kWide), "a short stripe: one row less, wide words");
     const u32 step2 = LANES < 16 ? laneStep : 0x00100010u;
     const u32 step1 = LANES < 16 ? laneStep : 16u;
     constexpr u32 kSel = 0x0c0c000cu | ((u32)BYTE << 8);
@@ -659,6 +663,10 @@
 constexpr int min_waves() { return min_waves_of(KIND, R, LANES, MULTI); }
 constexpr int vgpr_slot_of(int KIND, int R, int LANES, bool MULTI) { return (512 / min_waves_of(KIND, R, LANES, MULTI)) & ~7; }
 
+constexpr bool mixed_stripes_kernel(bool packed, int R, int lanes, bool multi) {
+    return packed && multi && lanes == 16 && R >= 2 && R <= SWK_WAVES3_MAX_R_MULTI;
+}
+
 template <int KIND, int R, int LANES, bool MULTI, bool OFFS = false>
 __global__ void __launch_bounds__(kThreads, (min_waves<KIND, R, LANES, MULTI>())) sw_scan_kernel(const ScanParams p) {
     using A = Arith<KIND>;
@@ -671,6 +679,7 @@
     constexpr bool kUni = A::kPacked;
     constexpr bool kAddr = A::kPacked && MULTI && LANES == 16;
     constexpr bool kChain = kAddr;
+    constexpr bool kMixed = mixed_stripes_kernel(A::kPacked, R, LANES, MULTI);
     constexpr int P = OFFS ? frame_classes(A::kPacked, R, LANES, MULTI, kUni) : 1;
     __shared__ __attribute__((aligned(16))) unsigned char lds[16 + G::kTileBytes];
     __shared__ int chainEnd[kChain ? (kThreads / 64) * kChainMax : 1];
@@ -851,14 +860,17 @@
         }
 
         u32 maxv = 0u;
-        for (int stripe = 0; stripe < p.nstripes; stripe++) {
-            const bool first = stripe == 0;
+        auto stripe_body = [&](const int stripe, auto rows_tag) {
+            constexpr int RR = decltype(rows_tag)::value;
+            const bool first = RR == R && stripe == 0;
+            const bool border0 = RR != R && stripe == p.nstripes - p.short_stripes;
+            const u32 wrapLast = RR == R ? p.wrap_last : p.wrap_last_short;
             if constexpr (MULTI) {
                 __syncthreads();
                 load_tile<G::kTileBytes>(lds, p.profile + (size_t)stripe * G::kTileBytes);
                 __syncthreads();
             }
-            StripeState<KIND, R, P> st;
+            StripeState<KIND, RR, P> st;
             u32 zw[P + 5];
             const int tg0 = kUni ? __builtin_amdgcn_readfirstlane(LANES * stripe) : 0;
             auto load_levels = [&](int q) {
@@ -871,8 +883,8 @@
             if constexpr (kUni) {
                 load_levels(0);
 #pragma unroll
-                for (int r = 0; r < R; r++) { st.H[r] = zw[r % P]; st.E[r] = zw[r % P + 1]; }
-                st.upH_prev = A::gap(zw[(R - 1) % P], p.gex); st.Hlast = zw[(R - 1) % P]; st.Fout = zw[0];
+                for (int r = 0; r < RR; r++) { st.H[r] = zw[r % P]; st.E[r] = zw[r % P + 1]; }
+                st.upH_prev = A::gap((border0 && lane == 0) ? zw[(R - 1) % P] : zw[(RR - 1) % P], p.gex); st.Hlast = zw[(RR - 1) % P]; st.Fout = zw[0];
                 const u32 seed = (kChain && cnt > 1) ? 0u : maxv;
 #pragma unroll
                 for (int d = 0; d < P + 3; d++) st.maxv[d] = A::add(seed, zw[d + 1]);
@@ -882,8 +894,8 @@
 #pragma unroll
                 for (int k = 2; k < P + 5; k++) zc[k] = A::add(zc[k - 1], apos);
 #pragma unroll
-                for (int r = 0; r < R; r++) { st.H[r] = zc[r % P]; st.E[r] = zc[r % P + 1]; }
-                st.upH_prev = zc[(R - 1) % P]; st.Hlast = zc[(R - 1) % P]; st.Fout = zbefore;
+                for (int r = 0; r < RR; r++) { st.H[r] = zc[r % P]; st.E[r] = zc[r % P + 1]; }
+                st.upH_prev = zc[(RR - 1) % P]; st.Hlast = zc[(RR - 1) % P]; st.Fout = zbefore;
 #pragma unroll
                 for (int k = 0; k < P + 4; k++) st.Zc[k] = zc[k + 1];
 #pragma unroll
@@ -914,10 +926,10 @@
             const u32* const gIn = MULTI ? gBorder + 2 * (LANES - 1) + 4 * lane : nullptr;
             auto first_stripe_pairs = [&](int j) -> uint4 {
                 if constexpr (kUni) {
-                    constexpr int kLastClass = (R - 1) % P;
+                    constexpr int kLastClass = (RR - 1) % P;
                     return make_uint4(A::zero_at(p.gex_mag, (j & kmask) + kLastClass), A::kZero, A::zero_at(p.gex_mag, ((j + 1) & kmask) + kLastClass), A::kZero);
                 } else if constexpr (OFFS) {
-                    constexpr int kLastClass = (R - 1) % P;
+                    constexpr int kLastClass = (RR - 1) % P;
                     const int K = 4 * rq;
                     const int j0 = K > 0 ? (j & (K - 1)) : j, j1 = K > 0 ? ((j + 1) & (K - 1)) : j + 1;
                     return make_uint4(A::zero_at(p.gex_mag, j0 + LANES + kLastClass), A::kZero, A::zero_at(p.gex_mag, j1 + LANES + kLastClass), A::kZero);
@@ -965,7 +977,7 @@
                 if constexpr (kUni) {
                     const u32 w = p.renorm_word;
 #pragma unroll
-                    for (int r = 0; r < R; r++) { st.H[r] = A::lower(st.H[r], w); st.E[r] = A::lower(st.E[r], w); }
+                    for (int r = 0; r < RR; r++) { st.H[r] = A::lower(st.H[r], w); st.E[r] = A::lower(st.E[r], w); }
                     st.upH_prev = A::lower(st.upH_prev, w);
                     if constexpr (KIND == I16X2) st.upH_prev = A::true_max(st.upH_prev, A::gap(A::kZero, p.gex));
                     st.Hlast = A::lower(st.Hlast, w);
@@ -1001,8 +1013,8 @@
                             nxtW = stream_word(BYTE + 1);
                         }
                     }
-                    dp_step<KIND, R, LANES, BYTE, MULTI, OFFS, P, true, kUni, kAddr>(st, lds, lettersA, lettersB, p.gop, p.gex, in.x, in.y, apos, first,
-                                                                                 p.wrap_class, p.wrap_last, head, laneStep, zw);
+                    dp_step<KIND, RR, LANES, BYTE, MULTI, OFFS, P, true, kUni, kAddr, R>(st, lds, lettersA, lettersB, p.gop, p.gex, in.x, in.y, apos, first,
+                                                                                     p.wrap_class, wrapLast, head, laneStep, zw);
                     if constexpr (kUni && BYTE == 3) {
                         if (lower) lower_frame();
                     }
@@ -1043,8 +1055,8 @@
 #pragma unroll
                         for (int d = 0; d < P + 3; d++) st.maxv[d] = zw[d + 1];
 #pragma unroll
-                        for (int r = 0; r < R; r++) { st.H[r] = zw[r % P]; st.E[r] = zw[r % P + 1]; }
-                        st.upH_prev = A::gap(zw[(R - 1) % P], p.gex); st.Hlast = zw[(R - 1) % P]; st.Fout = zw[0];
+                        for (int r = 0; r < RR; r++) { st.H[r] = zw[r % P]; st.E[r] = zw[r % P + 1]; }
+                        st.upH_prev = A::gap((border0 && ln == 0) ? zw[(R - 1) % P] : zw[(RR - 1) % P], p.gex); st.Hlast = zw[(RR - 1) % P]; st.Fout = zw[0];
                     }
                 }
             };
@@ -1114,6 +1126,15 @@
                 maxv = st.maxv[0];
             }
             if constexpr (MULTI) __builtin_amdgcn_fence(__ATOMIC_RELEASE, "workgroup");
+        };
+        const int tallStripes = kMixed ? __builtin_amdgcn_readfirstlane(p.nstripes - p.short_stripes) : p.nstripes;
+        for (int stripe = 0; stripe < p.nstripes; stripe++) {
+            if constexpr (kMixed) {
+                if (stripe < tallStripes) stripe_body(stripe, std::integral_constant<int, R>{});
+                else stripe_body(stripe, std::integral_constant<int, R - 1>{});
+            } else {
+                stripe_body(stripe, std::integral_constant<int, R>{});
+            }
         }
 
         auto finish = [&](bool valid0, bool valid1, int pos0, int pos1, u32 maxv, int nq, int col0) {
@@ -1189,7 +1210,7 @@
 template <int KIND, int R, int LANES>
 __global__ void sw_build_profile_kernel(const int8_t* __restrict__ query, int32_t qlen,
                                         const int8_t* __restrict__ matrix21, int32_t pad_row, int32_t nstripes,
-                                        unsigned char* __restrict__ profile, int32_t shift, int32_t head_extra) {
+                                        unsigned char* __restrict__ profile, int32_t shift, int32_t head_extra, int32_t short_stripes) {
     using A = Arith<KIND>;
     using G = Geometry<KIND, R, LANES>;
     constexpr int kWordsPerRow = G::kRowBytes / 4;
@@ -1204,18 +1225,21 @@
         const int w = G::C::first(chunk) + sub;
         u32 v = 0;
         if (sub < G::C::words(chunk) && w < G::NW) {
+            const swp::StripeRows sr = swp::stripe_rows(LANES, R, nstripes, short_stripes, stripe);
+            const int h = sr.height;
             auto entry = [&](int row_in_lane) -> u32 {
-                if (row_in_lane >= R) return 0u;
-                const int64_t row = (int64_t)stripe * G::kStripeRows + lane * R + row_in_lane;
+                if (row_in_lane >= h) return 0u;
+                const int64_t row = sr.first_row + lane * h + row_in_lane;
                 const bool pssm = query == nullptr;
                 const int qc = row < qlen ? (pssm ? (int)row : (int)query[row]) : pad_row;
                 const int score = pssm ? (int)matrix21[pssm_index(qc, letter)] : (int)matrix21[qc * kLetters + letter];
                 const int P = frame_classes(A::kPacked, R, LANES, nstripes > 1, head_extra != 0);
-                const int cls = row_in_lane % P, above = (row_in_lane == 0 ? R - 1 : row_in_lane - 1) % P;
+                const bool border0 = short_stripes > 0 && stripe == nstripes - short_stripes && lane == 0;
+                const int cls = row_in_lane % P, above = (row_in_lane == 0 ? (border0 ? R - 1 : h - 1) : row_in_lane - 1) % P;
                 const int head = row_in_lane == 0 ? head_extra : 0;
                 return A::encode_score(score + shift * (1 + head + cls - above));
             };
-            if constexpr (G::kWide) v = w < R ? (entry(w) | (A::kOne << 16)) : 0u;
+            if constexpr (G::kWide) v = w < h ? (entry(w) | (A::kOne << 16)) : 0u;
             else if constexpr (A::kPacked) v = entry(2 * w) | (entry(2 * w + 1) << 16);
             else v = entry(w);
         }
diff --git a/cudasw4_amd/csrc/sw_kind_f16x2.hip b/cudasw4_amd/csrc/sw_kind_f16x2.hip
--- a/cudasw4_amd/csrc/sw_kind_f16x2.hip
+++ b/cudasw4_amd/csrc/sw_kind_f16x2.hip
@@ -3,15 +3,15 @@
 namespace swk {
 #define SWK_CASE_SCAN16_F16X2(R) case R: return launch_scan_r<F16X2, R, 16>(multi, offs, grid, reserve, stream, p);
 #define SWK_CASE_SCAN64_F16X2(R) case R: return launch_scan_r<F16X2, R, 64>(multi, offs, grid, reserve, stream, p);
-#define SWK_CASE_PROF16_F16X2(R) case R: return launch_profile_r<F16X2, R, 16>(q, qlen, m, pr, ns, out, shift, hx, s);
-#define SWK_CASE_PROF64_F16X2(R) case R: return launch_profile_r<F16X2, R, 64>(q, qlen, m, pr, ns, out, shift, hx, s);
+#define SWK_CASE_PROF16_F16X2(R) case R: return launch_profile_r<F16X2, R, 16>(q, qlen, m, pr, ns, out, shift, hx, ks, s);
+#define SWK_CASE_PROF64_F16X2(R) case R: return launch_profile_r<F16X2, R, 64>(q, qlen, m, pr, ns, out, shift, hx, ks, s);
 #define SWK_CASE_TILE16_F16X2(R) case R: return tile_bytes_r<F16X2, R, 16>();
 #define SWK_CASE_TILE64_F16X2(R) case R: return tile_bytes_r<F16X2, R, 64>();
 #define SWK_CASE_SCAN8_F16X2(R) case R: return launch_scan_r<F16X2, R, 8>(multi, offs, grid, reserve, stream, p);
-#define SWK_CASE_PROF8_F16X2(R) case R: return launch_profile_r<F16X2, R, 8>(q, qlen, m, pr, ns, out, shift, hx, s);
+#define SWK_CASE_PROF8_F16X2(R) case R: return launch_profile_r<F16X2, R, 8>(q, qlen, m, pr, ns, out, shift, hx, ks, s);
 #define SWK_CASE_TILE8_F16X2(R) case R: return tile_bytes_r<F16X2, R, 8>();
 #define SWK_CASE_SCAN4_F16X2(R) case R: return launch_scan_r<F16X2, R, 4>(multi, offs, grid, reserve, stream, p);
-#define SWK_CASE_PROF4_F16X2(R) case R: return launch_profile_r<F16X2, R, 4>(q, qlen, m, pr, ns, out, shift, hx, s);
+#define SWK_CASE_PROF4_F16X2(R) case R: return launch_profile_r<F16X2, R, 4>(q, qlen, m, pr, ns, out, shift, hx, ks, s);
 #define SWK_CASE_TILE4_F16X2(R) case R: return tile_bytes_r<F16X2, R, 4>();
 SWK_DEFINE_KIND(launch_f16x2, F16X2, SWK_FOR_EACH_R_PACKED)
 }
diff --git a/cudasw4_amd/csrc/sw_kind_f32.hip b/cudasw4_amd/csrc/sw_kind_f32.hip
--- a/cudasw4_amd/csrc/sw_kind_f32.hip
+++ b/cudasw4_amd/csrc/sw_kind_f32.hip
@@ -3,15 +3,15 @@
 namespace swk {
 #define SWK_CASE_SCAN16_F32(R) case R: return launch_scan_r<F32, R, 16>(multi, offs, grid, reserve, stream, p);
 #define SWK_CASE_SCAN64_F32(R) case R: return launch_scan_r<F32, R, 64>(multi, offs, grid, reserve, stream, p);
-#define SWK_CASE_PROF16_F32(R) case R: return launch_profile_r<F32, R, 16>(q, qlen, m, pr, ns, out, shift, hx, s);
-#define SWK_CASE_PROF64_F32(R) case R: return launch_profile_r<F32, R, 64>(q, qlen, m, pr, ns, out, shift, hx, s);
+#define SWK_CASE_PROF16_F32(R) case R: return launch_profile_r<F32, R, 16>(q, qlen, m, pr, ns, out, shift, hx, ks, s);
+#define SWK_CASE_PROF64_F32(R) case R: return launch_profile_r<F32, R, 64>(q, qlen, m, pr, ns, out, shift, hx, ks, s);
 #define SWK_CASE_TILE16_F32(R) case R: return tile_bytes_r<F32, R, 16>();
 #define SWK_CASE_TILE64_F32(R) case R: return tile_bytes_r<F32, R, 64>();
 #define SWK_CASE_SCAN8_F32(R) case R: return launch_scan_r<F32, R, 8>(multi, offs, grid, reserve, stream, p);
-#define SWK_CASE_PROF8_F32(R) case R: return launch_profile_r<F32, R, 8>(q, qlen, m, pr, ns, out, shift, hx, s);
+#define SWK_CASE_PROF8_F32(R) case R: return launch_profile_r<F32, R, 8>(q, qlen, m, pr, ns, out, shift, hx, ks, s);
 #define SWK_CASE_TILE8_F32(R) case R: return tile_bytes_r<F32, R, 8>();
 #define SWK_CASE_SCAN4_F32(R) case R: return launch_scan_r<F32, R, 4>(multi, offs, grid, reserve, stream, p);
-#define SWK_CASE_PROF4_F32(R) case R: return launch_profile_r<F32, R, 4>(q, qlen, m, pr, ns, out, shift, hx, s);
+#define SWK_CASE_PROF4_F32(R) case R: return launch_profile_r<F32, R, 4>(q, qlen, m, pr, ns, out, shift, hx, ks, s);
 #define SWK_CASE_TILE4_F32(R) case R: return tile_bytes_r<F32, R, 4>();
 SWK_DEFINE_KIND(launch_f32, F32, SWK_FOR_EACH_R_I32)
 }
diff --git a/cudasw4_amd/csrc/sw_kind_i16x2.hip b/cudasw4_amd/csrc/sw_kind_i16x2.hip
--- a/cudasw4_amd/csrc/sw_kind_i16x2.hip
+++ b/cudasw4_amd/csrc/sw_kind_i16x2.hip
@@ -3,15 +3,15 @@
 namespace swk {
 #define SWK_CASE_SCAN16_I16X2(R) case R: return launch_scan_r<I16X2, R, 16>(multi, offs, grid, reserve, stream, p);
 #define SWK_CASE_SCAN64_I16X2(R) case R: return launch_scan_r<I16X2, R, 64>(multi, offs, grid, reserve, stream, p);
-#define SWK_CASE_PROF16_I16X2(R) case R: return launch_profile_r<I16X2, R, 16>(q, qlen, m, pr, ns, out, shift, hx, s);
-#define SWK_CASE_PROF64_I16X2(R) case R: return launch_profile_r<I16X2, R, 64>(q, qlen, m, pr, ns, out, shift, hx, s);
+#define SWK_CASE_PROF16_I16X2(R) case R: return launch_profile_r<I16X2, R, 16>(q, qlen, m, pr, ns, out, shift, hx, ks, s);
+#define SWK_CASE_PROF64_I16X2(R) case R: return launch_profile_r<I16X2, R, 64>(q, qlen, m, pr, ns, out, shift, hx, ks, s);
 #define SWK_CASE_TILE16_I16X2(R) case R: return tile_bytes_r<I16X2, R, 16>();
 #define SWK_CASE_TILE64_I16X2(R) case R: return tile_bytes_r<I16X2, R, 64>();
 #define SWK_CASE_SCAN8_I16X2(R) case R: return launch_scan_r<I16X2, R, 8>(multi, offs, grid, reserve, stream, p);
-#define SWK_CASE_PROF8_I16X2(R) case R: return launch_profile_r<I16X2, R, 8>(q, qlen, m, pr, ns, out, shift, hx, s);
+#define SWK_CASE_PROF8_I16X2(R) case R: return launch_profile_r<I16X2, R, 8>(q, qlen, m, pr, ns, out, shift, hx, ks, s);
 #define SWK_CASE_TILE8_I16X2(R) case R: return tile_bytes_r<I16X2, R, 8>();
 #define SWK_CASE_SCAN4_I16X2(R) case R: return launch_scan_r<I16X2, R, 4>(multi, offs, grid, reserve, stream, p);
-#define SWK_CASE_PROF4_I16X2(R) case R: return launch_profile_r<I16X2, R, 4>(q, qlen, m, pr, ns, out, shift, hx, s);
+#define SWK_CASE_PROF4_I16X2(R) case R: return launch_profile_r<I16X2, R, 4>(q, qlen, m, pr, ns, out, shift, hx, ks, s);
 #define SWK_CASE_TILE4_I16X2(R) case R: return tile_bytes_r<I16X2, R, 4>();
 SWK_DEFINE_KIND(launch_i16x2, I16X2, SWK_FOR_EACH_R_PACKED)
 }
diff --git a/cudasw4_amd/csrc/sw_kind_i32.hip b/cudasw4_amd/csrc/sw_kind_i32.hip
--- a/cudasw4_amd/csrc/sw_kind_i32.hip
+++ b/cudasw4_amd/csrc/sw_kind_i32.hip
@@ -3,15 +3,15 @@
 namespace swk {
 #define SWK_CASE_SCAN16_I32(R) case R: return launch_scan_r<I32, R, 16>(multi, offs, grid, reserve, stream, p);
 #define SWK_CASE_SCAN64_I32(R) case R: return launch_scan_r<I32, R, 64>(multi, offs, grid, reserve, stream, p);
-#define SWK_CASE_PROF16_I32(R) case R: return launch_profile_r<I32, R, 16>(q, qlen, m, pr, ns, out, shift, hx, s);
-#define SWK_CASE_PROF64_I32(R) case R: return launch_profile_r<I32, R, 64>(q, qlen, m, pr, ns, out, shift, hx, s);
+#define SWK_CASE_PROF16_I32(R) case R: return launch_profile_r<I32, R, 16>(q, qlen, m, pr, ns, out, shift, hx, ks, s);
+#define SWK_CASE_PROF64_I32(R) case R: return launch_profile_r<I32, R, 64>(q, qlen, m, pr, ns, out, shift, hx, ks, s);
 #define SWK_CASE_TILE16_I32(R) case R: return tile_bytes_r<I32, R, 16>();
 #define SWK_CASE_TILE64_I32(R) case R: return tile_bytes_r<I32, R, 64>();
 #define SWK_CASE_SCAN8_I32(R) case R: return launch_scan_r<I32, R, 8>(multi, offs, grid, reserve, stream, p);
-#define SWK_CASE_PROF8_I32(R) case R: return launch_profile_r<I32, R, 8>(q, qlen, m, pr, ns, out, shift, hx, s);
+#define SWK_CASE_PROF8_I32(R) case R: return launch_profile_r<I32, R, 8>(q, qlen, m, pr, ns, out, shift, hx, ks, s);
 #define SWK_CASE_TILE8_I32(R) case R: return tile_bytes_r<I32, R, 8>();
 #define SWK_CASE_SCAN4_I32(R) case R: return launch_scan_r<I32, R, 4>(multi, offs, grid, reserve, stream, p);
-#define SWK_CASE_PROF4_I32(R) case R: return launch_profile_r<I32, R, 4>(q, qlen, m, pr, ns, out, shift, hx, s);
+#define SWK_CASE_PROF4_I32(R) case R: return launch_profile_r<I32, R, 4>(q, qlen, m, pr, ns, out, shift, hx, ks, s);
 #define SWK_CASE_TILE4_I32(R) case R: return tile_bytes_r<I32, R, 4>();
 SWK_DEFINE_KIND(launch_i32, I32, SWK_FOR_EACH_R_I32)
 }
diff --git a/cudasw4_amd/csrc/sw_launch.hpp b/cudasw4_amd/csrc/sw_launch.hpp
--- a/cudasw4_amd/csrc/sw_launch.hpp
+++ b/cudasw4_amd/csrc/sw_launch.hpp
@@ -39,7 +39,7 @@
 struct KindLaunch {
     hipError_t (*scan)(int R, int lanes, bool multi, bool offs, int grid, int reserve, hipStream_t stream, const ScanParams& p);
     hipError_t (*profile)(int R, int lanes, const int8_t* query, int32_t qlen, const int8_t* matrix21, int32_t pad_row,
-                          int32_t nstripes, unsigned char* out, int32_t shift, int32_t head_extra, hipStream_t stream);
+                          int32_t nstripes, unsigned char* out, int32_t shift, int32_t head_extra, int32_t short_stripes, hipStream_t stream);
     size_t (*tile_bytes)(int R, int lanes);
     hipError_t (*warm)(hipStream_t stream);
     bool packed;
@@ -132,14 +132,16 @@
 
 template <int KIND, int R, int LANES>
 hipError_t launch_profile_r(const int8_t* query, int32_t qlen, const int8_t* matrix21, int32_t pad_row, int32_t nstripes,
-                            unsigned char* out, int32_t shift, int32_t head_extra, hipStream_t stream) {
+                            unsigned char* out, int32_t shift, int32_t head_extra, int32_t short_stripes, hipStream_t stream) {
     if constexpr (R > max_rows(KIND, LANES)) {
         return hipErrorInvalidValue;
     } else {
+        if (short_stripes < 0 || (short_stripes > 0 && (short_stripes >= nstripes || !mixed_stripes_kernel(Arith<KIND>::kPacked, R, LANES, nstripes > 1))))
+            return hipErrorInvalidValue;
         const size_t total = (size_t)nstripes * kLetters * (Geometry<KIND, R, LANES>::kRowBytes / 4);
         const int grid = (int)std::min<size_t>((total + 255) / 256, 65536);
         hipLaunchKernelGGL((sw_build_profile_kernel<KIND, R, LANES>), dim3(grid), dim3(256), 0, stream, query, qlen,
-                           matrix21, pad_row, nstripes, out, shift, head_extra);
+                           matrix21, pad_row, nstripes, out, shift, head_extra, short_stripes);
         return hipGetLastError();
     }
 }
@@ -166,7 +168,7 @@
         return hipErrorInvalidValue;                                                                                \
     }                                                                                                               \
     static hipError_t FN##_profile(int R, int lanes, const int8_t* q, int32_t qlen, const int8_t* m, int32_t pr,    \
-                                   int32_t ns, unsigned char* out, int32_t shift, int32_t hx, hipStream_t s) {      \
+                                   int32_t ns, unsigned char* out, int32_t shift, int32_t hx, int32_t ks, hipStream_t s) { \
         if (lanes == 16) { switch (R) { FOR_EACH_R(SWK_CASE_PROF16_##KIND) } }                                      \
         else if (lanes == 64) { switch (R) { FOR_EACH_R(SWK_CASE_PROF64_##KIND) } }                                 \
         else if (lanes == 8) { switch (R) { FOR_EACH_R(SWK_CASE_PROF8_##KIND) } }                                   \
diff --git a/cudasw4_amd/csrc/sw_plan.hpp b/cudasw4_amd/csrc/sw_plan.hpp
--- a/cudasw4_amd/csrc/sw_plan.hpp
+++ b/cudasw4_amd/csrc/sw_plan.hpp
@@ -47,6 +47,7 @@
     int kind = 0;
     bool fell_back = false;
     int lanes = 16, rows = 0, nstripes = 0;
+    int short_stripes = 0;
     bool multi = false;
     bool offs = false;
     int frame = 0;
@@ -65,4 +66,18 @@
 
 LaunchPlan plan_launch(const PlanSettings& s, const LaunchRequest& req);
 
+constexpr int short_stripes_of(int32_t qlen, int lanes, int rows, int nstripes) {
+    const int64_t spare = (int64_t)rows * nstripes - ((int64_t)qlen + lanes - 1) / lanes;
+    return (qlen <= 0 || rows < 2 || nstripes < 2 || spare <= 0) ? 0 : (int)(spare < nstripes - 1 ? spare : nstripes - 1);
 }
+struct StripeRows {
+    int height;
+    int64_t first_row;
+};
+constexpr StripeRows stripe_rows(int lanes, int rows, int nstripes, int short_stripes, int stripe) {
+    const int tall = nstripes - short_stripes;
+    return stripe < tall ? StripeRows{rows, (int64_t)lanes * rows * stripe}
+                         : StripeRows{rows - 1, (int64_t)lanes * rows * tall + (int64_t)lanes * (rows - 1) * (stripe - tall)};
+}
+
+}
diff --git a/include/cudasw4_amd_engine.h b/include/cudasw4_amd_engine.h
--- a/include/cudasw4_amd_engine.h
+++ b/include/cudasw4_amd_engine.h
@@ -31,6 +31,7 @@
 
 int sw_launch_vgpr_slot(sw_ctx* ctx, int kind, int part_id, int32_t n, int32_t max_subject_len);
 int sw_set_rows_pipeline_slot(sw_ctx* ctx, int vgprs);
+int sw_launch_short_stripes(sw_ctx* ctx, int kind, int part_id, int32_t n, int32_t max_subject_len);
 size_t sw_scan_rows_pipelined_temp_bytes(sw_ctx* ctx, int32_t n, int32_t max_subject_len);
 int sw_scan_rows_pipelined(sw_ctx* ctx, const int8_t* chars, const uint64_t* offsets, const int32_t* lengths,
                            int32_t first_pos, int32_t n, int32_t max_subject_len, int gop, int gex, float* scores,
```
